# chrism0dwk/covid19uk

Hardware: AMD Instinct MI355X
Metric: posterior samples/sec, 380-LAD UK SEIR (higher is better)
Workload: dtype f64; 1 GPU; uk380: M=380 LADs x T=365 days, P=750 parameters; chains_per_gpu=8, chains_total=8, sweep=HMC(16 leapfrogs) + 5 x [S->E move, E->I move, S->E occult, E->I occult], draws_recorded=theta + events[M,T,3] (uint16 counts) + kernel results per sweep, parallelism=chains sharded over 1 GPU(s), no data-path collective

## Files before the change

covid19uk_amd/_lib.py:

```python
from __future__ import annotations

import ctypes
import os

_HERE = os.path.dirname(os.path.abspath(__file__))
LIB_PATH = os.path.join(_HERE, "libseirhip.so")

c_double_p = ctypes.POINTER(ctypes.c_double)
c_void_pp = ctypes.POINTER(ctypes.c_void_p)
c_int64_p = ctypes.POINTER(ctypes.c_int64)


class SeirDesc(ctypes.Structure):
    _fields_ = [
        ("M", ctypes.c_int32), ("T", ctypes.c_int32),
        ("max_chains", ctypes.c_int32), ("device", ctypes.c_int32),
        ("Cstar", c_double_p), ("N", c_double_p), ("W", c_double_p),
        ("weekday_c", c_double_p), ("log_area_c", c_double_p),
        ("car_Q", c_double_p), ("car_half_logdet", ctypes.c_double),
        ("init_state", c_double_p),
        ("nu", ctypes.c_double), ("time_delta", ctypes.c_double),
        ("rate_floor", ctypes.c_double),
    ]


class SeirSamplerDesc(ctypes.Structure):
    _fields_ = [
        ("num_chains", ctypes.c_int32),
        ("dmax", ctypes.c_int32), ("nmax", ctypes.c_int32), ("m", ctypes.c_int32),
        ("occult_nmax", ctypes.c_int32), ("num_event_time_updates", ctypes.c_int32),
        ("t_range_lo", ctypes.c_int32), ("t_range_hi", ctypes.c_int32),
        ("num_leapfrog_steps", ctypes.c_int32), ("trace_capacity", ctypes.c_int32),
        ("first_chain_id", ctypes.c_int32), ("record_events", ctypes.c_int32),
        ("seed", ctypes.c_uint64),
        ("moves_mode", ctypes.c_int32), ("hmc_mode", ctypes.c_int32), ("use_graph", ctypes.c_int32),
        ("chain_groups", ctypes.c_int32), ("disable_mask", ctypes.c_int32), ("debug_pair", ctypes.c_int32),
        ("leap_rows", ctypes.c_int32), ("thin", ctypes.c_int32),
    ]


class SeirSimDesc(ctypes.Structure):
    _fields_ = [
        ("num_draws", ctypes.c_int32), ("num_steps", ctypes.c_int32),
        ("first_draw_id", ctypes.c_int32), ("reserved", ctypes.c_int32),
        ("seed", ctypes.c_uint64),
        ("par", ctypes.POINTER(ctypes.c_double)), ("log_baseline", ctypes.POINTER(ctypes.c_double)),
        ("spatial", ctypes.POINTER(ctypes.c_double)), ("W", ctypes.POINTER(ctypes.c_double)),
        ("weekday_c", ctypes.POINTER(ctypes.c_double)), ("init_state", ctypes.POINTER(ctypes.c_double)),
        ("events", ctypes.POINTER(ctypes.c_double)),
    ]


ABI_VERSION = 4
OPT_DEBUG_SKEW, OPT_XCD_AFFINITY, OPT_GEMM_F32, OPT_EVAL_FORM, OPT_RT_STAGING_KIB = 0, 1, 2, 3, 4
ERR_INVALID, ERR_STATE = -1, -3
ERR_HANDOFF = -4
MMAX = 4
MOVE_TRACE = 2 + 4 * MMAX
FORECAST_MAX_H = 128
FORECAST_ID_SHIFT, FORECAST_MAX_CHAIN = 20, 2048
CHECK_MAX_DAYS = 128
ORDER_STATS_MAX_RANKS = 16
GROUPS_MAX = 256
SELFTEST_FN = {"fast_log": (0, False, False), "fast_rcp": (1, False, False), "mv_log": (2, False, False),
               "softplus_tab": (3, False, False), "softplus_sigmoid_tab": (4, False, True), "softplus": (5, False, False),
               "lfact_bf": (6, False, False), "lbinom_tab": (7, True, False), "lbinom_const": (8, True, False),
               "lbinom_bf": (9, True, False), "log1mexp_tab": (10, False, False), "log1mexp": (11, False, False),
               "log1mexp_series": (12, False, True), "l1me_inv_series": (13, False, True), "l1me_inv_k": (14, False, True),
               "l1me_inv_series_k": (15, False, True), "log1mexp_diff_slow": (16, True, False), "fast_log_k": (17, False, False)}
SELFTEST_DELTA = {"band": 0, "own_ei": 1, "own_se": 2}
SELFTEST_WAVE = {"wave_sum": (0, True), "wave_min": (1, False), "wave_incl_scan": (2, True),
                 "wave_incl_suffix_scan": (3, False), "block_excl_scan_256": (4, True),
                 "block_incl_suffix_scan_256": (5, False), "block_sum_256": (6, False)}


class SeirError(RuntimeError):
    def __init__(self, msg, code=0):
        super().__init__(msg)
        self.code = code


class HandoffTimeout(SeirError):
    """A wait inside one of the persistent launches gave up (SEIR_ERR_HANDOFF from a read of the trace): its
    workgroups were not all resident -- something else holds part of the GPU.  `ChainSampler` recovers from it by
    itself (snapshot, restore, per-step launch forms)."""


_SIGNATURES = {
    "seir_abi_version": (ctypes.c_int, []),
    "seir_last_error": (ctypes.c_char_p, []),
    "seir_create": (ctypes.c_int, [ctypes.POINTER(SeirDesc), c_void_pp]),
    "seir_destroy": (None, [ctypes.c_void_p]),
    "seir_num_params": (ctypes.c_int, [ctypes.c_void_p]),
    "seir_set_initial_state": (ctypes.c_int, [ctypes.c_void_p, c_double_p]),
    "seir_log_prob": (ctypes.c_int, [ctypes.c_void_p, ctypes.c_int32, c_double_p, c_double_p, c_double_p]),
    "seir_log_prob_grad": (ctypes.c_int, [ctypes.c_void_p, ctypes.c_int32, c_double_p, c_double_p,
                                          c_double_p, c_double_p]),
    "seir_log_prob_dev": (ctypes.c_int, [ctypes.c_void_p, ctypes.c_int32] + [ctypes.c_void_p] * 4),
    "seir_prepare_events_dev": (ctypes.c_int, [ctypes.c_void_p, ctypes.c_int32, ctypes.c_void_p]),
    "seir_eval_prepared_dev": (ctypes.c_int, [ctypes.c_void_p, ctypes.c_int32] + [ctypes.c_void_p] * 3),
    "seir_sync": (ctypes.c_int, [ctypes.c_void_p]),
    "seir_stream": (ctypes.c_void_p, [ctypes.c_void_p]),
    "seir_set_option": (ctypes.c_int, [ctypes.c_void_p, ctypes.c_int32, ctypes.c_int32]),
    "seir_malloc": (ctypes.c_int, [c_void_pp, ctypes.c_uint64]),
    "seir_free": (ctypes.c_int, [ctypes.c_void_p]),
    "seir_memcpy_h2d": (ctypes.c_int, [ctypes.c_void_p, ctypes.c_void_p, ctypes.c_uint64]),
    "seir_memcpy_d2h": (ctypes.c_int, [ctypes.c_void_p, ctypes.c_void_p, ctypes.c_uint64]),
    "seir_timer_start": (ctypes.c_int, [ctypes.c_void_p]),
    "seir_timer_stop": (ctypes.c_int, [ctypes.c_void_p, ctypes.POINTER(ctypes.c_float)]),
    "seir_time_kernel": (ctypes.c_int, [ctypes.c_void_p, ctypes.c_int32, ctypes.c_int32, ctypes.c_int32,
                                        ctypes.POINTER(ctypes.c_float)]),
    "seir_selftest_math": (ctypes.c_int, [ctypes.c_void_p, ctypes.c_int32] + [c_double_p] * 4),
    "seir_selftest_math_wide": (ctypes.c_int, [ctypes.c_void_p, ctypes.c_int32] + [c_double_p] * 3),
    "seir_selftest_fn": (ctypes.c_int, [ctypes.c_void_p, ctypes.c_int32, ctypes.c_int32] + [c_double_p] * 4),
    "seir_selftest_band_delta": (ctypes.c_int, [ctypes.c_void_p, ctypes.c_int32, ctypes.c_int32] + [c_double_p] * 7 +
                                 [ctypes.c_double, ctypes.c_double, c_double_p]),
    "seir_selftest_wave": (ctypes.c_int, [ctypes.c_void_p, ctypes.c_int32, ctypes.c_int32, ctypes.c_int32] +
                           [ctypes.c_void_p] * 3),
    "seir_reproduction_number": (ctypes.c_int, [ctypes.c_void_p, ctypes.c_int32, c_double_p, c_double_p, c_double_p]),
    "seir_within_between": (ctypes.c_int, [ctypes.c_void_p, ctypes.c_int32, c_double_p, c_double_p, ctypes.c_double,
                                           c_double_p, c_double_p]),
    "seir_simulate": (ctypes.c_int, [ctypes.c_void_p, ctypes.POINTER(SeirSimDesc)]),
    "seir_selftest_binomial": (ctypes.c_int, [ctypes.c_void_p, ctypes.c_int32, ctypes.POINTER(ctypes.c_int32),
                                              c_double_p, ctypes.c_uint64, ctypes.POINTER(ctypes.c_int32)]),
    "seir_sampler_create": (ctypes.c_int, [ctypes.c_void_p, ctypes.POINTER(SeirSamplerDesc), c_void_pp]),
    "seir_sampler_destroy": (None, [ctypes.c_void_p]),
    "seir_sampler_set_state": (ctypes.c_int, [ctypes.c_void_p, c_double_p, c_double_p]),
    "seir_sampler_get_state": (ctypes.c_int, [ctypes.c_void_p, c_double_p, c_double_p, c_double_p]),
    "seir_sampler_set_kernel": (ctypes.c_int, [ctypes.c_void_p, c_double_p, c_double_p]),
    "seir_sampler_get_kernel": (ctypes.c_int, [ctypes.c_void_p, c_double_p, c_double_p]),
    "seir_sampler_set_adaptation": (ctypes.c_int, [ctypes.c_void_p, ctypes.c_int32, ctypes.c_int32,
                                                   ctypes.c_int32, ctypes.c_double, c_double_p, c_double_p,
                                                   c_double_p]),
    "seir_sampler_refresh": (ctypes.c_int, [ctypes.c_void_p]),
    "seir_sampler_reset_trace": (ctypes.c_int, [ctypes.c_void_p]),
    "seir_sampler_reset_trace_at": (ctypes.c_int, [ctypes.c_void_p, ctypes.c_int32]),
    "seir_sampler_set_thin": (ctypes.c_int, [ctypes.c_void_p, ctypes.c_int32]),
    "seir_sampler_thin": (ctypes.c_int, [ctypes.c_void_p, ctypes.POINTER(ctypes.c_int32)]),
    "seir_sampler_read_trace_async": (ctypes.c_int, [ctypes.c_void_p, ctypes.c_int32, ctypes.c_int32, c_double_p,
                                                     ctypes.c_void_p, c_double_p, c_double_p]),
    "seir_sampler_trace_wait": (ctypes.c_int, [ctypes.c_void_p]),
    "seir_host_alloc": (ctypes.c_int, [c_void_pp, ctypes.c_uint64]),
    "seir_host_free": (ctypes.c_int, [ctypes.c_void_p]),
    "seir_sampler_run": (ctypes.c_int, [ctypes.c_void_p, ctypes.c_int32]),
    "seir_sampler_read_trace": (ctypes.c_int, [ctypes.c_void_p, ctypes.c_int32, ctypes.c_int32, c_double_p,
                                               ctypes.c_void_p, c_double_p, c_double_p]),
    "seir_sampler_time_grad_kernel": (ctypes.c_int, [ctypes.c_void_p, ctypes.c_int32,
                                                     ctypes.POINTER(ctypes.c_float)]),
    "seir_sampler_time_leapfrog": (ctypes.c_int, [ctypes.c_void_p, ctypes.c_int32, ctypes.POINTER(ctypes.c_float),
                                                  ctypes.POINTER(ctypes.c_int32), ctypes.POINTER(ctypes.c_int32)]),
    "seir_sampler_pair_timeouts": (ctypes.c_int, [ctypes.c_void_p, ctypes.POINTER(ctypes.c_uint32)]),
    "seir_sampler_xcd_local": (ctypes.c_int, [ctypes.c_void_p]),
    "seir_sampler_snapshot": (ctypes.c_int, [ctypes.c_void_p, ctypes.c_int32]),
    "seir_sampler_restore": (ctypes.c_int, [ctypes.c_void_p, ctypes.c_int32]),
    "seir_sampler_debug_fail_handoff": (ctypes.c_int, [ctypes.c_void_p, ctypes.c_int32]),
    "seir_sampler_set_launch_form": (ctypes.c_int, [ctypes.c_void_p, ctypes.c_int32, ctypes.c_int32]),
    "seir_sampler_launch_form": (ctypes.c_int, [ctypes.c_void_p, ctypes.POINTER(ctypes.c_int32),
                                                ctypes.POINTER(ctypes.c_int32)]),
    "seir_sampler_summary_reset": (ctypes.c_int, [ctypes.c_void_p]),
    "seir_sampler_summarize": (ctypes.c_int, [ctypes.c_void_p, ctypes.c_int32, ctypes.c_int32, ctypes.c_int32]),
    "seir_sampler_read_marginals": (ctypes.c_int, [ctypes.c_void_p, ctypes.c_int32, ctypes.c_int32,
                                                   c_int64_p, c_int64_p, c_int64_p]),
    "seir_sampler_read_marginals_async": (ctypes.c_int, [ctypes.c_void_p, ctypes.c_int32, ctypes.c_int32,
                                                         c_int64_p, c_int64_p, c_int64_p]),
    "seir_sampler_read_summary": (ctypes.c_int, [ctypes.c_void_p, ctypes.POINTER(ctypes.c_uint64),
                                                 ctypes.POINTER(ctypes.c_int32), c_int64_p,
                                                 ctypes.POINTER(ctypes.c_uint64)]),
    "seir_sampler_diag_reset": (ctypes.c_int, [ctypes.c_void_p, ctypes.c_int32]),
    "seir_sampler_diag_mark": (ctypes.c_int, [ctypes.c_void_p, ctypes.c_int32]),
    "seir_sampler_read_diag": (ctypes.c_int, [ctypes.c_void_p, ctypes.POINTER(ctypes.c_uint64), c_int64_p,
                                              ctypes.POINTER(ctypes.c_uint64)]),
    "seir_sampler_read_diag_mark": (ctypes.c_int, [ctypes.c_void_p, ctypes.c_int32, ctypes.POINTER(ctypes.c_uint64),
                                                   c_int64_p, ctypes.POINTER(ctypes.c_uint64)]),
    "seir_sampler_forecast_reset": (ctypes.c_int, [ctypes.c_void_p, ctypes.c_int32, c_double_p, c_double_p, ctypes.c_uint64]),
    "seir_sampler_forecast": (ctypes.c_int, [ctypes.c_void_p, ctypes.c_int32, ctypes.c_int32, c_double_p]),
    "seir_sampler_read_forecast_marginals": (ctypes.c_int, [ctypes.c_void_p, ctypes.c_int32, ctypes.c_int32,
                                                            c_int64_p, c_int64_p, c_int64_p]),
    "seir_sampler_read_forecast_marginals_async": (ctypes.c_int, [ctypes.c_void_p, ctypes.c_int32, ctypes.c_int32,
                                                                  c_int64_p, c_int64_p, c_int64_p]),
    "seir_sampler_read_forecast": (ctypes.c_int, [ctypes.c_void_p, ctypes.POINTER(ctypes.c_uint64),
                                                  ctypes.POINTER(ctypes.c_int32), c_int64_p,
                                                  ctypes.POINTER(ctypes.c_uint64)]),
    "seir_sampler_forecast_keep": (ctypes.c_int, [ctypes.c_void_p, ctypes.c_int64]),
    "seir_sampler_forecast_order_stats": (ctypes.c_int, [ctypes.c_void_p, c_int64_p, ctypes.c_int32, ctypes.c_int32,
                                                         ctypes.POINTER(ctypes.c_int32)]),
    "seir_order_stats": (ctypes.c_int, [ctypes.c_void_p, ctypes.POINTER(ctypes.c_int32), ctypes.c_int64, ctypes.c_int32,
                                        ctypes.c_int64, ctypes.c_int64, ctypes.c_int64, c_int64_p, ctypes.c_int32,
                                        ctypes.POINTER(ctypes.c_int32)]),
    "seir_sampler_check_reset": (ctypes.c_int, [ctypes.c_void_p, ctypes.c_int32, c_double_p, c_double_p, ctypes.c_uint64]),
    "seir_sampler_check": (ctypes.c_int, [ctypes.c_void_p, ctypes.c_int32, ctypes.c_int32]),
    "seir_sampler_read_check": (ctypes.c_int, [ctypes.c_void_p, ctypes.POINTER(ctypes.c_uint64),
                                               ctypes.POINTER(ctypes.c_int32), c_int64_p, ctypes.POINTER(ctypes.c_uint64)]),
    "seir_sampler_read_check_marginals": (ctypes.c_int, [ctypes.c_void_p, ctypes.c_int32, ctypes.c_int32,
                                                         c_int64_p, c_int64_p, c_int64_p]),
    "seir_sampler_read_check_marginals_async": (ctypes.c_int, [ctypes.c_void_p, ctypes.c_int32, ctypes.c_int32,
                                                               c_int64_p, c_int64_p, c_int64_p]),
    "seir_sampler_read_check_counts": (ctypes.c_int, [ctypes.c_void_p, ctypes.POINTER(ctypes.c_int32)] +
                                       [ctypes.POINTER(ctypes.c_uint32)] * 8),
    "seir_sampler_rt_reset": (ctypes.c_int, [ctypes.c_void_p, ctypes.c_int32, c_double_p]),
    "seir_sampler_rt": (ctypes.c_int, [ctypes.c_void_p, ctypes.c_int32, ctypes.c_int32]),
    "seir_sampler_read_rt_draws": (ctypes.c_int, [ctypes.c_void_p, ctypes.c_int32, ctypes.c_int32, c_double_p]),
    "seir_sampler_read_rt_draws_async": (ctypes.c_int, [ctypes.c_void_p, ctypes.c_int32, ctypes.c_int32, c_double_p]),
    "seir_sampler_read_rt": (ctypes.c_int, [ctypes.c_void_p, ctypes.POINTER(ctypes.c_uint64), c_double_p, c_double_p,
                                            c_double_p, ctypes.POINTER(ctypes.c_uint32)]),
    "seir_sampler_rt_keep": (ctypes.c_int, [ctypes.c_void_p, ctypes.c_int64]),
    "seir_sampler_rt_order_stats": (ctypes.c_int, [ctypes.c_void_p, c_int64_p, ctypes.c_int32, ctypes.c_int32, c_double_p]),
    "seir_order_stats_f64": (ctypes.c_int, [ctypes.c_void_p, c_double_p, ctypes.c_int64, ctypes.c_int32, ctypes.c_int64,
                                            ctypes.c_int64, ctypes.c_int64, c_int64_p, ctypes.c_int32, c_double_p]),
    "seir_sampler_wb_reset": (ctypes.c_int, [ctypes.c_void_p, ctypes.c_int32]),
    "seir_sampler_wb": (ctypes.c_int, [ctypes.c_void_p, ctypes.c_int32, ctypes.c_int32]),
    "seir_sampler_read_wb": (ctypes.c_int, [ctypes.c_void_p, ctypes.POINTER(ctypes.c_uint64), ctypes.POINTER(ctypes.c_uint32),
                                            c_double_p, c_double_p, c_double_p, c_double_p, c_double_p,
                                            ctypes.POINTER(ctypes.c_uint32)]),
    "seir_sampler_read_wb_draws": (ctypes.c_int, [ctypes.c_void_p, ctypes.c_int32, ctypes.c_int32, c_double_p, c_double_p]),
    "seir_sampler_read_wb_draws_async": (ctypes.c_int, [ctypes.c_void_p, ctypes.c_int32, ctypes.c_int32, c_double_p,
                                                        c_double_p]),
    "seir_sampler_groups_set": (ctypes.c_int, [ctypes.c_void_p, ctypes.c_int32, ctypes.POINTER(ctypes.c_int32),
                                               ctypes.POINTER(ctypes.c_int32)]),
    "seir_sampler_read_group_marginals": (ctypes.c_int, [ctypes.c_void_p, ctypes.c_int32, ctypes.c_int32, ctypes.c_int32,
                                                         c_int64_p, c_int64_p]),
    "seir_sampler_read_group_marginals_async": (ctypes.c_int, [ctypes.c_void_p, ctypes.c_int32, ctypes.c_int32, ctypes.c_int32,
                                                               c_int64_p, c_int64_p]),
    "seir_group_sums": (ctypes.c_int, [ctypes.c_void_p, ctypes.POINTER(ctypes.c_int32), ctypes.c_int64, ctypes.c_int32,
                                       ctypes.c_int32, ctypes.c_int32, ctypes.POINTER(ctypes.c_int32),
                                       ctypes.POINTER(ctypes.c_int32), c_int64_p]),
    "seir_sampler_group_rt": (ctypes.c_int, [ctypes.c_void_p, c_double_p]),
    "seir_sampler_group_wb": (ctypes.c_int, [ctypes.c_void_p, ctypes.c_int32]),
    "seir_sampler_read_group_rt": (ctypes.c_int, [ctypes.c_void_p, ctypes.c_int32, ctypes.c_int32, c_double_p]),
    "seir_sampler_read_group_rt_async": (ctypes.c_int, [ctypes.c_void_p, ctypes.c_int32, ctypes.c_int32, c_double_p]),
    "seir_sampler_read_group_wb": (ctypes.c_int, [ctypes.c_void_p, ctypes.c_int32, ctypes.c_int32, c_double_p, c_double_p]),
    "seir_sampler_read_group_wb_async": (ctypes.c_int, [ctypes.c_void_p, ctypes.c_int32, ctypes.c_int32, c_double_p, c_double_p]),
    "seir_group_wsums": (ctypes.c_int, [ctypes.c_void_p, c_double_p, ctypes.c_int64, ctypes.c_int32, ctypes.c_int32,
                                        ctypes.c_int32, ctypes.POINTER(ctypes.c_int32), ctypes.POINTER(ctypes.c_int32),
                                        c_double_p, c_double_p]),
}

_lib = None


def exported_symbols():
    return sorted(_SIGNATURES)


def load():
    global _lib
    if _lib is None:
        if not os.path.exists(LIB_PATH):
            raise SeirError(
                f"{LIB_PATH} not found: build the HIP extension first "
                "(python -c 'import __graft_entry__ as g; g.build()'). "
                "This package has no CPU fallback.")
        try:
            import torch
        except ImportError:
            pass
        lib = ctypes.CDLL(LIB_PATH)
        for name, (res, args) in _SIGNATURES.items():
            fn = getattr(lib, name)
            fn.restype = res
            fn.argtypes = args
        if lib.seir_abi_version() != ABI_VERSION:
            raise SeirError(f"{LIB_PATH} has ABI {lib.seir_abi_version()}, this binding needs {ABI_VERSION}: rebuild it")
        _lib = lib
    return _lib


def check(rc):
    if rc != 0:
        msg = load().seir_last_error()
        text = msg.decode() if msg else "?"
        cls = HandoffTimeout if rc == ERR_HANDOFF else SeirError
        raise cls(f"libseirhip call failed ({rc}): {text}", rc)
```

covid19uk_amd/csrc/moves_kernel.h:

```cpp
#pragma once
#include "handoff.h"
#include "sampler_kernels.h"

namespace seir {

#ifdef SEIR_STAMPS
#ifndef SEIR_STAMP_SLOT
#define SEIR_STAMP_SLOT 1
#endif
#define MSTAMP(i) do { if (threadIdx.x == 0 && stamp_on) ((unsigned long long *)(stamp_hs + 16))[i] = __builtin_amdgcn_s_memrealtime(); } while (0)
#else
#define MSTAMP(i) do {} while (0)
#endif

#ifdef PAIR_STAMPS
#define QSTAMP(slot_, step_, i_) do { if (threadIdx.x == 0 && (b_stamp) == 0 && (step_) < 12 && (slot_) < 27) \
    ch.leap_st[((size_t)(slot_) * 12 + (step_)) * 16 + (i_)] = __builtin_amdgcn_s_memrealtime(); } while (0)
#else
#define QSTAMP(slot_, step_, i_) do {} while (0)
#endif

constexpr int MVB = 512;
constexpr int MVW = MVB / WAVE;
constexpr int MVU = 4;

struct MvShared {
    Move mv;
    int acc;
    int nsel;
    int sel[MMAX];
    int ired[MVW * 4];
    double dred[MVW * 2];
    double u[2 * MMAX][2];
    double logq_part[MMAX];
    int pend_valid[MMAX];
};

template <int CTRL, int ROW_MASK>
__device__ __forceinline__ int dpp_min_step(int v) {
    return min(v, __builtin_amdgcn_update_dpp(0x7fffffff, v, CTRL, ROW_MASK, 0xf, false));
}
__device__ __forceinline__ int wave_min_int(int v) {
    v = dpp_min_step<0x111, 0xf>(v);
    v = dpp_min_step<0x112, 0xf>(v);
    v = dpp_min_step<0x114, 0xf>(v);
    v = dpp_min_step<0x118, 0xf>(v);
    v = dpp_min_step<0x142, 0xa>(v);
    v = dpp_min_step<0x143, 0xc>(v);
    return __builtin_amdgcn_readlane(v, 63);
}

__device__ __forceinline__ void mv_sum2(double &a, double &b2, double *sh) {
    a = wave_sum(a); b2 = wave_sum(b2);
    const int lane = threadIdx.x & 63, wave = threadIdx.x >> 6;
    lds_barrier();
    if (lane == 0) { sh[wave * 2] = a; sh[wave * 2 + 1] = b2; }
    lds_barrier();
    double x = 0.0, y = 0.0;
#pragma unroll
    for (int j = 0; j < MVW; ++j) { x += sh[j * 2]; y += sh[j * 2 + 1]; }
    a = x; b2 = y;
}

struct MvLds {
    const int *rt;
    int *rg;
#ifdef SEIR_STAMPS
    double *stamp_hs; bool stamp_on;
#endif
};

__device__ __forceinline__ double mv_log(double x, const double2 *ltab) { return x == 1.0 ? 0.0 : fast_log(x, ltab); }

__device__ inline void mv_draw(const SamplerCfg &s, const Chains &ch, int b, MoveSpec spec, MvShared &sm, int T) {
    Move &mv = sm.mv;
    const int tid = threadIdx.x;
    if (tid >= 2 * MMAX && tid != 64) return;
    const RngKey key = rng_key(s, ch, b);
    const uint32_t stream = RS_MOVE_BASE + (uint32_t)(spec.scan * 4 + spec.slot);
    if (tid < 2 * MMAX) rng_uniform2(key, stream, (uint32_t)tid, sm.u[tid][0], sm.u[tid][1]);
    if (tid == 64) {
        mv.valid = (s.disable_mask >> (1 + spec.slot)) & 1 ? 0 : 1;
        mv.n = 0; mv.tgt = spec.tgt; mv.kind = spec.kind; mv.slot = spec.slot;
        mv.logq = 0.0; mv.any_dI = 0; mv.LO = T; mv.HI = -1;
        for (int j = 0; j < MMAX; ++j) { mv.tm[j] = mv.tt[j] = mv.tdt[j] = mv.tx[j] = 0; mv.b[j] = -1; sm.pend_valid[j] = -1; }
        double ua, ub;
        rng_uniform2(key, stream, 15u, ua, ub);
        mv.logu = cold_log(ua);
    }
}

__device__ __forceinline__ int wv_popc(unsigned long long m) { return __builtin_popcountll(m); }
__device__ __forceinline__ int wv_kth_bit(unsigned long long mask, int k, int lane) {
    const int below = (int)__builtin_amdgcn_mbcnt_hi((unsigned)(mask >> 32), __builtin_amdgcn_mbcnt_lo((unsigned)mask, 0u));
    const bool me = ((mask >> lane) & 1ull) != 0ull && below == k;
    return (int)__builtin_ctzll(__builtin_amdgcn_ballot_w64(me));
}
constexpr int WV_MCH = 6;
struct HotRows {
    unsigned long long mask[WV_MCH];
    int H;
};
__device__ __forceinline__ HotRows wv_hot_rows(const int *tot, int M, int lane) {
    HotRows h;
    h.H = 0;
    if (M <= WV_MCH * WAVE) {
        int v[WV_MCH];
#pragma unroll
        for (int c = 0; c < WV_MCH; ++c) { const int m = c * WAVE + lane; v[c] = m < M ? tot[m] : 0; }
#pragma unroll
        for (int c = 0; c < WV_MCH; ++c) { h.mask[c] = __builtin_amdgcn_ballot_w64(v[c] > 0); h.H += wv_popc(h.mask[c]); }
    } else {
#pragma unroll
        for (int c = 0; c < WV_MCH; ++c) h.mask[c] = 0ull;
        for (int m0 = 0; m0 < M; m0 += WAVE) {
            const int m = m0 + lane;
            h.H += wv_popc(__builtin_amdgcn_ballot_w64(m < M && tot[m] > 0));
        }
    }
    return h;
}
__device__ __forceinline__ int wv_hot_row(const HotRows &h, const int *tot, int M, int p, int lane) {
    int row = 0;
    bool found = false;
    if (M <= WV_MCH * WAVE) {
#pragma unroll
        for (int c = 0; c < WV_MCH; ++c) {
            const int cnt = wv_popc(h.mask[c]);
            if (!found && p < cnt) { row = c * WAVE + wv_kth_bit(h.mask[c], p, lane); found = true; }
            if (!found) p -= cnt;
        }
    } else {
        for (int m0 = 0; m0 < M; m0 += WAVE) {
            const int m = m0 + lane;
            const unsigned long long mask = __builtin_amdgcn_ballot_w64(m < M && tot[m] > 0);
            const int cnt = wv_popc(mask);
            if (!found && p < cnt) { row = m0 + wv_kth_bit(mask, p, lane); found = true; }
            if (!found) p -= cnt;
        }
    }
    return row;
}
template <int NCH>
__device__ __forceinline__ int wv_at(const int (&v)[NCH], int t) {
    int r = 0;
#pragma unroll
    for (int c = 0; c < NCH; ++c)
        if ((t >> 6) == c) r = __builtin_amdgcn_readlane(v[c], t & 63);
    return r;
}

template <int NCH>
__device__ inline void mv_propose_wave(const Dims &d, const Work &w, const SamplerCfg &s, const Chains &ch, int b,
                                       MoveSpec spec, MvShared &sm, const MvLds &L, const double2 *ltab,
                                       bool rows_only) {
    Move &mv = sm.mv;
    const int tid = threadIdx.x, wave = tid >> 6, lane = tid & 63, M = d.M, T = d.T;
#ifdef SEIR_STAMPS
    double *stamp_hs = L.stamp_hs; const bool stamp_on = L.stamp_on;
#endif
    MSTAMP(4);
    const int tgt = spec.tgt;
    lds_barrier();
    if (spec.kind == 0) {
        const int *rt = L.rt;
        const HotRows hr = wv_hot_rows(rt, M, lane);
        const int H = hr.H;
        const int nsel = min(min(s.mmax, MMAX), H);
        int pos[MMAX], chosen[MMAX], rowj[MMAX];
#pragma unroll
        for (int j = 0; j < MMAX; ++j) { pos[j] = 0; rowj[j] = 0; chosen[j] = 0x7fffffff; }
#pragma unroll
        for (int j = 0; j < MMAX; ++j) {
            if (j < nsel) {
                int p = rng_index(sm.u[2 * j][0], H - j);
#pragma unroll
                for (int a = 0; a < MMAX; ++a)
                    if (a < j && p >= chosen[a]) ++p;
                pos[j] = p;
                chosen[j] = p;
#pragma unroll
                for (int a = MMAX - 1; a >= 1; --a)
                    if (a <= j && chosen[a - 1] > chosen[a]) { const int tmp = chosen[a]; chosen[a] = chosen[a - 1]; chosen[a - 1] = tmp; }
            }
        }
#pragma unroll
        for (int j = 0; j < MMAX; ++j)
            if (j < nsel) rowj[j] = wv_hot_row(hr, rt, M, pos[j], lane);
        if (rows_only) {
            if (tid == 0) {
                sm.nsel = nsel;
#pragma unroll
                for (int j = 0; j < MMAX; ++j)
                    if (j < nsel) sm.sel[j] = rowj[j];
            }
            lds_barrier();
            return;
        }
        MSTAMP(5);
        if (wave < nsel) {
            const int j = wave;
            int m = 0;
#pragma unroll
            for (int jj = 0; jj < MMAX; ++jj)
                if (jj == j) m = rowj[jj];
            const size_t rowoff = ((size_t)b * d.Mp + m) * d.Tp;
            int rk[NCH], rsrc[NCH], rdst[NCH];
#pragma unroll
            for (int c = 0; c < NCH; ++c) {
                const int t = c * WAVE + lane;
                const bool in = t < T;
                rk[c] = in ? w.K[tgt][rowoff + t] : 0;
                rsrc[c] = in ? w.St[tgt][rowoff + t] : 0;
                rdst[c] = in ? w.St[tgt + 1][rowoff + t] : 0;
            }
            MSTAMP(6);
            int D = 0;
            unsigned long long hot[NCH];
#pragma unroll
            for (int c = 0; c < NCH; ++c) { hot[c] = __builtin_amdgcn_ballot_w64(rk[c] > 0); D += wv_popc(hot[c]); }
            int r = rng_index(sm.u[2 * j][1], D), t = 0;
            {
                bool found = false;
#pragma unroll
                for (int c = 0; c < NCH; ++c) {
                    const int cnt = wv_popc(hot[c]);
                    if (!found && r < cnt) { t = c * WAVE + wv_kth_bit(hot[c], r, lane); found = true; }
                    if (!found) r -= cnt;
                }
            }
            MSTAMP(7);
// ... 323 lines not shown
            } else {
                __syncthreads();
                for (int m = tid; m < M; m += MVB) rtl[m] = w.rowtot[((size_t)b * 2 + next.tgt) * d.Mp + m];
            }
            lds_barrier();
        } else {
            if (pre_rt) {
#pragma unroll
                for (int k = 0; k < PRE_RT; ++k) {
                    const int m = tid + k * MVB;
                    if (m < M) L.rg[m] = rt_pre[k];
                }
                lds_barrier();
                if (patch && tid == 0)
                    for (int i = 0; i < pend.n; ++i) {
                        if (pend.a[i] >= s.tr_lo && pend.a[i] < s.tr_hi) L.rg[pend.m[i]] += pend.dka[i];
                        if (pend.b[i] >= s.tr_lo && pend.b[i] < s.tr_hi) L.rg[pend.m[i]] += pend.dkb[i];
                    }
                lds_barrier();
            } else {
                __syncthreads();
                range_totals_to_lds(d, w, s, b, next.tgt, L.rg);
            }
        }
        MSTAMP(3);
#ifdef SEIR_STAMPS
        L.stamp_hs = stamp_hs; L.stamp_on = stamp_on;
#endif
        mv_propose<NCH>(d, w, s, ch, b, next, sm, L, ltab);
        MSTAMP(10);
        if (tid == 0) ch.mv[(size_t)(pbuf ^ 1) * s.B + b] = sm.mv;
        MSTAMP(11);
    }
}

constexpr int PRE_RT = 4;

__device__ __forceinline__ void mv_prefetch_rows(const Dims &d, const Work &w, const SamplerCfg &s, int b, MoveSpec spec,
                                                 bool on, int (&pre)[PRE_RT]) {
    const int tid = threadIdx.x;
#pragma unroll
    for (int k = 0; k < PRE_RT; ++k) {
        const int m = tid + k * MVB;
        pre[k] = 0;
        if (on && m < d.M) {
            if (spec.kind == 0) {
                pre[k] = w.rowtot[((size_t)b * 2 + spec.tgt) * d.Mp + m];
            } else {
                pre[k] = w.rngtot[((size_t)b * 2 + spec.tgt) * d.Mp + m];
            }
        }
    }
}

__device__ __forceinline__ void mv_rows_to_lds(const Dims &d, const Work &w, const SamplerCfg &s, int b, MoveSpec spec,
                                               bool pre_ok, const int (&pre)[PRE_RT], const Move *fix, MvLds &L,
                                               int *rtl) {
    const int tid = threadIdx.x, M = d.M;
    int *dst = spec.kind == 0 ? rtl : L.rg;
    if (pre_ok) {
#pragma unroll
        for (int k = 0; k < PRE_RT; ++k) {
            const int m = tid + k * MVB;
            if (m < M) dst[m] = pre[k];
        }
        lds_barrier();
        if (fix && tid == 0)
            for (int i = 0; i < fix->n; ++i) {
                if (spec.kind == 0) {
                    dst[fix->m[i]] += fix->dka[i] + fix->dkb[i];
                } else {
                    if (fix->a[i] >= s.tr_lo && fix->a[i] < s.tr_hi) dst[fix->m[i]] += fix->dka[i];
                    if (fix->b[i] >= s.tr_lo && fix->b[i] < s.tr_hi) dst[fix->m[i]] += fix->dkb[i];
                }
            }
        lds_barrier();
    } else {
        __syncthreads();
        if (spec.kind == 0) {
            for (int m = tid; m < M; m += MVB) dst[m] = w.rowtot[((size_t)b * 2 + spec.tgt) * d.Mp + m];
            lds_barrier();
        } else {
            range_totals_to_lds(d, w, s, b, spec.tgt, L.rg);
        }
    }
}

__device__ __forceinline__ void mv_apply_rows(const Dims &d, const Work &w, const SamplerCfg &s, int b, const Move &mv,
                                              int *trans = nullptr) {
    const int tid = threadIdx.x;
    for (int i = 0; i < mv.n; ++i) {
        const size_t rowoff = ((size_t)b * d.Mp + mv.m[i]) * d.Tp;
        const int src = mv.tgt, dst = mv.tgt + 1;
        for (int t = mv.lo[i] + 1 + tid; t <= mv.hi[i]; t += MVB) {
            w.St[src][rowoff + t] += mv.dsrc[i];
            w.St[dst][rowoff + t] -= mv.dsrc[i];
            if (mv.tgt == 1) w.Dir[(size_t)b * d.Tp + t] -= (double)mv.dsrc[i];
        }
        if (tid == 0) {
            w.K[mv.tgt][rowoff + mv.a[i]] += mv.dka[i];
            if (mv.b[i] >= 0) w.K[mv.tgt][rowoff + mv.b[i]] += mv.dkb[i];
            int *prt = w.rowtot + ((size_t)b * 2 + mv.tgt) * d.Mp + mv.m[i];
            const int dk = mv.dka[i] + mv.dkb[i];
            const int ra = (mv.a[i] >= s.tr_lo && mv.a[i] < s.tr_hi) ? mv.dka[i] : 0;
            const int rb = (mv.b[i] >= s.tr_lo && mv.b[i] < s.tr_hi) ? mv.dkb[i] : 0;
            int *prg = w.rngtot + ((size_t)b * 2 + mv.tgt) * d.Mp + mv.m[i];
            if (trans != nullptr) {
                const int rt0 = *prt, rg0 = (ra + rb != 0) ? *prg : 1;
                int tb = 0;
                if ((rt0 > 0) != (rt0 + dk > 0)) tb |= 1;
                if (ra + rb != 0 && (rg0 > 0) != (rg0 + ra + rb > 0)) tb |= 2;
                *trans |= tb;
                *prt = rt0 + dk;
                if (ra + rb != 0) *prg = rg0 + ra + rb;
            } else {
                *prt += dk;
                if (ra + rb != 0) *prg += ra + rb;
            }
        }
        __syncthreads();
    }
}

__device__ __forceinline__ void mv_trace(const SamplerCfg &s, const Chains &ch, int b, const Move &mv, int acc,
                                         unsigned tr_slot, double lp) {
    if (tr_slot < (unsigned)s.cap) {
        double *tr = ch.tr_mv + (((size_t)tr_slot * s.B + b) * 4 + mv.slot) * NMVTR;
        tr[0] = (double)acc;
        tr[1] = lp;
        for (int j = 0; j < MMAX; ++j) {
            tr[2 + j] = mv.tm[j]; tr[2 + MMAX + j] = mv.tt[j];
            tr[2 + 2 * MMAX + j] = mv.tdt[j]; tr[2 + 3 * MMAX + j] = mv.tx[j];
        }
    }
}

__device__ __forceinline__ void mv_own_rows_to_down(const Dims &d, const Consts &c, const Work &w, int b, const Move &mv,
                                                    double psi, const double2 *ltab, const Move *fp, double *red,
                                                    double *od) {
    double dth = 0.0, dcn = 0.0;
    if (mv.valid && mv.n > 0) own_rows_delta<MVB>(d, c, w, b, mv, psi, 0, d.M, ltab, dth, dcn, fp);
    mv_sum2(dth, dcn, red);
    if (threadIdx.x == 0) {
        od[0] = dth;
        od[1] = dcn;
    }
}

struct PairNote {
    int ok;
    int n, rows[MMAX];
};
static_assert(sizeof(PairNote) == (2 + MMAX) * sizeof(int), "k_move_pair writes the note as 2 + MMAX ints");

__device__ __forceinline__ void move_copy_l2(Move *dst, const Move *src, int t0) {
    const int i = (int)threadIdx.x - t0;
    if (i >= 0 && i < MOVE_DW) reinterpret_cast<int *>(dst)[i] = ld_l2(reinterpret_cast<const int *>(src) + i);
}
__device__ __forceinline__ void wait_token(const unsigned *p_, unsigned token, unsigned *late) {
    hs_wait<1, HS_CHECK, HS_LIMIT, HS_CALLER>([&] { return ld_l2(p_) == token; }, late);
}
__device__ __forceinline__ unsigned wait_token_flag(const unsigned *p_, unsigned token, unsigned *late) {
    unsigned v;
    hs_wait<1, HS_CHECK, HS_LIMIT, HS_CALLER>([&] { return ((v = ld_l2(p_)) & 0x7fffffffu) == token; }, late);
    return v >> 31;
}
static_assert((MOVE_DW + 1) / 2 <= 32, "Chains::llmv holds 32 words per descriptor");
template <bool SOLO, typename TT>
__device__ __forceinline__ TT ld_band(const TT *p_) { return SOLO ? *p_ : ld_l2(p_); }
template <bool SOLO, int NRB>
__device__ __forceinline__ void pair_band_block(const Dims &d, const Consts &c, const Work &w, const SamplerCfg &s,
                                                const Chains &ch, int b, int bx, int nband, unsigned token, bool has_r1,
                                                bool has_r2, int buf, int st_slot = 0, int st_step = 0) {
    const int b_stamp = b - d.b0;
    (void)b_stamp;
    __shared__ Move mvA, mvB, fp;
    __shared__ int mv_sel;
    __shared__ double sh_th[MVW], sh_cn[MVW];
    __shared__ double2 ltab[LDSTAB_N];
    int tid = threadIdx.x;
    asm volatile("" : "+v"(tid));
    const int wave = tid >> 6, lane = tid & 63;
    if (tid < LDSTAB_N) ltab[tid] = c.logtab[tid];
    const double psi = w.scal[(size_t)b * NSCAL + SC_PSI];
    const unsigned *done = ch.done + (size_t)b * 2 * TAIL_STRIDE;
    const int rpb = (d.M + nband - 1) / nband;
    const int r_lo = bx * rpb, r_hi = min(d.M, r_lo + rpb);
#ifndef PAIR_BAND_BACKOFF
#define PAIR_BAND_BACKOFF 0
#endif
    if (tid == 0) {
        if (PAIR_BAND_BACKOFF > 0) __builtin_amdgcn_s_sleep(PAIR_BAND_BACKOFF);
        wait_token(done + 4, token, ch.late + ch.late_fatal + b);
    }
    QSTAMP(st_slot, st_step, 1);
    __syncthreads();
    move_copy_l2(&fp, ch.fpend + b, 128);
    __syncthreads();
    const bool has_fp = fp.valid == 1;
    constexpr int NPF = 2;
    constexpr bool PREF = NRB == 2;
    constexpr int NRP = PREF ? NRB : 1;
    double cfb[NRP][MMAX], Fpre[NRP][NPF];
#pragma unroll
    for (int r = 0; r < NRP; ++r) {
        const int j = r_lo + wave + r * MVW;
        const bool onr = PREF && has_fp && j < r_hi;
#pragma unroll
        for (int i = 0; i < MMAX; ++i)
            cfb[r][i] = (onr && i < fp.n) ? c.Cstar[(size_t)fp.m[i] * d.Kp0 + j] * c.invN[fp.m[i]] * (double)(-fp.dsrc[i]) : 0.0;
#pragma unroll
        for (int q = 0; q < NPF; ++q) {
            const int t = fp.LO + q * WAVE + lane;
            Fpre[r][q] = (onr && t <= fp.HI) ? ld_band<SOLO>(w.F + ((size_t)b * d.Mp + j) * d.Tp + t) : 0.0;
        }
    }
    const bool pre_ok = PREF && (!has_fp || fp.HI - fp.LO < NPF * WAVE);
    if (tid == 0) wait_token(done + 5, token, ch.late + ch.late_fatal + b);
    if (has_r1) {
        if (wave == 1) move_wait_ll<MOVE_DW>(reinterpret_cast<int *>(&mvA), ch.llmv + ((size_t)buf * s.B + b) * 32, lane, token, ch.late + ch.late_fatal + b);
        QSTAMP(st_slot, st_step, 2);
        __syncthreads();
    } else {
        QSTAMP(st_slot, st_step, 2);
        __syncthreads();
        move_copy_l2(&mvA, ch.mv + (size_t)buf * s.B + b, 0);
        __syncthreads();
    }
    auto evaluate = [&](const Move &mv) -> double {
        double dth = 0.0;
        if (mv.valid && mv.n > 0 && mv.any_dI) {
            const double *ea = w.ea + (size_t)b * d.Tp;
            constexpr int NR = 2;
    #pragma unroll 1
            for (int r0 = 0; r0 < NRB; r0 += NR) {
            int jr[NR];
            bool on[NR];
            double eb[NR], coef[NR][MMAX], cfp[NR][MMAX];
    #pragma unroll
            for (int r = 0; r < NR; ++r) {
                jr[r] = r_lo + wave + (r0 + r) * MVW;
                bool mine = false;
    #pragma unroll
                for (int i = 0; i < MMAX; ++i) mine |= (i < mv.n && mv.m[i] == jr[r]);
                on[r] = jr[r] < r_hi && !mine;
                const int j = on[r] ? jr[r] : r_lo;
                eb[r] = w.eb[(size_t)b * d.Mp + j];
    #pragma unroll
                for (int i = 0; i < MMAX; ++i) {
                    coef[r][i] = (on[r] && i < mv.n) ? c.Cstar[(size_t)mv.m[i] * d.Kp0 + j] * c.invN[mv.m[i]] * (double)(-mv.dsrc[i]) : 0.0;
                    if (PREF) cfp[r][i] = on[r] ? cfb[PREF ? r : 0][i] : 0.0;
                    else cfp[r][i] = (has_fp && on[r] && i < fp.n) ? c.Cstar[(size_t)fp.m[i] * d.Kp0 + j] * c.invN[fp.m[i]] * (double)(-fp.dsrc[i]) : 0.0;
                }
            }
            for (int t0 = mv.LO; t0 <= mv.HI; t0 += WAVE) {
                const int t = t0 + lane;
                double dF[NR], S[NR], I[NR], kse[NR], F[NR];
                bool act[NR];
    #pragma unroll
                for (int r = 0; r < NR; ++r) {
                    dF[r] = 0.0;
    #pragma unroll
                    for (int i = 0; i < MMAX; ++i)
                        if (i < mv.n && t > mv.lo[i] && t <= mv.hi[i]) dF[r] += coef[r][i];
                    act[r] = on[r] && t <= mv.HI && dF[r] != 0.0;
                    const size_t q = ((size_t)b * d.Mp + (on[r] ? jr[r] : r_lo)) * d.Tp + (act[r] ? t : mv.LO);
                    S[r] = (double)ld_band<SOLO>(w.St[0] + q); I[r] = (double)ld_band<SOLO>(w.St[2] + q);
                    kse[r] = (double)ld_band<SOLO>(w.K[0] + q); F[r] = ld_band<SOLO>(w.F + q);
                }
    #pragma unroll
                for (int r = 0; r < NR; ++r) {
                    if (!act[r]) continue;
                    if (has_fp) {
                        double dFp = 0.0;
    #pragma unroll
                        for (int i = 0; i < MMAX; ++i)
                            if (i < fp.n && t > fp.lo[i] && t <= fp.hi[i]) dFp += cfp[r][i];
                        if (dFp != 0.0) F[r] += dFp;
                    }
                    dth += band_delta(S[r], I[r], kse[r], F[r], dF[r], ea[t] * eb[r], psi * c.W[t], d.rate_floor * d.dt, d.dt, ltab);
                }
            }
            }
        }
        return dth;
    };
    double dth = evaluate(mvA);
    QSTAMP(st_slot, st_step, 3);
    if (tid == 0) mv_sel = (int)wait_token_flag(done + 0, token, ch.late + ch.late_fatal + b);
    __syncthreads();
    if (mv_sel) {
        move_copy_l2(&mvB, ch.mvfix + (size_t)buf * s.B + b, 64);
        __syncthreads();
        dth = evaluate(mvB);
    }
    dth = wave_sum(dth);
    if (lane == 0) sh_th[wave] = dth;
    __syncthreads();
    double dsum = 0.0;
    if (tid == 0) {
#pragma unroll
        for (int k = 0; k < MVW; ++k) dsum += sh_th[k];
        if (!SOLO) {
            double *out = ch.Dpart + ((size_t)b * nband + bx) * 2;
            out[0] = dsum;
            out[1] = 0.0;
        }
        QSTAMP(st_slot, st_step, 4);
        if (has_fp) {
            if (has_r1) wait_token(done + 1, token, ch.late + ch.late_fatal + b);
            if (has_r2) wait_token(done + 2, token, ch.late + ch.late_fatal + b);
        }
        QSTAMP(st_slot, st_step, 5);
    }
    auto publish = [&]() {
        if (!SOLO) return;
        asm volatile("s_waitcnt vmcnt(0)" ::: "memory");
        __syncthreads();
        if (tid == 0) {
            uint4 *out = ch.llD + (((size_t)buf * s.B + b) * nband + bx) * 2;
            pair_sums_store(out, dsum, 0.0, token);
            QSTAMP(st_slot, st_step, 10);
        }
    };
    if (!has_fp) { publish(); return; }
    if (!has_fp) return;
    __syncthreads();
#pragma unroll
    for (int r = 0; r < NRB; ++r) {
        const int j = r_lo + wave + r * MVW;
        if (j >= r_hi) continue;
        double *Fr = w.F + ((size_t)b * d.Mp + j) * d.Tp;
        double cfr[MMAX];
#pragma unroll
        for (int i = 0; i < MMAX; ++i) {
            if (PREF) cfr[i] = cfb[PREF ? r : 0][i];
            else cfr[i] = i < fp.n ? c.Cstar[(size_t)fp.m[i] * d.Kp0 + j] * c.invN[fp.m[i]] * (double)(-fp.dsrc[i]) : 0.0;
        }
        if (pre_ok) {
#pragma unroll
            for (int q = 0; q < NPF; ++q) {
                const int t = fp.LO + q * WAVE + lane;
                double dFp = 0.0;
#pragma unroll
                for (int i = 0; i < MMAX; ++i)
                    if (i < fp.n && t > fp.lo[i] && t <= fp.hi[i]) dFp += cfr[i];
                if (t <= fp.HI && dFp != 0.0) Fr[t] = Fpre[PREF ? r : 0][q] + dFp;
            }
        } else {
            for (int t = fp.LO + lane; t <= fp.HI; t += WAVE) {
                double dFp = 0.0;
#pragma unroll
                for (int i = 0; i < MMAX; ++i)
                    if (i < fp.n && t > fp.lo[i] && t <= fp.hi[i]) dFp += cfr[i];
                if (dFp != 0.0) Fr[t] = ld_band<SOLO>(Fr + t) + dFp;
            }
        }
    }
    publish();
    (void)sh_cn;
}

__device__ __forceinline__ void pair_band_finish(const Dims &d, const Consts &c, const Work &w, const SamplerCfg &s,
                                                 const Chains &ch, int b, int bx, int nband, unsigned token, unsigned slot,
                                                 int record) {
    __shared__ Move fp;
    int tid = threadIdx.x;
    asm volatile("" : "+v"(tid));
    const int wave = tid >> 6, lane = tid & 63;
    const unsigned *done = ch.done + (size_t)b * 2 * TAIL_STRIDE;
    const int rpb = (d.M + nband - 1) / nband;
    const int r_lo = bx * rpb, r_hi = min(d.M, r_lo + rpb);
    if (tid == 0) wait_token(done + 4, token, ch.late + ch.late_fatal + b);
    __syncthreads();
    move_copy_l2(&fp, ch.fpend + b, 128);
    if (tid == 0) wait_token(done + 5, token, ch.late + ch.late_fatal + b);
    __syncthreads();
    for (int m = r_lo + wave; m < r_hi; m += MVW) {
        if (fp.valid == 1) {
            double coef[MMAX];
#pragma unroll
            for (int i = 0; i < MMAX; ++i)
                coef[i] = i < fp.n ? c.Cstar[(size_t)fp.m[i] * d.Kp0 + m] * c.invN[fp.m[i]] * (double)(-fp.dsrc[i]) : 0.0;
            double *Fr = w.F + ((size_t)b * d.Mp + m) * d.Tp;
            for (int t = fp.LO + lane; t <= fp.HI; t += WAVE) {
                double dF = 0.0;
#pragma unroll
                for (int i = 0; i < MMAX; ++i)
                    if (i < fp.n && t > fp.lo[i] && t <= fp.hi[i]) dF += coef[i];
                if (dF != 0.0) Fr[t] += dF;
            }
        }
        if (!record || slot >= (unsigned)s.cap) continue;
        const size_t o0 = (((size_t)slot * s.B + b) * d.M + m) * d.T * 3;
        int *out = (int *)ch.tr_events + o0;
        unsigned short *out16 = (unsigned short *)ch.tr_events + o0;
        const size_t q0 = ((size_t)b * d.Mp + m) * d.Tp;
        for (int t0 = 0; t0 < d.T; t0 += 4 * WAVE) {
            int k0[4], k1[4], k2[4];
#pragma unroll
            for (int j = 0; j < 4; ++j) {
                const int t = t0 + j * WAVE + lane;
                const bool in = t < d.Tp;
                k0[j] = in ? w.K[0][q0 + t] : 0;
                k1[j] = in ? w.K[1][q0 + t] : 0;
                k2[j] = in ? w.K[2][q0 + t] : 0;
            }
#pragma unroll
            for (int j = 0; j < 4; ++j) {
                const int t = t0 + j * WAVE + lane;
                if (t < d.T) {
                    if (s.ev16) {
                        if ((unsigned)(k0[j] | k1[j] | k2[j]) > 0xffffu) ch.ev_overflow[0] = 1u;
                        out16[t * 3 + 0] = (unsigned short)k0[j]; out16[t * 3 + 1] = (unsigned short)k1[j];
                        out16[t * 3 + 2] = (unsigned short)k2[j];
                    } else {
                        out[t * 3 + 0] = k0[j]; out[t * 3 + 1] = k1[j]; out[t * 3 + 2] = k2[j];
                    }
                }
            }
        }
    }
}

template <int NCH, bool SOLO>
__device__ __forceinline__ void pair_step(const Dims &d, const Consts &c, const Work &w, const SamplerCfg &s, const Chains &ch,
                                          MoveSpec se, MoveSpec next, MoveSpec se_next, int have_prev, int have_pre, int pbuf,
                                          int lidx, int dbg, int nband, int nroles, int slot, int b, int fin = 0,
                                          unsigned sweep0 = 0u, int lprev = 0, unsigned tslot = TRACE_NOT_RECORDED) {
    extern __shared__ __attribute__((aligned(16))) int dyn_i[];
    __shared__ MvShared sm_se, sm_nx;
    __shared__ Move pendA, pendB;
    __shared__ PairNote note;
    __shared__ double pre_down[2], s_down[4], s_dsum[2];
    __shared__ double2 ltab[LDSTAB_N];
    __shared__ int s_sel, s_acc_se, s_conf, s_late, s_late2, s_use_pre, s_trans;
    int tid = threadIdx.x;
    asm volatile("" : "+v"(tid));
    asm volatile("" : "+s"(b));
    const int b_stamp = b - d.b0;
    (void)b_stamp;
    QSTAMP(slot, lidx, 0);
    if (slot >= nroles) {
        if (nband == 0) return;
        if (fin) {
            pair_band_finish(d, c, w, s, ch, b, slot - nroles, nband, pair_token(sweep0, lidx), tslot, fin & 2);
            return;
        }
        const unsigned tok = pair_token(ch.sweep[b], lidx);
        const bool r1 = next.kind >= 0 && nroles >= 2, r2 = se_next.kind >= 0 && nroles == 3;
        if ((d.M + nband - 1) / nband > 2 * MVW)
            pair_band_block<SOLO, 4>(d, c, w, s, ch, b, slot - nroles, nband, tok, r1, r2, pbuf ^ 1, slot, lidx);
        else
            pair_band_block<SOLO, 2>(d, c, w, s, ch, b, slot - nroles, nband, tok, r1, r2, pbuf ^ 1, slot, lidx);
        return;
    }
    const int role = slot == nroles - 1 ? 0 : slot + 1;
    const int M = d.M, T = d.T;
    const bool do_se = role == 0 && se.kind >= 0, do_nx = next.kind >= 0, do_pre = se_next.kind >= 0 && nroles == 3;
    if (role == 1 && !do_nx) return;
    if (role == 2 && !do_pre) return;
#ifdef SEIR_STAMPS
    double *stamp_hs = ch.hs + (size_t)b * NHS;
    const bool stamp_on = do_se && b == 0 && se.slot == (SEIR_STAMP_SLOT & 2) && se.scan == 0;
#define PSTAMP(i) do { if (threadIdx.x == 0 && stamp_on) ((unsigned long long *)(stamp_hs + 16))[i] = __builtin_amdgcn_s_memrealtime(); } while (0)
#ifndef SEIR_STAMP_ROLE
#define SEIR_STAMP_ROLE 1
#endif
    const bool rstamp_on = role == SEIR_STAMP_ROLE && b == 0 && se.slot == (SEIR_STAMP_SLOT & 2) && se.scan == 0;
#ifdef SEIR_STAMP_PROPOSE
#define RSTAMP(i) do { if (threadIdx.x == 0 && rstamp_on) ((unsigned long long *)(stamp_hs + 16))[(i) + 4] = __builtin_amdgcn_s_memrealtime(); } while (0)
#undef PSTAMP
#define PSTAMP(i) do {} while (0)
#else
#define RSTAMP(i) do { if (threadIdx.x == 0 && rstamp_on) ((unsigned long long *)(stamp_hs + 16))[i] = __builtin_amdgcn_s_memrealtime(); } while (0)
#endif
#else
#define PSTAMP(i) do {} while (0)
#define RSTAMP(i) do {} while (0)
#endif
    PSTAMP(0);
    RSTAMP(8);
    const bool pre_ok = M <= PRE_RT * MVB;
    const MoveSpec &mine = role == 2 ? se_next : next;
    int pre_se[PRE_RT], pre_nx[PRE_RT];
    mv_prefetch_rows(d, w, s, b, se, do_se && pre_ok, pre_se);
    mv_prefetch_rows(d, w, s, b, mine, (role == 2 || do_nx) && pre_ok, pre_nx);
    const unsigned token = pair_token(ch.sweep[b], lidx);
    double dth0 = 0.0, dcn0 = 0.0;
    int ld_i = 0;
    double ld_d = 0.0;
    if (have_prev) {
        if (tid >= 64 && tid < 64 + MOVE_DW) ld_i = reinterpret_cast<const int *>(ch.mv + (size_t)pbuf * s.B + b)[tid - 64];
        if (tid >= 128 && tid < 128 + MOVE_DW) ld_i = reinterpret_cast<const int *>(ch.mvfix + (size_t)pbuf * s.B + b)[tid - 128];
        if (tid == 192) ld_i = ch.mvsel[(size_t)pbuf * s.B + b];
        if (tid >= 196 && tid < 200) ld_d = ch.Down[(((size_t)pbuf * 2 + ((tid - 196) >> 1)) * s.B + b) * 2 + ((tid - 196) & 1)];
        if (!SOLO) {
            if (tid < s.nrb_d) {
                dth0 = ch.Dpart[((size_t)b * s.nrb_d + tid) * 2];
                dcn0 = ch.Dpart[((size_t)b * s.nrb_d + tid) * 2 + 1];
            }
            for (int i = tid + MVB; i < s.nrb_d; i += MVB) {
                dth0 += ch.Dpart[((size_t)b * s.nrb_d + i) * 2];
                dcn0 += ch.Dpart[((size_t)b * s.nrb_d + i) * 2 + 1];
            }
        }
    }
    constexpr int DW0 = SOLO ? MVB - WAVE : 0;
    if (SOLO && have_prev) {
        static_assert(MVB >= 253, "one thread per band workgroup (plan_sweep: 3 + nband <= 256)");
        const bool few = s.nrb_d <= WAVE;
        const int i0 = few ? tid - DW0 : tid;
        if (few ? tid >= DW0 : (tid & ~(WAVE - 1)) < s.nrb_d) {
            const uint4 *src = ch.llD + (((size_t)pbuf * s.B + b) * s.nrb_d + min(i0, s.nrb_d - 1)) * 2;
            double th, cn;
            pair_sums_wait(src, pair_token(ch.sweep[b], lprev), ch.late + ch.late_fatal + b, th, cn);
            if (i0 < s.nrb_d) { dth0 = th; dcn0 = cn; }
#ifdef PAIR_STAMPS
            if (tid == DW0 && b_stamp == 0 && lidx < 12) ch.leap_st[((size_t)slot * 12 + lidx) * 16 + 7] = __builtin_amdgcn_s_memrealtime();
#endif
        }
    }
    const bool pre_avail = do_se && have_pre;
    if (pre_avail) {
        if (tid >= 256 && tid < 256 + MOVE_DW) ld_i = reinterpret_cast<const int *>(ch.mvs + (size_t)pbuf * s.B + b)[tid - 256];
        if (tid >= 320 && tid < 320 + 2 + MMAX) ld_i = reinterpret_cast<const int *>(ch.prev + (size_t)pbuf * s.B + b)[tid - 320];
        if (tid == 328 || tid == 329) ld_d = ch.DownS[((size_t)pbuf * s.B + b) * 2 + (tid - 328)];
    }
    static_assert(MOVE_DW <= 64 && 2 + MMAX <= 8, "the entry loads of pair_step: disjoint thread ranges");
    double hs_th = 0.0, hs_cn = 0.0, psi = 0.0;
    unsigned tr_slot = 0xffffffffu;
    double2 ld_t = make_double2(0.0, 0.0);
    if (tid < LDSTAB_N) ld_t = c.logtab[tid];
    if (role == 0 && tid == 0) {
        const double *hs = ch.hs + (size_t)b * NHS;
        hs_th = hs[HS_LP_THETA]; hs_cn = hs[HS_LP_CONST];
        tr_slot = SOLO ? tslot : chain_trace_slot(s, ch, ch.sweep[b]);
    }
    psi = w.scal[(size_t)b * NSCAL + SC_PSI];
    QSTAMP(slot, lidx, 6);
    if (do_se && !pre_avail) mv_draw(s, ch, b, se, sm_se, T);
    if (role != 0 || do_nx) mv_draw(s, ch, b, mine, sm_nx, T);
    QSTAMP(slot, lidx, 14);
    if (have_prev) {
        if (tid >= 64 && tid < 64 + MOVE_DW) reinterpret_cast<int *>(&pendA)[tid - 64] = ld_i;
        if (tid >= 128 && tid < 128 + MOVE_DW) reinterpret_cast<int *>(&pendB)[tid - 128] = ld_i;
        if (tid == 192) s_sel = ld_i;
        if (tid >= 196 && tid < 200) s_down[tid - 196] = ld_d;
    }
    if (pre_avail) {
        if (tid >= 256 && tid < 256 + MOVE_DW) reinterpret_cast<int *>(&sm_se.mv)[tid - 256] = ld_i;
        if (tid >= 320 && tid < 320 + 2 + MMAX) reinterpret_cast<int *>(&note)[tid - 320] = ld_i;
        if (tid == 328 || tid == 329) pre_down[tid - 328] = ld_d;
    }
    if (tid < LDSTAB_N) ltab[tid] = ld_t;
    if (have_prev && s.nrb_d <= WAVE && tid >= DW0 && tid < DW0 + WAVE) {
        const double a = wave_sum(dth0), a2 = wave_sum(dcn0);
        if (tid == DW0) { s_dsum[0] = 0.0 + a; s_dsum[1] = 0.0 + a2; }
    }
    if (role != 0) {
        asm volatile("s_waitcnt vmcnt(0)" ::: "memory");
        QSTAMP(slot, lidx, 12);
        __syncthreads();
        QSTAMP(slot, lidx, 13);
        const int late_bit = role == 1 ? 1 : 4, absent_bit = role == 1 ? 2 : 8;
        if (dbg & late_bit)
            for (int i = 0; i < 100; ++i) __builtin_amdgcn_s_sleep(127);
        if (tid == 0 && !(dbg & absent_bit))
            st_l2((role == 1 ? ch.hand : ch.hand2) + b, token);
    }
    MvLds L{};
    int *rtl = dyn_i + M;
    L.rt = rtl;
    L.rg = dyn_i;
    bool pend_acc = false;
    const Move *pendp = nullptr;
    if (have_prev) {
        __syncthreads();
        QSTAMP(slot, lidx, 15);
        const Move &pend = s_sel ? pendB : pendA;
        pendp = &pend;
        if (s.nrb_d <= WAVE) {
            dth0 = s_dsum[0]; dcn0 = s_dsum[1];
        } else {
            mv_sum2(dth0, dcn0, sm_nx.dred);
        }
        dth0 += s_down[s_sel ? 2 : 0];
        dcn0 += s_down[s_sel ? 3 : 1];
        const double ratio = dth0 + dcn0 + pend.logq;
        pend_acc = pend.valid && pend.logu < ratio;
    }
    if (role != 0) {
        const Move *fix = (pend_acc && pendp->tgt == mine.tgt) ? pendp : nullptr;
        RSTAMP(9);
#if defined(SEIR_STAMPS) && defined(SEIR_STAMP_PROPOSE)
        L.stamp_hs = stamp_hs; L.stamp_on = rstamp_on;
#endif
        QSTAMP(slot, lidx, 1);
        mv_rows_to_lds(d, w, s, b, mine, pre_ok, pre_nx, fix, L, rtl);
        mv_propose<NCH>(d, w, s, ch, b, mine, sm_nx, L, ltab);
        QSTAMP(slot, lidx, 2);
        RSTAMP(10);
        Move *out = (role == 1 ? ch.mv : ch.mvs) + (size_t)(pbuf ^ 1) * s.B + b;
        move_copy(out, &sm_nx.mv, MVB - WAVE);
        if (nband > 0 && role == 1 && tid >= MVB - WAVE)
            move_store_ll<MOVE_DW>(ch.llmv + ((size_t)(pbuf ^ 1) * s.B + b) * 32, reinterpret_cast<const int *>(&sm_nx.mv), tid - (MVB - WAVE),
                                   token);
        const Move *fpp = (pend_acc && pendp->any_dI) ? pendp : nullptr;
        double *od = role == 1 ? ch.Down + (((size_t)(pbuf ^ 1) * 2 + 0) * s.B + b) * 2
                               : ch.DownS + ((size_t)(pbuf ^ 1) * s.B + b) * 2;
        mv_own_rows_to_down(d, c, w, b, sm_nx.mv, psi, ltab, fpp, sm_nx.dred, od);
        QSTAMP(slot, lidx, 3);
        RSTAMP(11);
        if (nband > 0) {
            __syncthreads();
            if (tid == 0)
                st_l2(ch.done + (size_t)b * 2 * TAIL_STRIDE + role, token);
        }
        return;
    }
    if (!have_prev && tid == 64) {
        ch.fpend[b].valid = 0;
        if (nband > 0) {
            asm volatile("s_waitcnt vmcnt(0)" ::: "memory");
            st_l2(ch.done + (size_t)b * 2 * TAIL_STRIDE + 4, token);
        }
    }
    bool late = false, late2 = false;
    auto wait_roles = [&]() {
        if (tid == 0) {
            const bool l1 = do_nx && hs_wait<2, 0, HS_LIMIT_ROLES, HS_NONE>([&] { return ld_l2(ch.hand + b) == token; });
            const bool l2 = do_pre && hs_wait<2, 0, HS_LIMIT_ROLES, HS_NONE>([&] { return ld_l2(ch.hand2 + b) == token; });
            s_late = l1; s_late2 = l2;
            if (l1 || l2) ch.late[b] += 1;
            __builtin_amdgcn_fence(__ATOMIC_ACQUIRE, "agent");
        }
        lds_barrier();
        late = s_late != 0;
        late2 = s_late2 != 0;
    };
    bool waited = !do_nx && !do_pre;
    if (have_prev) {
        const Move &mv = *pendp;
        if (pend_acc && !waited) { wait_roles(); waited = true; }
        if (pend_acc && mv.any_dI) move_copy(ch.fpend + b, &mv, MVB - WAVE);
        else if (tid == MVB - WAVE) ch.fpend[b].valid = 0;
        if (nband > 0 && tid >= MVB - WAVE) {
            asm volatile("s_waitcnt vmcnt(0)" ::: "memory");
            if (tid == MVB - WAVE)
                st_l2(ch.done + (size_t)b * 2 * TAIL_STRIDE + 4, token);
        }
        if (pend_acc) mv_apply_rows(d, w, s, b, mv);
        if (tid == 0) {
            if (pend_acc) {
                double *hs = ch.hs + (size_t)b * NHS;
                hs_th += dth0; hs_cn += dcn0;
                hs[HS_LP_THETA] = hs_th; hs[HS_LP_CONST] = hs_cn;
            }
            mv_trace(s, ch, b, mv, pend_acc ? 1 : 0, tr_slot, hs_th + hs_cn);
        }
        lds_barrier();
    }
    PSTAMP(1);
    QSTAMP(slot, lidx, 1);
    if (fin && nband > 0) {
        __syncthreads();
        if (tid == 0)
            st_l2(ch.done + (size_t)b * 2 * TAIL_STRIDE + 5, token);
    }
    bool se_acc = false;
    if (do_se) {
        const Move *fpp = (pend_acc && pendp->any_dI) ? pendp : nullptr;
        if (tid == 0) {
            int use = pre_avail && note.ok;
            if (use) {
                const Move &mv = sm_se.mv;
                for (int i = 0; i < mv.n; ++i) {
                    for (int j = 0; j < note.n; ++j) use &= mv.m[i] != note.rows[j];
                    if (pend_acc)
                        for (int j = 0; j < pendp->n; ++j) use &= mv.m[i] != pendp->m[j];
                }
            }
            s_use_pre = use;
        }
        lds_barrier();
        const bool use_pre = s_use_pre != 0;
        double dth = 0.0, dcn = 0.0;
        if (!use_pre) {
            if (pre_avail) {
                lds_barrier();
                mv_draw(s, ch, b, se, sm_se, T);
            }
            mv_rows_to_lds(d, w, s, b, se, pre_ok, pre_se, nullptr, L, rtl);
            PSTAMP(2);
            mv_propose<NCH>(d, w, s, ch, b, se, sm_se, L, ltab);
            PSTAMP(3);
        }
        const Move &mv = sm_se.mv;
        if (use_pre && fpp == nullptr) {
            dth = pre_down[0]; dcn = pre_down[1];
        } else {
            if (mv.valid && mv.n > 0) own_rows_delta<MVB>(d, c, w, b, mv, psi, 0, M, ltab, dth, dcn, fpp);
            PSTAMP(4);
            mv_sum2(dth, dcn, sm_se.dred);
        }
        if (tid == 0) {
            const double ratio = dth + dcn + mv.logq;
            s_acc_se = (mv.valid && mv.logu < ratio) ? 1 : 0;
        }
        lds_barrier();
        se_acc = s_acc_se != 0;
        if (se_acc && !waited) { wait_roles(); waited = true; }
        if (tid == 0) s_trans = 0;
        if (se_acc) mv_apply_rows(d, w, s, b, mv, &s_trans);
        if (tid == 0) {
            if (se_acc) {
                double *hs = ch.hs + (size_t)b * NHS;
                hs_th += dth; hs_cn += dcn;
                hs[HS_LP_THETA] = hs_th; hs[HS_LP_CONST] = hs_cn;
            }
            mv_trace(s, ch, b, mv, s_acc_se, tr_slot, hs_th + hs_cn);
        }
        __syncthreads();
        if (nband > 0 && tid == 0)
            st_l2(ch.done + (size_t)b * 2 * TAIL_STRIDE + 5, token);
        PSTAMP(5);
        QSTAMP(slot, lidx, 2);
    }
    if (next.kind == -2 && tid == 0) ch.sweep[b] += 1;
    if (do_nx) {
        const bool changed = se_acc || pend_acc;
        if (changed) {
            const Move *fix = (pend_acc && pendp->tgt == next.tgt) ? pendp : nullptr;
            mv_rows_to_lds(d, w, s, b, next, pre_ok, pre_nx, fix, L, rtl);
            PSTAMP(6);
            mv_propose<NCH>(d, w, s, ch, b, next, sm_nx, L, ltab, true);
        }
        if (tid == 0) {
            int conf = late ? 1 : 0;
            if (changed)
                for (int j = 0; j < sm_nx.nsel; ++j) {
                    const int row = sm_nx.sel[j];
                    if (se_acc)
                        for (int i = 0; i < sm_se.mv.n; ++i) conf |= sm_se.mv.m[i] == row;
                    if (pend_acc)
                        for (int i = 0; i < pendp->n; ++i) conf |= pendp->m[i] == row;
                }
            s_conf = conf;
            ch.mvsel[(size_t)(pbuf ^ 1) * s.B + b] = conf;
        }
        lds_barrier();
        if (s_conf) {
            mv_propose<NCH>(d, w, s, ch, b, next, sm_nx, L, ltab);
            move_copy(ch.mvfix + (size_t)(pbuf ^ 1) * s.B + b, &sm_nx.mv, MVB - WAVE);
            const Move *fpp = (pend_acc && pendp->any_dI) ? pendp : nullptr;
            mv_own_rows_to_down(d, c, w, b, sm_nx.mv, psi, ltab, fpp, sm_nx.dred,
                                ch.Down + (((size_t)(pbuf ^ 1) * 2 + 1) * s.B + b) * 2);
        }
        PSTAMP(7);
        QSTAMP(slot, lidx, 3);
    }
    if (do_pre && tid == 0) {
        int *nt = reinterpret_cast<int *>(ch.prev + (size_t)(pbuf ^ 1) * s.B + b);
        const int n_pend = pend_acc ? pendp->n : 0, n_se = se_acc ? sm_se.mv.n : 0;
        const bool se_keeps = !se_acc || (((s_trans & (se_next.kind == 0 ? 1 : 2)) == 0) && n_pend + n_se <= MMAX);
        nt[0] = (se_keeps && !(waited && late2)) ? 1 : 0;
        nt[1] = n_pend + (se_keeps ? n_se : 0);
#pragma unroll
        for (int j = 0; j < MMAX; ++j) {
            int row = -1;
            if (j < n_pend) row = pendp->m[j];
            else if (se_keeps && j - n_pend < n_se) row = sm_se.mv.m[j - n_pend];
            nt[2 + j] = row;
        }
    }
    if (nband > 0) {
        __syncthreads();
        if (tid == 0)
            st_l2(ch.done + (size_t)b * 2 * TAIL_STRIDE + 0, token | ((do_nx && s_conf) ? 0x80000000u : 0u));
    }
}

template <int NCH>
__global__ __launch_bounds__(MVB) void k_move_pair(Dims d, Consts c, Work w, SamplerCfg s, Chains ch, MoveSpec se,
                                                   MoveSpec next, MoveSpec se_next, int have_prev, int have_pre,
                                                   int pbuf, int nbk, int lidx, int dbg, int nband) {
    debug_skew(d);
    const int nroles = (int)gridDim.x / nbk - nband, slot = (int)blockIdx.x / nbk;
    const int b = d.b0 + (int)blockIdx.x - slot * nbk;
    if (d.nlive > 0 && (int)blockIdx.x - slot * nbk >= d.nlive) return;
    pair_step<NCH, false>(d, c, w, s, ch, se, next, se_next, have_prev, have_pre, pbuf, lidx, dbg, nband, nroles, slot, b);
    const int b_stamp = b - d.b0;
    (void)b_stamp;
    QSTAMP(slot, lidx, 8);
}

constexpr int PBAR_STRIDE = 64;
__device__ __forceinline__ void pair_chain_barrier(const Chains &ch, int b, unsigned target, int b_stamp = 0, int st_slot = 0,
                                                   int st_step = 0) {
    asm volatile("s_waitcnt vmcnt(0)" ::: "memory");
    __syncthreads();
    QSTAMP(st_slot, st_step, 10);
    if (threadIdx.x == 0) {
        unsigned *cnt = ch.pbar + (size_t)b * PBAR_STRIDE;
        const unsigned old = add_l2(cnt, 1u);
        __builtin_amdgcn_fence(__ATOMIC_ACQUIRE, "agent");
#ifndef PBAR_SLEEP
#define PBAR_SLEEP 1
#endif
        if (old + 1u != target)
            hs_wait<PBAR_SLEEP, HS_CHECK, HS_LIMIT, HS_CALLER>([&] { return (int)(ld_l2(cnt) - target) >= 0; }, ch.late + ch.late_fatal + b);
        asm volatile("s_waitcnt vmcnt(0)" ::: "memory");
    }
    QSTAMP(st_slot, st_step, 11);
    __syncthreads();
}

__device__ __forceinline__ void pair_band_next_step() {
    __syncthreads();
    if (threadIdx.x == 0) {
        __builtin_amdgcn_fence(__ATOMIC_ACQUIRE, "agent");
        asm volatile("s_waitcnt vmcnt(0)" ::: "memory");
    }
    __syncthreads();
}

constexpr int PAIR_DBG_DELAYS = 16 | 32 | 64 | 128;
__device__ __forceinline__ void pair_debug_delay(int dbg, int slot, int nroles, int pair, int b) {
    const bool band = slot >= nroles, role0 = slot == nroles - 1;
    bool on = ((dbg & 16) && band) || ((dbg & 32) && role0) || ((dbg & 64) && !band && !role0);
    if (dbg & 128) {
        unsigned h = (unsigned)slot * 0x9e3779b1u ^ (unsigned)pair * 0x85ebca6bu ^ (unsigned)b * 0xc2b2ae35u;
        h ^= h >> 15; h *= 0x2c1b3c6du; h ^= h >> 12;
        on = on || h % 3u == 0u;
    }
    if (on)
        for (int i = 0; i < 9; ++i) __builtin_amdgcn_s_sleep(127);
}

template <int NCH>
__global__ __launch_bounds__(MVB) void k_move_pairs(Dims d, Consts c, Work w, SamplerCfg s, Chains ch, int npairs, int pre_on,
                                                    int nbk, int dbg, int nband, unsigned pbase, int fin) {
    debug_skew(d);
    const int nroles = (int)gridDim.x / nbk - nband, slot = (int)blockIdx.x / nbk;
    const int b = d.b0 + (int)blockIdx.x - slot * nbk;
    if (d.nlive > 0 && (int)blockIdx.x - slot * nbk >= d.nlive) return;
    const MoveSpec none{-1, 0, 0, 0};
    const unsigned sweep0 = ch.sweep[b];
    const unsigned tslot = chain_trace_slot(s, ch, sweep0);
    for (int pair = 0; pair <= npairs; ++pair) {
        const bool closing = pair == npairs;
        const int scan = pair >> 1, half = pair & 1, nh = half ^ 1, nscan = scan + half;
        const bool pre = pre_on && pair + 1 < npairs;
        const MoveSpec se = closing ? none : MoveSpec{half, 0, 2 * half, scan};
        const MoveSpec nx = closing ? MoveSpec{-2, 0, 0, 0} : MoveSpec{half, 1, 2 * half + 1, scan};
        const MoveSpec se_next = pre ? MoveSpec{nh, 0, 2 * nh, nscan} : none;
        if (dbg & PAIR_DBG_DELAYS) pair_debug_delay(dbg, slot, nroles, pair, b);
        pair_step<NCH, true>(d, c, w, s, ch, se, nx, se_next, pair > 0 ? 1 : 0, (pair > 0 && pre_on && !closing) ? 1 : 0, pair & 1,
                       closing ? 62 : pair, closing ? 0 : dbg, (closing && !fin) ? 0 : nband, nroles, slot, b, closing ? fin : 0, sweep0,
                       pair - 1, tslot);
        if (closing) break;
        const int b_stamp = b - d.b0;
        (void)b_stamp;
        QSTAMP(slot, pair, 8);
        if (slot < nroles) pair_chain_barrier(ch, b, pbase + (unsigned)((pair + 1) * nroles), b_stamp, slot, pair);
        else pair_band_next_step();
        QSTAMP(slot, pair, 9);
    }
}

inline size_t k_move_pa2_lds_bytes(const Dims &d) {
    return sizeof(int) * ((size_t)2 * d.M);
}
inline size_t k_move_pairs_lds_bytes(const Dims &d) {
    const size_t need = k_move_pa2_lds_bytes(d), half = 82 * 1024;
    return need > half ? need : half;
}

}
```

covid19uk_amd/csrc/seir_hip.hip:

```cpp
#include <hip/hip_runtime.h>

#include <algorithm>
#include <atomic>
#include <cmath>
#include <cstdarg>
#include <cstdio>
#include <cstring>
#include <new>
#include <vector>

#include "../../include/seir_hip.h"
#include "sampler_kernels.h"
#include "sim_kernels.h"
#include "moves_kernel.h"
#include "selftest_kernels.h"
#include "rt_kernels.h"
#include "sweep_plan.h"
#include "summary_kernels.h"
#include "forecast_kernels.h"
#include "check_kernels.h"
#include "rt_trace_kernels.h"
#include "wb_kernels.h"
#include "order_stats_kernels.h"
#include "order_stats64_kernels.h"
// ... 994 lines not shown
        HIP_TRY(hipMemcpyAsync(sp.p, sd->spatial + (size_t)s0 * M, sizeof(double) * nb * M, hipMemcpyHostToDevice, st));
        HIP_TRY(hipMemcpyAsync(init.p, sd->init_state + (size_t)s0 * M * 4, sizeof(double) * nb * M * 4,
                               hipMemcpyHostToDevice, st));
        SimArgs a{};
        a.n = nb; a.S = S; a.first_draw = sd->first_draw_id + s0;
        a.k0 = (uint32_t)(sd->seed & 0xffffffffu); a.k1 = (uint32_t)(sd->seed >> 32);
        a.par = par.as<double>(); a.a_path = ap.as<double>(); a.spatial = sp.as<double>();
        a.W = W.as<double>(); a.wd = wd.as<double>(); a.init = init.as<double>(); a.events = ev.as<double>();
        hipLaunchKernelGGL(k_simulate, dim3(nb), dim3(SIM_THREADS), lds, st, d, ctx->c, a);
        HIP_TRY(hipGetLastError());
        HIP_TRY(hipMemcpyAsync(sd->events + (size_t)s0 * M * S * 3, ev.p, per_draw * nb, hipMemcpyDeviceToHost, st));
        HIP_TRY(hipStreamSynchronize(st));
    }
    return 0;
}

__global__ void k_selftest_binomial(int count, const int *n, const double *p, uint32_t k0, uint32_t k1, int *out) {
    const int i = blockIdx.x * blockDim.x + threadIdx.x;
    if (i >= count) return;
    RngKey key{k0, k1, 0u, (uint32_t)i};
    out[i] = sim_binomial(n[i], p[i], key, RS_SIM_BASE);
}

extern "C" int seir_selftest_binomial(seir_ctx *ctx, int32_t count, const int32_t *n, const double *p, uint64_t seed,
                                      int32_t *out) {
    int rc = check_batch(ctx, 1);
    if (rc) return rc;
    if (count < 1 || !n || !p || !out) return fail(SEIR_ERR_INVALID, "bad arguments");
    DevBuf dn, dp, dout;
    if ((rc = dn.alloc(sizeof(int) * count)) || (rc = dp.alloc(sizeof(double) * count)) ||
        (rc = dout.alloc(sizeof(int) * count)))
        return rc;
    HIP_TRY(hipMemcpyAsync(dn.p, n, sizeof(int) * count, hipMemcpyHostToDevice, ctx->stream));
    HIP_TRY(hipMemcpyAsync(dp.p, p, sizeof(double) * count, hipMemcpyHostToDevice, ctx->stream));
    hipLaunchKernelGGL(k_selftest_binomial, dim3((count + 255) / 256), dim3(256), 0, ctx->stream, count, dn.as<int>(),
                       dp.as<double>(), (uint32_t)(seed & 0xffffffffu), (uint32_t)(seed >> 32), dout.as<int>());
    HIP_TRY(hipGetLastError());
    HIP_TRY(hipMemcpyAsync(out, dout.p, sizeof(int) * count, hipMemcpyDeviceToHost, ctx->stream));
    HIP_TRY(hipStreamSynchronize(ctx->stream));
    return 0;
}

struct Shadowed {
    void *p = nullptr;
    size_t bytes = 0;
    void *snap[2] = {nullptr, nullptr};
    bool valid[2] = {false, false};
};
struct MomentAcc : Shadowed {
    size_t cells = 0, B = 0;
    size_t count_words() const { return (B + 31) / 32 * 32; }
};

static void acc_layout(const MomentAcc &a, MomentBufs &mb) {
    mb.sum = (int64_t *)a.p;
    mb.sumsq = (uint64_t *)(mb.sum + a.cells);
    mb.count = mb.sumsq + a.cells;
    mb.ref = (int32_t *)(mb.count + a.count_words());
    mb.overflow = (unsigned *)(mb.ref + a.cells);
}
static int acc_alloc(Shadowed &a, size_t bytes) {
    a.bytes = bytes;
    HIP_TRY(hipMalloc(&a.p, bytes));
    HIP_TRY(hipMemset(a.p, 0, bytes));
    return 0;
}
static int acc_alloc(MomentAcc &a, size_t cells, size_t B, MomentBufs &mb) {
    a.cells = cells; a.B = B;
    if (int rc = acc_alloc(a, cells * (sizeof(int64_t) + sizeof(uint64_t) + sizeof(int32_t)) + a.count_words() * sizeof(uint64_t) + 8))
        return rc;
    acc_layout(a, mb);
    return 0;
}
static int acc_zero(Shadowed &a, hipStream_t st) {
    HIP_TRY(hipMemsetAsync(a.p, 0, a.bytes, st));
    return 0;
}
static int acc_shadow(Shadowed &a, int slot, bool save, hipStream_t st) {
    if (!save && !a.valid[slot]) return 0;
    if (!a.snap[slot]) HIP_TRY(hipMalloc(&a.snap[slot], a.bytes));
    HIP_TRY(hipMemcpyAsync(save ? a.snap[slot] : a.p, save ? a.p : a.snap[slot], a.bytes, hipMemcpyDeviceToDevice, st));
    if (save) a.valid[slot] = true;
    return 0;
}
static void acc_invalidate(Shadowed &a) { a.valid[0] = a.valid[1] = false; }
static void acc_free(Shadowed &a) {
    for (void *q : {a.p, a.snap[0], a.snap[1]}) if (q) (void)hipFree(q);
    a = Shadowed{};
}
static int acc_read(const MomentAcc &a, hipStream_t st, uint64_t *count, int32_t *ref, int64_t *sum, uint64_t *sumsq, unsigned *flag) {
    MomentBufs mb{};
    acc_layout(a, mb);
    HIP_TRY(hipMemcpyAsync(flag, mb.overflow, sizeof(*flag), hipMemcpyDeviceToHost, st));
    if (count) HIP_TRY(hipMemcpyAsync(count, mb.count, sizeof(uint64_t) * a.B, hipMemcpyDeviceToHost, st));
    if (ref) HIP_TRY(hipMemcpyAsync(ref, mb.ref, sizeof(int32_t) * a.cells, hipMemcpyDeviceToHost, st));
    if (sum) HIP_TRY(hipMemcpyAsync(sum, mb.sum, sizeof(int64_t) * a.cells, hipMemcpyDeviceToHost, st));
    if (sumsq) HIP_TRY(hipMemcpyAsync(sumsq, mb.sumsq, sizeof(uint64_t) * a.cells, hipMemcpyDeviceToHost, st));
    HIP_TRY(hipStreamSynchronize(st));
    return 0;
}

struct GroupOut {
    int64_t *ev = nullptr, *st0 = nullptr;
    int L = 0;
};

struct GroupCurve {
    bool on = false;
    int planes = 1;
    int D = 0, slots = 0;
    int *offsets = nullptr;
    double *weights = nullptr;
    double *cells[2] = {nullptr, nullptr}, *out[2] = {nullptr, nullptr};
};

struct Rollout {
    bool on = false;
    ForecastBufs fb{};
    int slots = 0;
    int ndmax = 0;
    std::vector<void *> allocs;
    MomentAcc acc;
    long long j = 0;
    long long snap_j[2] = {0, 0};
};

struct seir_sampler {
    seir_ctx *ctx = nullptr;
    SamplerCfg cfg{};
    Chains ch{};
    int record_events = 1;
    int cus = 0, leap_occ[2] = {0, 0};
    bool pairs_lds_attr = false;
    std::vector<void *> allocs;
    int ngroups = 1;
    std::vector<hipStream_t> gstream;
    std::vector<hipGraph_t> graph;
    std::vector<hipGraphExec_t> gexec;
    hipEvent_t ev_fork = nullptr;
    std::vector<hipEvent_t> ev_join;
    hipStream_t copy_stream = nullptr;
    hipEvent_t ev_burst = nullptr, ev_copy = nullptr;
    bool copy_pending = false;
    bool use_graph = false;
    int leap_rows = 0;
    std::vector<hipEvent_t> prof_ev;
    int prof_i = -1;
    bool vt_dirty = true;
    unsigned long long leap_rsteps = 0;
    unsigned long long leap_steps = 0;
    bool xcd_local = false;
    unsigned long long tail_count = 0;
    unsigned pbar_count = 0;
    int pair_debug = 0;
    int moves_mode = 0;
    int graph_skew = 0, graph_aff = 3;
    bool have_state = false;
    double *ev_stage = nullptr;
    enum { R_OTHER = 0, R_STATE = 1, R_HANDOFF = 2 };
    struct Region { void *p; size_t bytes; int kind; };
    std::vector<Region> regions;
    void *snap[2] = {nullptr, nullptr};
    bool snap_valid[2] = {false, false};
    size_t snap_bytes = 0;
    bool poisoned = false;
    int poison_chain = 0;
    unsigned poison_count = 0;
    int hmc_mode = 0;
    int thin_pending = 1;
    bool sum_on = false;
    MomentBufs sum{};
    MomentAcc sum_acc;
    bool diag_on = false;
    SummaryDiag<1> diag{};
    Shadowed diag_buf;
    Rollout fc;
    double *fc_steps_host = nullptr;
    double *fc_steps_dev = nullptr;
    hipEvent_t fc_ev_steps = nullptr;
    bool fc_steps_pending = false;
    int *fc_keep = nullptr;
    long long fc_keep_cap = 0;
    Rollout ck;
    CheckCmp ck_cmp{};
    Shadowed ck_cnt;
    bool rt_on = false;
    RtBufs rt{};
    int rt_slots = 0;
    std::vector<void *> rt_allocs;
    Shadowed rt_acc;
    double *rt_keep = nullptr;
    long long rt_keep_cap = 0;
    long long rt_keep_stride = 0;
    long long rt_j = 0;
    long long rt_snap_j[2] = {0, 0};
    bool wb_on = false;
    WbBufs wb{};
    int wb_slots = 0;
    std::vector<void *> wb_allocs;
    Shadowed wb_acc;
    bool grp_on = false;
    GroupTable grp{};
    GroupOut grp_out[3];
    std::vector<int> grp_offsets;
    GroupCurve grt, gwb;
};

template <typename T>
static int s_alloc(seir_sampler *s, std::vector<void *> &list, T **p, size_t count, int kind = seir_sampler::R_OTHER) {
    void *q = nullptr;
    const size_t bytes = (count ? count : 1) * sizeof(T);
    HIP_TRY(hipMalloc(&q, bytes));
    list.push_back(q);
    if (kind != seir_sampler::R_OTHER) s->regions.push_back({q, bytes, kind});
    HIP_TRY(hipMemset(q, 0, bytes));
    *p = (T *)q;
    return 0;
}
#define S_ALLOC(list, ptr, ...) if (!rc) rc = s_alloc(s, s->list, &(ptr), __VA_ARGS__)

static void rollout_free(Rollout &r) {
    for (void *p : r.allocs) (void)hipFree(p);
    r.allocs.clear();
    acc_free(r.acc);
    r.on = false;
    r.fb = ForecastBufs{};
}
static int rollout_shadow(Rollout &r, int slot, bool save, hipStream_t st) {
    if (save) r.snap_j[slot] = r.j;
    else if (r.acc.valid[slot]) r.j = r.snap_j[slot];
    return acc_shadow(r.acc, slot, save, st);
}

static void gcurve_release(GroupCurve &c) {
    for (int x = 0; x < 2; ++x) {
        if (c.cells[x]) (void)hipFree(c.cells[x]);
        if (c.out[x]) (void)hipFree(c.out[x]);
        c.cells[x] = c.out[x] = nullptr;
    }
    if (c.offsets) (void)hipFree(c.offsets);
    c.offsets = nullptr;
    c.D = c.slots = 0;
}
static void gcurve_rt_off(seir_sampler *s) {
    gcurve_release(s->grt);
    if (s->grt.weights) (void)hipFree(s->grt.weights);
    s->grt.weights = nullptr;
    s->grt.on = false;
}
static int gcurve_fit(seir_sampler *s, bool rt);

static void groups_free(seir_sampler *s) {
    gcurve_rt_off(s);
    gcurve_release(s->gwb);
    s->grp_offsets.clear();
    for (GroupOut &o : s->grp_out) {
        if (o.ev) (void)hipFree(o.ev);
        if (o.st0) (void)hipFree(o.st0);
        o = GroupOut{};
    }
    if (s->grp.seg) (void)hipFree(const_cast<int *>(s->grp.seg));
    if (s->grp.members) (void)hipFree(const_cast<int *>(s->grp.members));
    s->grp = GroupTable{};
    s->grp_on = false;
}

static void drop_graph(seir_sampler *s) {
    for (auto &g : s->gexec) if (g) { (void)hipGraphExecDestroy(g); g = nullptr; }
    for (auto &g : s->graph) if (g) { (void)hipGraphDestroy(g); g = nullptr; }
}

extern "C" void seir_sampler_destroy(seir_sampler *s) {
    if (s) for (hipEvent_t e : s->prof_ev) (void)hipEventDestroy(e);
    if (s) s->prof_ev.clear();
    if (!s) return;
    (void)hipSetDevice(s->ctx->device);
    (void)hipStreamSynchronize(s->ctx->stream);
    drop_graph(s);
    for (auto st : s->gstream) if (st) { (void)hipStreamSynchronize(st); (void)hipStreamDestroy(st); }
    for (auto e : s->ev_join) if (e) (void)hipEventDestroy(e);
    if (s->ev_fork) (void)hipEventDestroy(s->ev_fork);
    if (s->copy_stream) { (void)hipStreamSynchronize(s->copy_stream); (void)hipStreamDestroy(s->copy_stream); }
    if (s->ev_burst) (void)hipEventDestroy(s->ev_burst);
    if (s->ev_copy) (void)hipEventDestroy(s->ev_copy);
    for (void *p : s->allocs) (void)hipFree(p);
    for (void *p : s->snap) if (p) (void)hipFree(p);
    for (void *p : s->rt_allocs) (void)hipFree(p);
    for (void *p : s->wb_allocs) (void)hipFree(p);
    rollout_free(s->fc); rollout_free(s->ck);
    acc_free(s->sum_acc); acc_free(s->diag_buf); acc_free(s->rt_acc); acc_free(s->ck_cnt); acc_free(s->wb_acc);
    if (s->fc_steps_host) (void)hipHostFree(s->fc_steps_host);
    if (s->fc_keep) (void)hipFree(s->fc_keep);
    if (s->rt_keep) (void)hipFree(s->rt_keep);
    groups_free(s);
    if (s->fc_ev_steps) (void)hipEventDestroy(s->fc_ev_steps);
    Work &w = s->ctx->w;
    for (int x = 0; x < 3; ++x) { w.K[x] = nullptr; w.St[x] = nullptr; }
    w.rowtot = w.rngtot = nullptr;
    w.TS = w.sp = w.gst = w.Vt = w.acur = w.rirc = w.CT = w.CG = w.Lpart0 = nullptr;
    delete s;
}

static const void *leap_fn(int ts_mode, int ntc, int nst) {
    if (nst == 1) return (const void *)k_leap<1, 6, 1, 6>;
#define LEAP_ROW(TSM_, NTC_) ((const void *)k_leap<TSM_, NTC_, 2>)
    if (ts_mode == 1) return ntc == 1 ? LEAP_ROW(1, 1) : ntc == 6 ? LEAP_ROW(1, 6) : LEAP_ROW(1, 12);
    return ntc == 1 ? LEAP_ROW(2, 1) : ntc == 6 ? LEAP_ROW(2, 6) : LEAP_ROW(2, 12);
#undef LEAP_ROW
}
static decltype(&k_se_chunk<1, 1>) se_chunk_fn(int ts_mode, int ntc) {
    if (ts_mode == 1) return ntc == 1 ? k_se_chunk<1, 1> : ntc == 6 ? k_se_chunk<1, 6> : k_se_chunk<1, 12>;
    return ntc == 1 ? k_se_chunk<2, 1> : ntc == 6 ? k_se_chunk<2, 6> : k_se_chunk<2, 12>;
}
static decltype(&k_hmc_final<1>) hmc_final_fn(int ntc) { return ntc == 1 ? k_hmc_final<1> : ntc == 6 ? k_hmc_final<6> : k_hmc_final<12>; }
static decltype(&k_hmc_chunk<0>) hmc_chunk_fn(int ntc) {
    return ntc == 1 ? k_hmc_chunk<1> : ntc == 6 ? k_hmc_chunk<6> : ntc == 12 ? k_hmc_chunk<12> : k_hmc_chunk<0>;
}
static decltype(&k_hmc_step<0, 1, 1>) hmc_step_fn(int stage, const Dims &d) {
    const int ht = (d.Tp + HB - 1) / HB, hm = (d.M + HB - 1) / HB;
#define HMC_STEP(S_) (ht <= 1 ? (hm <= 1 ? k_hmc_step<S_, 1, 1> : hm <= 2 ? k_hmc_step<S_, 1, 2> : k_hmc_step<S_, 1, 4>) \
                              : (hm <= 1 ? k_hmc_step<S_, 2, 1> : hm <= 2 ? k_hmc_step<S_, 2, 2> : k_hmc_step<S_, 2, 4>))
    return stage == 0 ? HMC_STEP(0) : stage == 1 ? HMC_STEP(1) : HMC_STEP(2);
#undef HMC_STEP
}
static decltype(&k_move_pair<6>) move_pair_fn(int nch) { return nch == 6 ? k_move_pair<6> : nch == 12 ? k_move_pair<12> : k_move_pair<16>; }
static decltype(&k_move_pairs<6>) move_pairs_fn(int nch) { return nch == 6 ? k_move_pairs<6> : nch == 12 ? k_move_pairs<12> : k_move_pairs<16>; }
static decltype(&k_move_pa2<6>) move_pa2_fn(int nch) { return nch == 6 ? k_move_pa2<6> : nch == 12 ? k_move_pa2<12> : k_move_pa2<16>; }

static void apply_launch_form(seir_sampler *s, int hmc_mode, int moves_mode) {
    s->hmc_mode = hmc_mode;
    s->moves_mode = moves_form(moves_mode, s->cfg.n_scans);
}

extern "C" int seir_sampler_create(seir_ctx *ctx, const seir_sampler_desc *ds, seir_sampler **out) {
    if (!ctx || !ds || !out) return fail(SEIR_ERR_INVALID, "null argument");
    *out = nullptr;
    const Dims &d = ctx->d;
    const int B = ds->num_chains;
    if (B < 1 || B > ctx->Bmax) return fail(SEIR_ERR_INVALID, "num_chains=%d outside [1, %d]", B, ctx->Bmax);
    if (ctx->w.K[0]) return fail(SEIR_ERR_STATE, "this context already has a sampler");
    if (d.Tp > 2 * HB || d.M > 4 * HB)
        return fail(SEIR_ERR_INVALID, "sampler supports T <= %d and M <= %d", 2 * HB, 4 * HB);
    if (ds->m < 1 || ds->m > MMAX) return fail(SEIR_ERR_INVALID, "m=%d outside [1, %d]", ds->m, MMAX);
    if (ds->dmax < 1 || ds->nmax < 0 || ds->occult_nmax < 0 || ds->num_event_time_updates < 0)
        return fail(SEIR_ERR_INVALID, "bad dmax/nmax/occult_nmax/num_event_time_updates");
    if (ds->t_range_lo < 0 || ds->t_range_hi > d.T || ds->t_range_lo >= ds->t_range_hi)
        return fail(SEIR_ERR_INVALID, "occult t_range [%d,%d) outside [0,%d)", ds->t_range_lo, ds->t_range_hi, d.T);
    if (ds->num_leapfrog_steps < 1) return fail(SEIR_ERR_INVALID, "num_leapfrog_steps must be >= 1");
    if (ds->trace_capacity < 1) return fail(SEIR_ERR_INVALID, "trace_capacity must be >= 1");
    if (ds->record_events < 0 || ds->record_events > 2) return fail(SEIR_ERR_INVALID, "record_events is 0, 1 or 2");
    if (ds->moves_mode < 0 || ds->moves_mode > 4 || ds->hmc_mode < 0 || ds->hmc_mode > 6)
        return fail(SEIR_ERR_INVALID, "moves_mode is 0..4, hmc_mode 0..6");
    if (ds->disable_mask < 0 || ds->disable_mask > 31) return fail(SEIR_ERR_INVALID, "disable_mask is a 5-bit mask");
    if (ds->leap_rows != 0 && ds->leap_rows != 24 && ds->leap_rows != 32) return fail(SEIR_ERR_INVALID, "leap_rows is 0 (auto), 24 or 32");
    if (ds->thin < 0) return fail(SEIR_ERR_INVALID, "thin must be >= 0 (0 or 1: every sweep is recorded)");
    HIP_TRY(hipSetDevice(ctx->device));
    seir_sampler *s = new (std::nothrow) seir_sampler();
    if (!s) return fail(SEIR_ERR_DEVICE, "out of host memory");
    s->ctx = ctx;
    SamplerCfg &c = s->cfg;
    c.B = B; c.dmax = ds->dmax; c.nmax = ds->nmax; c.mmax = ds->m; c.occult_nmax = ds->occult_nmax;
    c.n_scans = ds->num_event_time_updates; c.tr_lo = ds->t_range_lo; c.tr_hi = ds->t_range_hi;
    c.L = ds->num_leapfrog_steps;
    c.k0 = (uint32_t)(ds->seed & 0xffffffffu); c.k1 = (uint32_t)(ds->seed >> 32);
    c.chain0 = ds->first_chain_id;
    c.adapt_step = 0; c.adapt_mass = 0; c.n_adapt = 0; c.target_accept = 0.75;
    c.cap = ds->trace_capacity;
    c.nrb_d = (d.M + 7) / 8;
    s->record_events = ds->record_events;
    c.ev16 = ds->record_events == 2 ? 1 : 0;
    s->use_graph = ds->use_graph != 0;
    s->pair_debug = ds->debug_pair;
    s->leap_rows = ds->leap_rows;
    apply_launch_form(s, ds->hmc_mode, ds->moves_mode);
    c.disable_mask = ds->disable_mask;
    c.thin = s->thin_pending = ds->thin < 1 ? 1 : ds->thin;
    {
        int g = ds->chain_groups;
        if (g < 1) g = 1;
        if (g > B) g = B;
        s->ngroups = g;
        s->gstream.assign(g, nullptr); s->graph.assign(g, nullptr); s->gexec.assign(g, nullptr);
        s->ev_join.assign(g, nullptr);
    }

    int rc = 0;
    Work &w = ctx->w;
    const size_t cells = (size_t)ctx->Bmax * d.Mp * d.Tp;
    Chains &ch = s->ch;
#define S_STATE(ptr, n) S_ALLOC(allocs, ptr, (n), seir_sampler::R_STATE)
#define S_HAND(ptr, n) S_ALLOC(allocs, ptr, (n), seir_sampler::R_HANDOFF)
    for (int x = 0; x < 3; ++x) { S_STATE(w.K[x], cells); S_STATE(w.St[x], cells); }
    S_STATE(w.rowtot, (size_t)ctx->Bmax * 2 * d.Mp);
    S_STATE(w.rngtot, (size_t)ctx->Bmax * 2 * d.Mp);
    S_ALLOC(allocs, w.TS, (size_t)ctx->Bmax * d.nmt * d.ntc * 4);
    S_ALLOC(allocs, w.Lpart0, (size_t)ctx->Bmax * d.nmt * d.ntc);
    S_STATE(w.sp, (size_t)ctx->Bmax * 2 * d.Mp);
    S_STATE(w.gst, (size_t)ctx->Bmax * 2 * GST_N);
    S_STATE(w.Vt, (size_t)ctx->Bmax * d.Tp);
    S_STATE(w.acur, (size_t)ctx->Bmax * d.Tp);
    S_ALLOC(allocs, w.rirc, (size_t)ctx->Bmax * 2 * d.Tp);
    S_STATE(w.CT, (size_t)ctx->Bmax * 2 * CT_MAXC * 4);
    S_STATE(w.CG, (size_t)ctx->Bmax * 2 * CT_MAXC * 2);
    S_STATE(ch.q, (size_t)B * d.Pp); S_STATE(ch.p, (size_t)B * d.Pp); S_STATE(ch.q0, (size_t)B * d.Pp);
    S_STATE(ch.grad, (size_t)B * d.Pp); S_STATE(ch.var, (size_t)B * d.Pp);
    S_STATE(ch.rv_mean, (size_t)B * d.Pp); S_STATE(ch.rv_m2, (size_t)B * d.Pp);
    S_STATE(ch.hs, (size_t)B * NHS);
    S_HAND(ch.mv, (size_t)2 * B);
    S_HAND(ch.fpend, (size_t)B);
    S_HAND(ch.mvfix, (size_t)2 * B);
    S_HAND(ch.mvsel, (size_t)2 * B);
    S_HAND(ch.hand, (size_t)B);
    S_HAND(ch.late, (size_t)2 * B);
    ch.late_fatal = B;
    S_HAND(ch.tail, (size_t)B * TAIL_STRIDE + (size_t)B * TAIL_FLAG_STRIDE);
    S_HAND(ch.leap, (size_t)B * LEAP_CH);
    S_HAND(ch.llK, (size_t)B * 2 * (d.Mp / 16) * d.Tp);
    S_HAND(ch.llR, (size_t)B * 2 * d.ntc * d.Mp);
    S_HAND(ch.llP, (size_t)B * 2 * d.ntc * (d.Mp / 16));
    S_HAND(ch.llTS, (size_t)B * 2 * d.ntc * (d.Mp / 16) * 4);
    S_HAND(ch.llT, (size_t)B * ((size_t)d.Tp + 2 * (size_t)d.Mp + 8));
    S_HAND(ch.llmv, (size_t)2 * B * 32);
    S_HAND(ch.k0part, (size_t)B * ROLE_SLOTS);
    S_HAND(ch.irl0, (size_t)B);
    S_ALLOC(allocs, ch.leap_st, (size_t)(B + 2) * 16 * 8 + 4096);
    S_HAND(ch.done, (size_t)B * 2 * TAIL_STRIDE);
    S_HAND(ch.pbar, (size_t)B * PBAR_STRIDE);
    S_HAND(ch.finpart, (size_t)B * ROLE_SLOTS * 4);
    S_HAND(ch.hand2, (size_t)B);
    S_HAND(ch.mvs, (size_t)2 * B);
    S_HAND(ch.DownS, (size_t)2 * B * 2);
    S_HAND(ch.prev, (size_t)2 * B);
    S_HAND(ch.Dpart, (size_t)B * c.nrb_d * 2);
    S_HAND(ch.llD, (size_t)2 * B * c.nrb_d * 2);
    S_HAND(ch.Down, (size_t)2 * 2 * B * 2);
    S_STATE(ch.sweep, (size_t)B); S_STATE(ch.slot0, 1);
    S_ALLOC(allocs, ch.tr_theta, (size_t)c.cap * B * d.P);
    {
        char *tre = nullptr;
        S_ALLOC(allocs, tre, s->record_events ? (size_t)c.cap * B * d.M * d.T * 3 * (c.ev16 ? 2 : 4) : 4);
        ch.tr_events = tre;
    }
    S_ALLOC(allocs, ch.ev_overflow, 1);
    S_ALLOC(allocs, ch.tr_hmc, (size_t)c.cap * B * 3);
    S_ALLOC(allocs, ch.tr_mv, (size_t)c.cap * B * 4 * NMVTR);
    S_ALLOC(allocs, s->ev_stage, (size_t)B * d.M * d.T * 3);
#undef S_STATE
#undef S_HAND
    if (!rc) {
        const size_t Bm = (size_t)ctx->Bmax;
        auto st_ = [&](void *p_, size_t bytes_) { s->regions.push_back({p_, bytes_, seir_sampler::R_STATE}); };
        st_(w.F, cells * sizeof(double));
        st_(w.rowconst, Bm * d.Mp * sizeof(double));
        st_(w.ea, Bm * d.Tp * sizeof(double)); st_(w.eb, Bm * d.Mp * sizeof(double)); st_(w.rir, Bm * d.Tp * sizeof(double));
        st_(w.scal, Bm * NSCAL * sizeof(double)); st_(w.Qs, Bm * d.Mp * sizeof(double));
        st_(w.Kir, Bm * d.Tp * sizeof(double)); st_(w.Dir, Bm * d.Tp * sizeof(double));
        st_(w.constsum, Bm * sizeof(double));
    }
    if (!rc) {
        std::vector<double> ones((size_t)B * d.Pp, 1.0), hs((size_t)B * NHS, 0.0);
        for (int b = 0; b < B; ++b) hs[(size_t)b * NHS + HS_EPS] = 0.1;
        hipError_t e = hipMemcpy(ch.var, ones.data(), ones.size() * sizeof(double), hipMemcpyHostToDevice);
        if (e == hipSuccess) e = hipMemcpy(ch.hs, hs.data(), hs.size() * sizeof(double), hipMemcpyHostToDevice);
        if (e != hipSuccess) rc = fail(SEIR_ERR_DEVICE, "sampler init copy failed: %s", hipGetErrorString(e));
    }
    if (!rc) {
        hipError_t e = hipEventCreateWithFlags(&s->ev_fork, hipEventDisableTiming);
        if (e == hipSuccess) e = hipStreamCreateWithFlags(&s->copy_stream, hipStreamNonBlocking);
        if (e == hipSuccess) e = hipEventCreateWithFlags(&s->ev_burst, hipEventDisableTiming);
        if (e == hipSuccess) e = hipEventCreateWithFlags(&s->ev_copy, hipEventDisableTiming);
        for (int g = 0; g < s->ngroups && e == hipSuccess; ++g) {
            e = hipStreamCreateWithFlags(&s->gstream[g], hipStreamNonBlocking);
            if (e == hipSuccess) e = hipEventCreateWithFlags(&s->ev_join[g], hipEventDisableTiming);
        }
        if (e != hipSuccess) rc = fail(SEIR_ERR_DEVICE, "sampler stream setup failed: %s", hipGetErrorString(e));
    }
    if (!rc && (HMC_FORMS[ds->hmc_mode].roles || ds->moves_mode == 0 || ds->moves_mode == 2 || ds->moves_mode == 4)) {
        if (ctx->xcd_local < 0) ctx->xcd_local = probe_xcd_local(ctx->stream) ? 1 : 0;
        const bool ok = ctx->xcd_local == 1;
        s->xcd_local = ok;
    }
    if (!rc) {
        (void)hipDeviceGetAttribute(&s->cus, hipDeviceAttributeMultiprocessorCount, ctx->device);
        for (int nst = 1; nst <= 2; ++nst)
            if (hipOccupancyMaxActiveBlocksPerMultiprocessor(&s->leap_occ[nst - 1], leap_fn(chunk_ts_mode(d.Mp), d.ntc, nst), 256, 0) != hipSuccess)
                s->leap_occ[nst - 1] = 0;
        const int nch = move_nch(d.Tp);
        s->pairs_lds_attr = hipFuncSetAttribute((const void *)move_pairs_fn(nch), hipFuncAttributeMaxDynamicSharedMemorySize,
                                                (int)k_move_pairs_lds_bytes(d)) == hipSuccess;
        const size_t plds = k_move_pa2_lds_bytes(d);
        for (const void *fn : {(const void *)move_pair_fn(nch), (const void *)move_pa2_fn(nch)})
            if (plds > 64 * 1024) (void)hipFuncSetAttribute(fn, hipFuncAttributeMaxDynamicSharedMemorySize, (int)plds);
    }
    if (rc) { seir_sampler_destroy(s); return rc; }
    *out = s;
    return 0;
}

extern "C" int seir_sampler_xcd_local(seir_sampler *s) { return (s && s->xcd_local) ? 1 : 0; }

static int sampler_check(seir_sampler *s) {
    if (!s) return fail(SEIR_ERR_INVALID, "null sampler");
    HIP_TRY(hipSetDevice(s->ctx->device));
    return 0;
}

static int drain(seir_sampler *s) {
    HIP_TRY(hipStreamSynchronize(s->ctx->stream));
    if (s->copy_pending) { (void)hipEventSynchronize(s->ev_copy); s->copy_pending = false; }
    return 0;
}

static int reset_handoffs(seir_sampler *s) {
    hipStream_t st = s->ctx->stream;
    for (const auto &r : s->regions)
        if (r.kind == seir_sampler::R_HANDOFF) HIP_TRY(hipMemsetAsync(r.p, 0, r.bytes, st));
    s->leap_rsteps = s->leap_steps = 0;
    s->tail_count = 0;
    s->pbar_count = 0;
    s->poisoned = false;
    return 0;
}

extern "C" int seir_sampler_set_launch_form(seir_sampler *s, int32_t hmc_mode, int32_t moves_mode) {
    int rc = sampler_check(s);
    if (rc) return rc;
    if (moves_mode < 0 || moves_mode > 4 || hmc_mode < 0 || hmc_mode > 6)
        return fail(SEIR_ERR_INVALID, "moves_mode is 0..4, hmc_mode 0..6");
    if (hmc_mode != s->hmc_mode || moves_form(moves_mode, s->cfg.n_scans) != s->moves_mode) {
        HIP_TRY(hipStreamSynchronize(s->ctx->stream));
        drop_graph(s);
        apply_launch_form(s, hmc_mode, moves_mode);
    }
    return 0;
}

extern "C" int seir_sampler_launch_form(seir_sampler *s, int32_t *hmc_mode, int32_t *moves_mode) {
    if (!s) return fail(SEIR_ERR_INVALID, "null sampler");
    if (hmc_mode) *hmc_mode = s->hmc_mode;
    if (moves_mode) *moves_mode = s->moves_mode;
    return 0;
}

extern "C" int seir_sampler_debug_fail_handoff(seir_sampler *s, int32_t chain) {
    int rc = sampler_check(s);
    if (rc) return rc;
    if (chain < 0 || chain >= s->cfg.B) return fail(SEIR_ERR_INVALID, "chain %d outside [0, %d)", chain, s->cfg.B);
    static const uint32_t one = 1u;
    HIP_TRY(hipMemcpyAsync(s->ch.late + s->ch.late_fatal + chain, &one, sizeof(one), hipMemcpyHostToDevice, s->ctx->stream));
    return 0;
}

static size_t summary_cells(const seir_sampler *s) { return (size_t)s->cfg.B * s->ctx->d.M * s->ctx->d.T * seir::SUMMARY_Q; }
static size_t diag_words(const seir_sampler *s) { return 6 * summary_cells(s) + 3 * (size_t)s->cfg.B; }
static uint64_t *diag_mark(const seir_sampler *s, int which) {
    const size_t n = summary_cells(s), B = (size_t)s->cfg.B;
    return (uint64_t *)s->diag_buf.p + 2 * n + B + (size_t)which * (B + 2 * n);
}
static int moments_shadow(seir_sampler *s, int slot, bool save) {
    hipStream_t st = s->ctx->stream;
    int rc = 0;
    if (s->sum_on) {
        if (s->diag_on) rc = acc_shadow(s->diag_buf, slot, save, st);
        if (!rc) rc = acc_shadow(s->sum_acc, slot, save, st);
    }
    if (!rc && s->fc.on) rc = rollout_shadow(s->fc, slot, save, st);
    if (!rc && s->rt_on) {
        if (save) s->rt_snap_j[slot] = s->rt_j;
        else if (s->rt_acc.valid[slot]) s->rt_j = s->rt_snap_j[slot];
        rc = acc_shadow(s->rt_acc, slot, save, st);
    }
    if (!rc && s->ck.on) {
        rc = rollout_shadow(s->ck, slot, save, st);
        if (!rc) rc = acc_shadow(s->ck_cnt, slot, save, st);
    }
    if (!rc && s->wb_on) rc = acc_shadow(s->wb_acc, slot, save, st);
    return rc;
}

extern "C" int seir_sampler_snapshot(seir_sampler *s, int32_t slot) {
    int rc = sampler_check(s);
    if (rc) return rc;
    if (slot < 0 || slot > 1) return fail(SEIR_ERR_INVALID, "snapshot slot is 0 or 1");
    if (!s->have_state) return fail(SEIR_ERR_STATE, "no chain state set");
    if (s->poisoned) return fail(SEIR_ERR_STATE, "the sampler's state is unreliable (hand-off time-out): nothing to snapshot");
    if (!s->snap_bytes)
        for (const auto &r : s->regions)
            if (r.kind == seir_sampler::R_STATE) s->snap_bytes += (r.bytes + 255) / 256 * 256;
    if (!s->snap[slot]) HIP_TRY(hipMalloc(&s->snap[slot], s->snap_bytes));
    size_t off = 0;
    for (const auto &r : s->regions)
        if (r.kind == seir_sampler::R_STATE) {
            HIP_TRY(hipMemcpyAsync((char *)s->snap[slot] + off, r.p, r.bytes, hipMemcpyDeviceToDevice, s->ctx->stream));
            off += (r.bytes + 255) / 256 * 256;
        }
    s->snap_valid[slot] = true;
    return moments_shadow(s, slot, true);
}

extern "C" int seir_sampler_restore(seir_sampler *s, int32_t slot) {
    int rc = sampler_check(s);
    if (rc) return rc;
    if (slot < 0 || slot > 1) return fail(SEIR_ERR_INVALID, "snapshot slot is 0 or 1");
    if (!s->snap_valid[slot] || !s->snap[slot]) return fail(SEIR_ERR_STATE, "no snapshot in slot %d", slot);
    hipStream_t st = s->ctx->stream;
    if ((rc = drain(s))) return rc;
    size_t off = 0;
    for (const auto &r : s->regions)
        if (r.kind == seir_sampler::R_STATE) {
            HIP_TRY(hipMemcpyAsync(r.p, (const char *)s->snap[slot] + off, r.bytes, hipMemcpyDeviceToDevice, st));
            off += (r.bytes + 255) / 256 * 256;
        }
    if ((rc = reset_handoffs(s))) return rc;
    if ((rc = moments_shadow(s, slot, false))) return rc;
    s->vt_dirty = true;
    HIP_TRY(hipStreamSynchronize(st));
    return 0;
}

static void enqueue_refresh(seir_sampler *s) {
    seir_ctx *ctx = s->ctx;
    const Dims &d = ctx->d;
    const int B = s->cfg.B;
    launch_scan<1>(ctx, whole(ctx, B), nullptr);
    hipLaunchKernelGGL(k_range_totals, dim3((d.M + 3) / 4, B), dim3(256), 0, ctx->stream, d, ctx->w, s->cfg);
    launch_colreduce(ctx, whole(ctx, B));
    launch_gemm(ctx, whole(ctx, B));
    hipLaunchKernelGGL(k_chain_tables, dim3(B), dim3(256), 0, ctx->stream, d, ctx->c, ctx->w, s->ch);
    launch_se<1>(ctx, whole(ctx, B), false);
    hipLaunchKernelGGL(k_chain_refresh, dim3(B), dim3(256), (size_t)d.Tp * sizeof(double), ctx->stream, d, ctx->c,
                       ctx->w, s->ch);
}

extern "C" int seir_sampler_refresh(seir_sampler *s) {
    int rc = sampler_check(s);
    if (rc) return rc;
    if (!s->have_state) return fail(SEIR_ERR_STATE, "no chain state set");
    if (s->poisoned) {
        HIP_TRY(hipStreamSynchronize(s->ctx->stream));
        if ((rc = reset_handoffs(s))) return rc;
    }
    enqueue_refresh(s);
    HIP_TRY(hipGetLastError());
    return 0;
}

extern "C" int seir_sampler_set_state(seir_sampler *s, const double *u, const double *events) {
    int rc = sampler_check(s);
    if (rc) return rc;
    if (!u || !events) return fail(SEIR_ERR_INVALID, "null pointer");
    seir_ctx *ctx = s->ctx;
    const Dims &d = ctx->d;
    const int B = s->cfg.B;
    for (size_t i = 0, n = (size_t)B * d.M * d.T * 3; i < n; ++i)
        if (!(events[i] >= 0.0 && events[i] < 2147483648.0 && events[i] == std::floor(events[i])))
            return fail(SEIR_ERR_INVALID, "events[%zu]=%g is not a non-negative integer count", i, events[i]);
    HIP_TRY(hipMemcpyAsync(s->ch.q, u, sizeof(double) * B * d.P, hipMemcpyHostToDevice, ctx->stream));
    HIP_TRY(hipMemcpyAsync(s->ch.q0, u, sizeof(double) * B * d.P, hipMemcpyHostToDevice, ctx->stream));
    HIP_TRY(hipMemcpyAsync(s->ev_stage, events, sizeof(double) * B * d.M * d.T * 3, hipMemcpyHostToDevice,
                           ctx->stream));
    hipLaunchKernelGGL(k_import_events, dim3(1024), dim3(256), 0, ctx->stream, d, ctx->w, s->ev_stage, B);
    s->have_state = true;
    if (s->poisoned && (rc = reset_handoffs(s))) return rc;
    enqueue_refresh(s);
    HIP_TRY(hipGetLastError());
    HIP_TRY(hipStreamSynchronize(ctx->stream));
    return 0;
}

extern "C" int seir_sampler_get_state(seir_sampler *s, double *u, double *events, double *logp) {
    int rc = sampler_check(s);
    if (rc) return rc;
    if (!s->have_state) return fail(SEIR_ERR_STATE, "no chain state set");
    seir_ctx *ctx = s->ctx;
    const Dims &d = ctx->d;
    const int B = s->cfg.B;
    if (u) HIP_TRY(hipMemcpyAsync(u, s->ch.q, sizeof(double) * B * d.P, hipMemcpyDeviceToHost, ctx->stream));
    if (events) {
        hipLaunchKernelGGL(k_export_events, dim3(1024), dim3(256), 0, ctx->stream, d, ctx->w, s->ev_stage, B);
        HIP_TRY(hipMemcpyAsync(events, s->ev_stage, sizeof(double) * B * d.M * d.T * 3, hipMemcpyDeviceToHost,
                               ctx->stream));
    }
    std::vector<double> hs;
    if (logp) {
        hs.resize((size_t)B * NHS);
        HIP_TRY(hipMemcpyAsync(hs.data(), s->ch.hs, sizeof(double) * B * NHS, hipMemcpyDeviceToHost, ctx->stream));
    }
    HIP_TRY(hipStreamSynchronize(ctx->stream));
    if (logp)
        for (int b = 0; b < B; ++b) logp[b] = hs[(size_t)b * NHS + HS_LP_THETA] + hs[(size_t)b * NHS + HS_LP_CONST];
    return 0;
}

static int hs_update(seir_sampler *s, const std::vector<std::pair<int, const double *>> &cols) {
    const int B = s->cfg.B;
    std::vector<double> hs((size_t)B * NHS);
    HIP_TRY(hipStreamSynchronize(s->ctx->stream));
    HIP_TRY(hipMemcpy(hs.data(), s->ch.hs, sizeof(double) * B * NHS, hipMemcpyDeviceToHost));
    for (auto &c : cols)
        for (int b = 0; b < B; ++b) hs[(size_t)b * NHS + c.first] = c.second[b];
    HIP_TRY(hipMemcpy(s->ch.hs, hs.data(), sizeof(double) * B * NHS, hipMemcpyHostToDevice));
    return 0;
}

extern "C" int seir_sampler_set_kernel(seir_sampler *s, const double *step_size, const double *variance) {
    int rc = sampler_check(s);
    if (rc) return rc;
    const Dims &d = s->ctx->d;
    const int B = s->cfg.B;
    if (step_size) {
        for (int b = 0; b < B; ++b)
            if (!(step_size[b] > 0.0)) return fail(SEIR_ERR_INVALID, "step_size[%d] must be positive", b);
        if ((rc = hs_update(s, {{HS_EPS, step_size}}))) return rc;
    }
    HIP_TRY(hipStreamSynchronize(s->ctx->stream));
    if (variance) {
        for (size_t i = 0; i < (size_t)B * d.P; ++i)
            if (!(variance[i] > 0.0)) return fail(SEIR_ERR_INVALID, "variance[%zu] must be positive", i);
        HIP_TRY(hipMemcpy(s->ch.var, variance, sizeof(double) * B * d.P, hipMemcpyHostToDevice));
        s->vt_dirty = true;
    } else {
        std::vector<double> ones((size_t)B * d.P, 1.0);
        HIP_TRY(hipMemcpy(s->ch.var, ones.data(), sizeof(double) * B * d.P, hipMemcpyHostToDevice));
        s->vt_dirty = true;
    }
    return 0;
}

extern "C" int seir_sampler_get_kernel(seir_sampler *s, double *step_size, double *variance) {
    int rc = sampler_check(s);
    if (rc) return rc;
    const Dims &d = s->ctx->d;
    const int B = s->cfg.B;
    HIP_TRY(hipStreamSynchronize(s->ctx->stream));
    if (step_size) {
        std::vector<double> hs((size_t)B * NHS);
        HIP_TRY(hipMemcpy(hs.data(), s->ch.hs, sizeof(double) * B * NHS, hipMemcpyDeviceToHost));
        for (int b = 0; b < B; ++b) step_size[b] = hs[(size_t)b * NHS + HS_EPS];
    }
    if (variance) HIP_TRY(hipMemcpy(variance, s->ch.var, sizeof(double) * B * d.P, hipMemcpyDeviceToHost));
    return 0;
}

extern "C" int seir_sampler_set_adaptation(seir_sampler *s, int32_t adapt_step, int32_t adapt_mass, int32_t n_adapt,
                                           double target, const double *rv_count, const double *rv_mean,
                                           const double *rv_var) {
    int rc = sampler_check(s);
    if (rc) return rc;
    const Dims &d = s->ctx->d;
    const int B = s->cfg.B;
    if (adapt_mass && (!rv_count || !rv_mean || !rv_var))
        return fail(SEIR_ERR_INVALID, "adapt_mass needs the initial running variance");
    if (adapt_step && !(target > 0.0 && target < 1.0)) return fail(SEIR_ERR_INVALID, "target_accept_prob in (0,1)");
    HIP_TRY(hipStreamSynchronize(s->ctx->stream));
    std::vector<double> hs((size_t)B * NHS);
    HIP_TRY(hipMemcpy(hs.data(), s->ch.hs, sizeof(double) * B * NHS, hipMemcpyDeviceToHost));
    for (int b = 0; b < B; ++b) {
        double *h = hs.data() + (size_t)b * NHS;
        h[HS_DA_ERR] = 0.0; h[HS_DA_STEP] = 0.0; h[HS_DA_LOGAVG] = 0.0;
        h[HS_DA_MU] = std::log(10.0 * h[HS_EPS]);
        if (adapt_mass) h[HS_RV_N] = rv_count[b];
    }
    HIP_TRY(hipMemcpy(s->ch.hs, hs.data(), sizeof(double) * B * NHS, hipMemcpyHostToDevice));
    if (adapt_mass) {
        std::vector<double> m2((size_t)B * d.P);
        for (int b = 0; b < B; ++b)
            for (int i = 0; i < d.P; ++i) {
                const double v = rv_var[(size_t)b * d.P + i];
                if (!(v > 0.0)) return fail(SEIR_ERR_INVALID, "running variance must be positive");
                m2[(size_t)b * d.P + i] = v * rv_count[b];
            }
        HIP_TRY(hipMemcpy(s->ch.rv_mean, rv_mean, sizeof(double) * B * d.P, hipMemcpyHostToDevice));
        HIP_TRY(hipMemcpy(s->ch.rv_m2, m2.data(), sizeof(double) * B * d.P, hipMemcpyHostToDevice));
        HIP_TRY(hipMemcpy(s->ch.var, rv_var, sizeof(double) * B * d.P, hipMemcpyHostToDevice));
    }
    SamplerCfg &c = s->cfg;
    if (c.adapt_step != adapt_step || c.adapt_mass != adapt_mass || c.n_adapt != n_adapt ||
        c.target_accept != target)
        drop_graph(s);
    c.adapt_step = adapt_step; c.adapt_mass = adapt_mass; c.n_adapt = n_adapt; c.target_accept = target;
    s->vt_dirty = true;
    return 0;
}

static int drop_graph_for_thin(seir_sampler *s) {
    bool captured = false;
    for (auto g : s->gexec) captured = captured || g != nullptr;
    if (!captured) return 0;
    HIP_TRY(hipStreamSynchronize(s->ctx->stream));
    drop_graph(s);
    return 0;
}
static int apply_pending_thin(seir_sampler *s) {
    if (s->cfg.thin == s->thin_pending) return 0;
    int rc = drop_graph_for_thin(s);
    if (rc) return rc;
    s->cfg.thin = s->thin_pending;
    return 0;
}

extern "C" int seir_sampler_set_thin(seir_sampler *s, int32_t thin) {
    int rc = sampler_check(s);
    if (rc) return rc;
    if (thin < 0) return fail(SEIR_ERR_INVALID, "thin must be >= 0 (0 or 1: every sweep is recorded)");
    s->thin_pending = thin < 1 ? 1 : thin;
    return s->thin_pending != s->cfg.thin ? drop_graph_for_thin(s) : 0;
}

extern "C" int seir_sampler_thin(seir_sampler *s, int32_t *thin) {
    if (!s) return fail(SEIR_ERR_INVALID, "null sampler");
    if (thin) *thin = s->thin_pending;
    return 0;
}

extern "C" int seir_sampler_reset_trace(seir_sampler *s) {
    int rc = sampler_check(s);
// ... 32 lines not shown
    group_range(s, g, b0, nb);
    return {d.M, d.Mp, d.Tp, d.ntc, d.nmt, c.nrb_d,
            nb, c.L, c.n_scans, s->record_events,
            s->hmc_mode, s->moves_mode, s->leap_rows,
            s->xcd_local, s->ngroups == 1, s->use_graph, s->ctx->opt_affinity,
            s->cus, s->leap_occ[0], s->leap_occ[1], s->pairs_lds_attr};
}

static void enqueue_sweep(seir_sampler *s, int g) {
    seir_ctx *ctx = s->ctx;
    const SamplerCfg &c = s->cfg;
    const SweepPlan p = plan_sweep(sweep_inputs(s, g));
    int b0, nb;
    group_range(s, g, b0, nb);
    LaunchCfg l{ctx->d, s->gstream[g], nb, ctx->opt_affinity};
    l.d.b0 = b0;
    l.d.skew = ctx->opt_skew;
    const Dims d0 = l.d;
    hipStream_t st = l.st;
    const int ntile = d0.ntc * d0.nmt;
    const bool prof = s->prof_i >= 0 && (size_t)(2 * s->prof_i + 1) < s->prof_ev.size() && g == 0;
    auto prof_mark = [&](int end) {
        if (prof) (void)hipEventRecord(s->prof_ev[2 * s->prof_i + end], st);
        if (prof) s->prof_i += end;
    };
    auto vt = [&] {
        if (s->vt_dirty || c.adapt_mass) hipLaunchKernelGGL(k_vt, dim3(nb), dim3(WAVE), 0, st, l.d, ctx->w, s->ch);
        s->vt_dirty = false;
    };
    auto launch_leap = [&](int par0, int nsteps, int fold) {
        Dims df = l.d;
        df.aff_nb = p.leap_nbv;
        df.nlive = p.leap_nlive;
        df.sp_par = 0;
        df.chunked = p.ts_mode;
        df.nmt = p.leap_nmt;
        const dim3 gf((unsigned)((p.leap_wgs + p.per) * p.leap_nbv));
        const unsigned long long step_base = s->leap_steps, role_base = s->leap_rsteps;
        s->leap_steps += (unsigned long long)nsteps;
        s->leap_rsteps += (unsigned long long)(nsteps - (((fold & 2) && !(fold & 4)) ? 1 : 0));
        for (int sub = 0; sub < p.leap_launches; ++sub) {
            df.b0 = l.d.b0 + sub * p.leap_nbv;
            void *args[] = {(void *)&df, (void *)&ctx->c, (void *)&ctx->w, (void *)&c, (void *)&s->ch, (void *)&par0, (void *)&nsteps,
                            (void *)&step_base, (void *)&role_base, (void *)&fold};
            (void)hipLaunchKernel(leap_fn(p.ts_mode, d0.ntc, p.leap_nst), gf, dim3(256), args, 0, st);
        }
    };
    auto se_chunk_steps = [&](int it0, int it1, int par, bool ends) {
        Dims df = l.d;
        df.aff_nb = p.nbv;
        df.nlive = p.nlive;
        df.chunked = p.ts_mode;
        for (int it = it0; it <= it1; ++it) {
            const int traj = !ends ? 0 : it == 0 ? 1 : it == 1 ? 2 : it == c.L ? 3 : 0;
            df.sp_par = par;
            Work wf = ctx->w;
            if (it == 0) wf.Lpart = wf.Lpart0;
            s->tail_count += (unsigned long long)ntile;
            const unsigned long long target = s->tail_count;
            hipLaunchKernelGGL(se_chunk_fn(p.ts_mode, d0.ntc), dim3((unsigned)((ntile + p.per) * p.nbv)), dim3(256), 0, st, df, ctx->c, wf,
                               c, s->ch, par, target, traj);
            if (it < c.L) par ^= 1;
        }
        return par;
    };
    l.d.sp_par = 0;
    if (p.hmc == SweepPlan::FOLD) {
        vt();
        prof_mark(0);
        launch_leap(1, c.L + 1, p.end_in_leap ? 7 : 3);
        prof_mark(1);
        if (!p.end_in_leap) {
            l.d.sp_par = c.L & 1 ? 0 : 1;
            l.d.chunked = 0;
            l.d.nmt = p.leap_nmt;
            launch_hmc(ctx, l, c, s->ch, 2, 3);
            l.d.nmt = d0.nmt;
        }
    } else if (p.hmc == SweepPlan::TAILFOLD) {
        vt();
        int par = 1;
        if (p.ts_mode == 2) hipLaunchKernelGGL(k_sp_prep, dim3(nb), dim3(256), 0, st, l.d, ctx->w, s->ch, par);
        prof_mark(0);
        par = se_chunk_steps(0, c.L, par, true);
        Dims dz = l.d;
        dz.aff_nb = p.final_aff ? nb : 0;
        hipLaunchKernelGGL(hmc_final_fn(d0.ntc), p.final_aff ? dim3(p.per * nb) : dim3(p.per, nb), dim3(WAVE), 0, st, dz, ctx->c, ctx->w, c, s->ch, par);
        prof_mark(1);
    } else {
        l.d.chunked = 0;
        launch_se<1>(ctx, l, true);
        l.d.chunked = p.ts_mode;
        launch_hmc(ctx, l, c, s->ch, 0);
        s->vt_dirty = false;
        if (p.inner == SweepPlan::SINGLE) {
            for (int i = 1; i < c.L; ++i) {
                launch_se<1>(ctx, l, true);
                launch_hmc(ctx, l, c, s->ch, 1);
            }
        } else {
            int par = 0;
            prof_mark(0);
            if (p.inner == SweepPlan::LEAP) {
                launch_leap(par, c.L - 1, 0);
                par = (c.L - 1) & 1;
            } else if (p.inner == SweepPlan::SE_CHUNK) {
                par = se_chunk_steps(1, c.L - 1, par, false);
            } else {
                for (int i = 1; i < c.L; ++i) {
                    l.d.sp_par = par;
                    launch_se<1>(ctx, l, true);
                    Dims dc = l.d;
                    dc.aff_nb = p.chunk_aff ? nb : 0;
                    hipLaunchKernelGGL(hmc_chunk_fn(d0.ntc), p.chunk_aff ? dim3(p.per * nb) : dim3(p.per, nb), dim3(WAVE), 0, st, dc, ctx->c, ctx->w, c, s->ch, par);
                    par ^= 1;
                }
            }
            l.d.sp_par = par;
            prof_mark(1);
        }
        l.d.chunked = 0;
        launch_se<1>(ctx, l, true);
        launch_hmc(ctx, l, c, s->ch, 2, p.inner == SweepPlan::SINGLE ? 0 : 3);
    }
    Dims d = l.d;
    d.aff_nb = p.move_aff ? nb : 0;
    const dim3 gm = p.move_aff ? dim3(c.nrb_d * nb) : dim3(c.nrb_d, nb);
    const size_t plds = k_move_pa2_lds_bytes(d);
    int have_prev = 0, pbuf = 0;
    if (p.moves == SweepPlan::SPLIT_MOVES) {
        const auto pa2_fn = move_pa2_fn(p.nch);
        for (int scan = 0; scan < c.n_scans; ++scan)
            for (int slot = 0; slot < 4; ++slot) {
                const MoveSpec spec{slot >= 2 ? 1 : 0, slot & 1, slot, scan};
                hipLaunchKernelGGL(pa2_fn, gm, dim3(MVB), plds, st, d, ctx->c, ctx->w, c, s->ch, spec,
                                   have_prev, pbuf);
                pbuf ^= 1;
                hipLaunchKernelGGL((k_move_delta<true>), gm, dim3(DELTA_THREADS), 0, st, d, ctx->c, ctx->w, c, s->ch, pbuf, 0);
                have_prev = 1;
            }
        if (have_prev) {
            const MoveSpec none{-2, 0, 0, 0};
            hipLaunchKernelGGL(pa2_fn, gm, dim3(MVB), plds, st, d, ctx->c, ctx->w, c, s->ch, none, 1, pbuf);
        }
    } else {
        const int npairs = 2 * c.n_scans;
        const auto pair_fn = move_pair_fn(p.nch);
        Dims dp = d;
        dp.nlive = p.pair_nlive;
        SamplerCfg cp = c;
        if (p.nband) cp.nrb_d = p.nband;
        if (p.moves == SweepPlan::PAIRS) {
            hipLaunchKernelGGL(move_pairs_fn(p.nch), dim3((3 + p.nband) * p.nbk), dim3(MVB), k_move_pairs_lds_bytes(d), st, dp, ctx->c, ctx->w, cp,
                               s->ch, npairs, 1, p.nbk, s->pair_debug, p.nband, s->pbar_count, s->record_events ? 3 : 1);
            s->pbar_count += (unsigned)(npairs * 3);
        } else {
            int have_pre = 0;
            for (int scan = 0; scan < c.n_scans; ++scan)
                for (int half = 0; half < 2; ++half) {
                    const int pair = 2 * scan + half;
                    const MoveSpec se{half, 0, 2 * half, scan}, nx{half, 1, 2 * half + 1, scan};
                    const bool pre = p.pre && pair + 1 < npairs;
                    const int nh = (half + 1) & 1, nscan = scan + (half == 1 ? 1 : 0);
                    const MoveSpec se_next = pre ? MoveSpec{nh, 0, 2 * nh, nscan} : MoveSpec{-1, 0, 0, 0};
                    hipLaunchKernelGGL(pair_fn, dim3(((pre ? 3 : 2) + p.nband) * p.nbk), dim3(MVB), plds, st, dp, ctx->c, ctx->w, cp,
                                       s->ch, se, nx, se_next, have_prev, have_pre, pbuf, p.nbk, pair, s->pair_debug, p.nband);
                    have_pre = pre ? 1 : 0;
                    pbuf ^= 1;
                    if (!p.nband)
                        hipLaunchKernelGGL((k_move_delta<false>), gm, dim3(DELTA_THREADS), 0, st, d, ctx->c, ctx->w, c, s->ch, pbuf, 1);
                    have_prev = 1;
                }
            if (have_prev) {
                const MoveSpec none{-1, 0, 0, 0}, close{-2, 0, 0, 0};
                hipLaunchKernelGGL(pair_fn, dim3(nb), dim3(MVB), plds, st, d, ctx->c, ctx->w, cp, s->ch, none, close, none, 1,
                                   0, pbuf, nb, 62, 0, 0);
                if (p.fpend == SweepPlan::F_APPLY) hipLaunchKernelGGL(k_apply_fpend, gm, dim3(256), 0, st, d, ctx->c, ctx->w, c, s->ch);
            }
        }
    }
    d.aff_nb = 0;
    if (p.record)
        hipLaunchKernelGGL(k_record, dim3((d.M + 3) / 4, nb), dim3(256), 0, st, d, ctx->c, ctx->w, c, s->ch, p.advance ? 0 : 1,
                           p.fpend == SweepPlan::F_RECORD ? 1 : 0);
    if (p.advance) hipLaunchKernelGGL(k_advance, dim3((nb + 63) / 64), dim3(64), 0, st, s->ch, b0, nb);
}

static int check_handoffs(seir_sampler *s);
extern "C" int seir_sampler_run(seir_sampler *s, int32_t n) {
    int rc = sampler_check(s);
    if (rc) return rc;
    if (!s->have_state) return fail(SEIR_ERR_STATE, "no chain state set");
    if (n < 0) return fail(SEIR_ERR_INVALID, "num_sweeps must be >= 0");
    if (s->poisoned) return check_handoffs(s);
    hipStream_t main_st = s->ctx->stream;
    HIP_TRY(hipEventRecord(s->ev_fork, main_st));
    for (int g = 0; g < s->ngroups; ++g) {
        hipStream_t st = s->gstream[g];
        HIP_TRY(hipStreamWaitEvent(st, s->ev_fork, 0));
        if (s->use_graph && (s->graph_skew != s->ctx->opt_skew || s->graph_aff != s->ctx->opt_affinity)) {
            drop_graph(s);
            s->graph_skew = s->ctx->opt_skew; s->graph_aff = s->ctx->opt_affinity;
        }
        if (s->use_graph && !s->gexec[g]) {
            HIP_TRY(hipStreamBeginCapture(st, hipStreamCaptureModeThreadLocal));
            enqueue_sweep(s, g);
            HIP_TRY(hipStreamEndCapture(st, &s->graph[g]));
            HIP_TRY(hipGraphInstantiate(&s->gexec[g], s->graph[g], nullptr, nullptr, 0));
        }
    }
    for (int i = 0; i < n; ++i)
        for (int g = 0; g < s->ngroups; ++g) {
            if (s->use_graph) HIP_TRY(hipGraphLaunch(s->gexec[g], s->gstream[g]));
            else enqueue_sweep(s, g);
        }
    for (int g = 0; g < s->ngroups; ++g) {
        HIP_TRY(hipEventRecord(s->ev_join[g], s->gstream[g]));
        HIP_TRY(hipStreamWaitEvent(main_st, s->ev_join[g], 0));
    }
    HIP_TRY(hipGetLastError());
    return 0;
}

static int check_handoffs(seir_sampler *s) {
    if ((s->pair_debug & 15) != 0) return 0;
    if (!s->poisoned) {
        std::vector<uint32_t> late((size_t)s->cfg.B, 0u);
        uint32_t *fatal = s->ch.late + s->ch.late_fatal;
        HIP_TRY(hipMemcpy(late.data(), fatal, sizeof(uint32_t) * late.size(), hipMemcpyDeviceToHost));
        for (size_t b = 0; b < late.size(); ++b)
            if (late[b]) { s->poisoned = true; s->poison_chain = (int)b; s->poison_count = late[b]; break; }
    }
    if (s->poisoned)
        return fail(SEIR_ERR_HANDOFF, "chain %d: %u in-launch hand-off(s) timed out -- the persistent launches could not get all "
                    "their workgroups on the GPU at once (another sampler or process holds part of it?).  Draws since the last "
                    "check are unreliable and the sampler refuses to go on until seir_sampler_restore / _set_state / _refresh; "
                    "hmc_mode 3 + moves_mode 4 (seir_sampler_set_launch_form) are the launch forms for a shared GPU",
                    s->poison_chain, s->poison_count);
    return 0;
}

static int check_ev_overflow(seir_sampler *s) {
    int rc = check_handoffs(s);
    if (rc) return rc;
    if (!s->cfg.ev16) return 0;
    unsigned flag = 0;
    HIP_TRY(hipMemcpy(&flag, s->ch.ev_overflow, sizeof(flag), hipMemcpyDeviceToHost));
    if (flag) return fail(SEIR_ERR_STATE, "an event count exceeded 65535: record_events=2 (uint16 trace) cannot hold this chain");
    return 0;
}

static int need_events(const seir_sampler *s, const char *verb) {
    if (s->record_events) return 0;
    if (!verb) return fail(SEIR_ERR_STATE, "sampler was created with record_events=0");
    return fail(SEIR_ERR_STATE, "sampler was created with record_events=0: there are no recorded events to %s", verb);
}

template <typename F>
static int on_copy_stream(seir_sampler *s, F fn) {
    HIP_TRY(hipEventRecord(s->ev_burst, s->ctx->stream));
    HIP_TRY(hipStreamWaitEvent(s->copy_stream, s->ev_burst, 0));
    if (int rc = fn(s->copy_stream)) return rc;
    HIP_TRY(hipEventRecord(s->ev_copy, s->copy_stream));
    s->copy_pending = true;
    return 0;
}

static int read_trace_check(seir_sampler *s, int32_t first, int32_t count, const void *events) {
    if (first < 0 || count < 0 || first + count > s->cfg.cap)
        return fail(SEIR_ERR_INVALID, "trace range [%d,%d) outside capacity %d", first, first + count, s->cfg.cap);
    return events ? need_events(s, nullptr) : 0;
}

static int copy_trace(seir_sampler *s, hipStream_t st, int32_t first, int32_t count, double *theta, void *events, double *hmc,
                      double *moves) {
    const Dims &d = s->ctx->d;
    const SamplerCfg &c = s->cfg;
    const size_t B = c.B;
    if (theta)
        HIP_TRY(hipMemcpyAsync(theta, s->ch.tr_theta + (size_t)first * B * d.P, sizeof(double) * count * B * d.P,
                               hipMemcpyDeviceToHost, st));
    if (events)
        HIP_TRY(hipMemcpyAsync(events, (const char *)s->ch.tr_events + (size_t)first * B * d.M * d.T * 3 * (c.ev16 ? 2 : 4),
                               (size_t)(c.ev16 ? 2 : 4) * count * B * d.M * d.T * 3, hipMemcpyDeviceToHost, st));
    if (hmc)
        HIP_TRY(hipMemcpyAsync(hmc, s->ch.tr_hmc + (size_t)first * B * 3, sizeof(double) * count * B * 3,
                               hipMemcpyDeviceToHost, st));
    if (moves)
        HIP_TRY(hipMemcpyAsync(moves, s->ch.tr_mv + (size_t)first * B * 4 * NMVTR,
                               sizeof(double) * count * B * 4 * NMVTR, hipMemcpyDeviceToHost, st));
    return 0;
}

extern "C" int seir_sampler_read_trace(seir_sampler *s, int32_t first, int32_t count, double *theta,
                                       void *events, double *hmc, double *moves) {
    int rc = sampler_check(s);
    if (rc) return rc;
    if ((rc = read_trace_check(s, first, count, events))) return rc;
    if ((rc = copy_trace(s, s->ctx->stream, first, count, theta, events, hmc, moves))) return rc;
    HIP_TRY(hipStreamSynchronize(s->ctx->stream));
    return check_ev_overflow(s);
}

extern "C" int seir_sampler_read_trace_async(seir_sampler *s, int32_t first, int32_t count, double *theta,
                                             void *events, double *hmc, double *moves) {
    int rc = sampler_check(s);
    if (rc) return rc;
    if ((rc = read_trace_check(s, first, count, events))) return rc;
    return on_copy_stream(s, [&](hipStream_t st) { return copy_trace(s, st, first, count, theta, events, hmc, moves); });
}

extern "C" int seir_sampler_trace_wait(seir_sampler *s) {
    int rc = sampler_check(s);
    if (rc) return rc;
    if (s->copy_pending) {
        HIP_TRY(hipEventSynchronize(s->ev_copy));
        s->copy_pending = false;
        return check_ev_overflow(s);
    }
    return 0;
}

struct TraceUser { const char *verb, *not_enabled, *name, *done; };
static const TraceUser SUMMARY_USER = {"summarise", "summaries are not enabled: call seir_sampler_summary_reset first"};
static const TraceUser RT_USER = {"form the reproduction number from",
                                   "the reproduction number is not enabled: call seir_sampler_rt_reset first"};
static const TraceUser WB_USER = {"form the within/between pressure shares from",
                                   "the within/between pressure shares are not enabled: call seir_sampler_wb_reset first"};
static const TraceUser FORECAST_USER = {"forecast from", "the forecast is not enabled: call seir_sampler_forecast_reset first",
                                         "forecast", "forecast"};
static const TraceUser CHECK_USER = {"check", "the in-sample check is not enabled: call seir_sampler_check_reset first", "check",
                                      "checked"};

static int trace_range_check(seir_sampler *s, bool enabled, const TraceUser &what, int32_t first = 0, int32_t count = 0) {
    if (int rc = need_events(s, what.verb)) return rc;
    if (!enabled) return fail(SEIR_ERR_STATE, "%s", what.not_enabled);
    if (first < 0 || count < 0 || (long long)first + count > s->cfg.cap)
        return fail(SEIR_ERR_INVALID, "trace range [%d,%lld) outside capacity %d", first, (long long)first + count, s->cfg.cap);
    return 0;
}

static int copy_marginals(seir_sampler *s, hipStream_t st, int32_t first, int32_t count, const MomentBufs &m, size_t E,
                          int64_t *by_day, int64_t *by_loc, int64_t *state_by_day) {
    const size_t B = s->cfg.B, f = (size_t)first, n = (size_t)count, M = (size_t)s->ctx->d.M;
    if (by_day) HIP_TRY(hipMemcpyAsync(by_day, m.by_day + f * B * E * 3, sizeof(int64_t) * n * B * E * 3, hipMemcpyDeviceToHost, st));
    if (by_loc) HIP_TRY(hipMemcpyAsync(by_loc, m.by_loc + f * B * M * 3, sizeof(int64_t) * n * B * M * 3, hipMemcpyDeviceToHost, st));
    if (state_by_day)
        HIP_TRY(hipMemcpyAsync(state_by_day, m.state_by_day + f * B * E * 3, sizeof(int64_t) * n * B * E * 3, hipMemcpyDeviceToHost, st));
// ... 1284 lines not shown
    if (async) return on_copy_stream(s, [&](hipStream_t st) { return copy_group_curves(s, st, c, first, count, dst); });
    if ((rc = copy_group_curves(s, s->ctx->stream, c, first, count, dst))) return rc;
    HIP_TRY(hipStreamSynchronize(s->ctx->stream));
    return check_ev_overflow(s);
}

extern "C" int seir_sampler_read_group_rt(seir_sampler *s, int32_t first, int32_t count, double *Rg) {
    return read_group_curves(s, true, false, first, count, Rg, nullptr);
}
extern "C" int seir_sampler_read_group_rt_async(seir_sampler *s, int32_t first, int32_t count, double *Rg) {
    return read_group_curves(s, true, true, first, count, Rg, nullptr);
}
extern "C" int seir_sampler_read_group_wb(seir_sampler *s, int32_t first, int32_t count, double *Wg, double *Bg) {
    return read_group_curves(s, false, false, first, count, Wg, Bg);
}
extern "C" int seir_sampler_read_group_wb_async(seir_sampler *s, int32_t first, int32_t count, double *Wg, double *Bg) {
    return read_group_curves(s, false, true, first, count, Wg, Bg);
}

static void gcurve_wsums_launch(const Dims &d, hipStream_t st, const int *offsets, const int *members, const double *weights,
                                const double *v, int G, int L, long long ld, long long v_d0, long long out_d0, long long nd,
                                double *out);

extern "C" int seir_group_wsums(seir_ctx *ctx, const double *v, int64_t nd, int32_t L, int32_t M, int32_t G, const int32_t *offsets,
                                const int32_t *members, const double *weights, double *out) {
    int rc = check_batch(ctx, 1);
    if (rc) return rc;
    if (!v || !out) return fail(SEIR_ERR_INVALID, "null pointer");
    if (nd < 1 || M < 1 || L < 1 || nd > 0x7fffffffll)
        return fail(SEIR_ERR_INVALID, "nd=%lld, M=%d, L=%d: at least one of each, nd below 2^31", (long long)nd, M, L);
    std::vector<int> seg;
    if ((rc = groups_parse(G, offsets, members, M, seg))) return rc;
    const size_t nin = (size_t)nd * L * M, nout = (size_t)nd * G * L, nnz = (size_t)offsets[G];
    DevBuf dv, dout, doff, dmem, dw;
    if ((rc = dv.alloc(sizeof(double) * nin)) || (rc = dout.alloc(sizeof(double) * nout)) ||
        (rc = doff.alloc(sizeof(int) * (size_t)(G + 1))) || (rc = dmem.alloc(sizeof(int) * nnz)) ||
        (weights && (rc = dw.alloc(sizeof(double) * nnz))))
        return rc;
    hipStream_t st = ctx->stream;
    HIP_TRY(hipMemcpyAsync(dv.p, v, sizeof(double) * nin, hipMemcpyHostToDevice, st));
    HIP_TRY(hipMemcpyAsync(doff.p, offsets, sizeof(int) * (size_t)(G + 1), hipMemcpyHostToDevice, st));
    HIP_TRY(hipMemcpyAsync(dmem.p, members, sizeof(int) * nnz, hipMemcpyHostToDevice, st));
    if (weights) HIP_TRY(hipMemcpyAsync(dw.p, weights, sizeof(double) * nnz, hipMemcpyHostToDevice, st));
    gcurve_wsums_launch(whole(ctx, 1).d, st, doff.as<int>(), dmem.as<int>(), dw.as<double>(), dv.as<double>(), G, L, M, 0, 0, nd,
                        dout.as<double>());
    HIP_TRY(hipGetLastError());
    HIP_TRY(hipMemcpyAsync(out, dout.p, sizeof(double) * nout, hipMemcpyDeviceToHost, st));
    HIP_TRY(hipStreamSynchronize(st));
    return 0;
}

extern "C" int seir_host_alloc(void **p, uint64_t bytes) {
    if (!p) return fail(SEIR_ERR_INVALID, "null pointer");
    HIP_TRY(hipHostMalloc(p, bytes ? bytes : 8, hipHostMallocDefault));
    return 0;
}
extern "C" int seir_host_free(void *p) {
    HIP_TRY(hipHostFree(p));
    return 0;
}

extern "C" int seir_sampler_time_grad_kernel(seir_sampler *s, int32_t iters, float *mean_ms) {
    int rc = sampler_check(s);
    if (rc) return rc;
    if (!s->have_state) return fail(SEIR_ERR_STATE, "no chain state set");
    if (!mean_ms || iters < 1) return fail(SEIR_ERR_INVALID, "bad iters/mean_ms");
    seir_ctx *ctx = s->ctx;
    LaunchCfg l = whole(ctx, s->cfg.B);
    l.d.chunked = plan_sweep(sweep_inputs(s, 0)).ts_mode;
    launch_se<1>(ctx, l, true);
    HIP_TRY(hipEventRecord(ctx->ev0, ctx->stream));
    for (int i = 0; i < iters; ++i) launch_se<1>(ctx, l, true);
    HIP_TRY(hipEventRecord(ctx->ev1, ctx->stream));
    HIP_TRY(hipEventSynchronize(ctx->ev1));
    float ms = 0.f;
    HIP_TRY(hipEventElapsedTime(&ms, ctx->ev0, ctx->ev1));
    HIP_TRY(hipGetLastError());
    *mean_ms = ms / iters;
    return 0;
}

extern "C" int seir_sampler_time_leapfrog(seir_sampler *s, int32_t sweeps, float *mean_ms, int32_t *launches, int32_t *evals) {
    int rc = sampler_check(s);
    if (rc) return rc;
    if (!s->have_state) return fail(SEIR_ERR_STATE, "no chain state set");
    if (!mean_ms || sweeps < 1 || sweeps > 4096) return fail(SEIR_ERR_INVALID, "bad sweeps/mean_ms");
    if (s->use_graph || s->ngroups != 1) return fail(SEIR_ERR_STATE, "timing of the leapfrog section needs stream launches on one stream");
    while (s->prof_ev.size() < (size_t)2 * sweeps) {
        hipEvent_t e;
        HIP_TRY(hipEventCreate(&e));
        s->prof_ev.push_back(e);
    }
    s->prof_i = 0;
    rc = seir_sampler_run(s, sweeps);
    const int recorded = s->prof_i;
    s->prof_i = -1;
    if (rc) return rc;
    HIP_TRY(hipStreamSynchronize(s->ctx->stream));
    if (recorded < 1) return fail(SEIR_ERR_STATE, "this sampler's sweep has no chunked leapfrog section (hmc_mode 1 or fewer than 3 leapfrog steps)");
    double sum = 0.0;
    for (int i = 0; i < recorded; ++i) {
        float ms = 0.f;
        HIP_TRY(hipEventElapsedTime(&ms, s->prof_ev[2 * i], s->prof_ev[2 * i + 1]));
        sum += ms;
    }
    *mean_ms = (float)(sum / recorded);
    const SweepPlan p = plan_sweep(sweep_inputs(s, 0));
    if (launches) *launches = p.section_launches;
    if (evals) *evals = p.section_evals;
    return 0;
}

#ifdef SE_STAMPS
extern "C" int seir_debug_read_ts(seir_ctx *ctx, double *out, int64_t n) {
    HIP_TRY(hipStreamSynchronize(ctx->stream));
    HIP_TRY(hipMemcpy(out, ctx->w.TS, sizeof(double) * n, hipMemcpyDeviceToHost));
    return 0;
}
#endif

#if defined(LEAP_STAMPS) || defined(PAIR_STAMPS)
extern "C" int seir_debug_leap_stamps(seir_sampler *s, unsigned long long *out, int reset) {
    HIP_TRY(hipStreamSynchronize(s->ctx->stream));
    const size_t n = (size_t)(s->cfg.B + 2) * 16 * 8 + 4096;
    HIP_TRY(hipMemcpy(out, s->ch.leap_st, n * 8, hipMemcpyDeviceToHost));
    if (reset) {
        std::vector<unsigned long long> h(n);
        for (size_t i = 0; i < n; ++i) h[i] = (i & 1) ? 0ull : ~0ull;
        HIP_TRY(hipMemcpy(s->ch.leap_st, h.data(), n * 8, hipMemcpyHostToDevice));
    }
    return 0;
}
#endif

#ifdef TAIL_STAMPS
extern "C" int seir_debug_tail_stamps(seir_sampler *s, unsigned long long *out, int reset) {
    HIP_TRY(hipStreamSynchronize(s->ctx->stream));
    const int B = s->cfg.B;
    std::vector<unsigned long long> h((size_t)B * TAIL_STRIDE);
    HIP_TRY(hipMemcpy(h.data(), s->ch.tail, h.size() * 8, hipMemcpyDeviceToHost));
    for (int b = 0; b < B; ++b)
        for (int k = 0; k < 8; ++k) out[b * 8 + k] = h[(size_t)b * TAIL_STRIDE + 8 + k];
    if (reset) {
        for (int b = 0; b < B; ++b) {
            unsigned long long *p = h.data() + (size_t)b * TAIL_STRIDE + 8;
            p[0] = p[2] = p[5] = ~0ull; p[1] = p[3] = p[4] = 0;
        }
        HIP_TRY(hipMemcpy(s->ch.tail, h.data(), h.size() * 8, hipMemcpyHostToDevice));
    }
    return 0;
}
#endif

extern "C" int seir_sampler_pair_timeouts(seir_sampler *s, uint32_t *out) {
    int rc = sampler_check(s);
    if (rc) return rc;
    if (!out) return fail(SEIR_ERR_INVALID, "null pointer");
    HIP_TRY(hipStreamSynchronize(s->ctx->stream));
    std::vector<uint32_t> both((size_t)2 * s->cfg.B, 0u);
    HIP_TRY(hipMemcpy(both.data(), s->ch.late, sizeof(uint32_t) * both.size(), hipMemcpyDeviceToHost));
    for (int b = 0; b < s->cfg.B; ++b) out[b] = both[b] + both[(size_t)s->cfg.B + b];
    return 0;
}

#ifdef SEIR_STAMPS
extern "C" int seir_sampler_debug_hs(seir_sampler *s, double *out) {
    HIP_TRY(hipStreamSynchronize(s->ctx->stream));
    HIP_TRY(hipMemcpy(out, s->ch.hs, sizeof(double) * s->cfg.B * NHS, hipMemcpyDeviceToHost));
    return 0;
}
#endif

static void groups_launch(const Dims &d, hipStream_t st, const GroupTable &gt, bool ev16, const void *ev, int M, int L,
                          long long ev_d0, long long out_d0, long long nd, int64_t *out, const int *St0, long long plane, int ndp,
                          int64_t *state0) {
    const int nchunk = (L + 63) / 64;
    for (long long off = 0; off < nd; off += GRP_NDMAX) {
        const dim3 grid((unsigned)(gt.nseg * nchunk), (unsigned)std::min<long long>(GRP_NDMAX, nd - off)), block(64 * GRP_WAVES);
        hipLaunchKernelGGL(ev16 ? k_group_sums<1> : k_group_sums<0>, grid, block, 0, st, d, gt, ev, M, L, nchunk, ev_d0 + off,
                           out_d0 + off, (unsigned long long *)out, St0, plane, ndp, (unsigned long long *)state0);
    }
}

#include "group_curve_kernels.h"

static void gcurve_wsums_launch(const Dims &d, hipStream_t st, const int *offsets, const int *members, const double *weights,
                                const double *v, int G, int L, long long ld, long long v_d0, long long out_d0, long long nd,
                                double *out) {
    const int nchunk = (L + GC_WAVES - 1) / GC_WAVES;
    for (long long off = 0; off < nd; off += GRP_NDMAX) {
        const dim3 grid((unsigned)(G * nchunk), (unsigned)std::min<long long>(GRP_NDMAX, nd - off)), block(64 * GC_WAVES);
        hipLaunchKernelGGL(weights ? k_group_wsums<1> : k_group_wsums<0>, grid, block, 0, st, d, offsets, members, weights, v, G, L,
                           ld, nchunk, v_d0 + off, out_d0 + off, out);
    }
}

static void gcurve_sums(seir_sampler *s, const LaunchCfg &l, const GroupCurve &c, int D, int slot0, int nj) {
    const int B = s->cfg.B;
    for (int x = 0; x < c.planes; ++x)
        gcurve_wsums_launch(l.d, l.st, c.offsets, s->grp.members, c.weights, c.cells[x], s->grp.G, D, l.d.Mp, 0,
                            (long long)slot0 * B, (long long)nj * B, c.out[x]);
}

static void gcurve_rt_trace_cells(seir_sampler *s, const LaunchCfg &l, int slot0, int nj) {
    const RtBufs &rb = s->rt;
    const int B = s->cfg.B;
    hipLaunchKernelGGL(k_rt_trace_cells<RT_DT>, dim3(rb.ncb, (rb.D + RT_DT - 1) / RT_DT, B), dim3(256),
                       k_rt_trace_lds_bytes<RT_DT>(l.d.Mp), l.st, l.d, s->ctx->c, rb, (const double *)s->ch.tr_theta, B, slot0, nj,
                       s->grt.cells[0], (long long)l.d.Mp);
}

static void gcurve_rt_gather(seir_sampler *s, const LaunchCfg &l, long long pos0, int nj) {
    const int B = s->cfg.B, D = s->rt.D;
    hipLaunchKernelGGL(k_rt_cells_from_keep, dim3((l.d.M + 255) / 256, D, B), dim3(256), 0, l.st, l.d, (const double *)s->rt_keep,
                       s->rt_keep_stride, pos0, B, D, nj, s->grt.cells[0], (long long)l.d.Mp);
}

static void gcurve_wb_trace_cells(seir_sampler *s, const LaunchCfg &l, int slot0, int nj) {
    const WbBufs &wb = s->wb;
    const int B = s->cfg.B;
    hipLaunchKernelGGL(k_wb_trace_cells<WB_DT>, dim3(wb.ncb, (wb.D + WB_DT - 1) / WB_DT, B), dim3(256),
                       k_wb_trace_lds_bytes<WB_DT>(l.d.Mp), l.st, l.d, s->ctx->c, wb, (const double *)s->ch.tr_theta, B, slot0, nj,
                       s->gwb.cells[0], s->gwb.cells[1], (long long)l.d.Mp);
}

static void gcurve_lds_attributes(int Mp) {
    const size_t rl = k_rt_trace_lds_bytes<RT_DT>(Mp), wl = k_wb_trace_lds_bytes<WB_DT>(Mp);
    if (rl > 64 * 1024)
        (void)hipFuncSetAttribute((const void *)k_rt_trace_cells<RT_DT>, hipFuncAttributeMaxDynamicSharedMemorySize, (int)rl);
    if (wl > 64 * 1024)
        (void)hipFuncSetAttribute((const void *)k_wb_trace_cells<WB_DT>, hipFuncAttributeMaxDynamicSharedMemorySize, (int)wl);
}
```

covid19uk_amd/csrc/sweep_plan.h:

```cpp
#pragma once

namespace seir {

namespace plan {
constexpr int WAVE = 64;
constexpr int CT_MAXC = 16;
constexpr int ROLE_SLOTS = 64;
}

inline bool xcd_affinity_applies(int per, int nb) {
    return (nb == 1 || nb == 2 || nb == 4 || (nb > 0 && nb % 8 == 0)) && ((long long)per * nb) % 8 == 0;
}

inline int moves_form(int moves_mode, int n_scans) { return n_scans > 30 ? 1 : moves_mode; }
inline int chunk_ts_mode(int Mp) { return Mp <= 512 ? 1 : 2; }
inline int move_nch(int Tp) { return Tp <= 6 * plan::WAVE ? 6 : Tp <= 12 * plan::WAVE ? 12 : 16; }

struct HmcForm { bool chunked, roles, leap, fold, end, tailfold; };
constexpr HmcForm HMC_FORMS[7] = {
    {true,  true,  true,  true,  true,  true},
    {false, false, false, false, false, false},
    {true,  false, false, false, false, false},
    {true,  true,  false, false, false, false},
    {true,  true,  true,  false, false, false},
    {true,  true,  true,  true,  false, false},
    {true,  true,  false, false, false, true},
};

struct SweepInputs {
    int M, Mp, Tp, ntc, nmt, nrb_d;
    int nb, L, n_scans, record_events;
    int hmc_mode, moves_mode, leap_rows;
    bool xcd_local;
    bool one_group, use_graph;
    int affinity;
    int cus;
    int leap_occ24, leap_occ32;
    bool pairs_lds;
};

struct SweepPlan {
    enum { FOLD, TAILFOLD, STAGE };
    enum { SINGLE, LEAP, SE_CHUNK, SPLIT };
    enum { PAIRS, PAIR, SPLIT_MOVES };
    enum { F_NONE, F_PAIRS, F_RECORD, F_APPLY };
    int hmc, inner, ts_mode, per, nbv, nlive;
    bool end_in_leap, chunk_aff, final_aff;
    int leap_nst, leap_nmt, leap_wgs, leap_nbv, leap_nlive, leap_launches;
    int section_launches, section_evals;
    int moves, nband, nbk, pair_nlive, nch, fpend;
    bool pre, move_aff, record, advance;
};

inline SweepPlan plan_sweep(const SweepInputs &in) {
    SweepPlan p{};
    const HmcForm f = HMC_FORMS[in.hmc_mode];
    const bool chunked = f.chunked && in.L >= 3 && in.ntc <= plan::CT_MAXC;
    p.ts_mode = chunked ? chunk_ts_mode(in.Mp) : 0;
    p.per = in.ntc + in.Mp / plan::WAVE;
    const int ntile = in.ntc * in.nmt;
    p.nbv = (in.nb + 7) / 8 * 8;
    p.nlive = p.nbv != in.nb ? in.nb : 0;
    const bool roles = chunked && f.roles && in.xcd_local && in.one_group && (in.affinity & 1) && !in.use_graph &&
                       (in.ntc == 1 || in.ntc == 6 || in.ntc == 12) && xcd_affinity_applies(ntile, p.nbv) &&
                       p.per <= plan::ROLE_SLOTS;
    p.leap_nst = 2; p.leap_nmt = in.nmt; p.leap_wgs = ntile / 2; p.leap_nbv = p.nbv;
    bool leap = false;
    if (roles && f.leap && in.nmt <= plan::WAVE && in.nmt % 2 == 0) {
        const int nmt24 = in.Mp / 24, wgs24 = in.ntc * nmt24;
        auto fit = [&](int nbv) {
            if (in.leap_rows != 32 && p.ts_mode == 1 && in.ntc == 6 && in.Mp % 24 == 0 && xcd_affinity_applies(wgs24, nbv) &&
                (long long)(wgs24 + p.per) * nbv <= (long long)in.leap_occ24 * in.cus) {
                p.leap_nst = 1; p.leap_nmt = nmt24; p.leap_wgs = wgs24;
                return true;
            }
            return in.leap_rows != 24 && (long long)(ntile / 2 + p.per) * nbv <= (long long)in.leap_occ32 * in.cus;
        };
        leap = fit(p.nbv);
        if (!leap && in.nb == 16 && fit(8)) { leap = true; p.leap_nbv = 8; }
    }
    p.leap_nlive = p.leap_nbv == p.nbv ? p.nlive : 0;
    p.leap_launches = p.nbv / p.leap_nbv;
    p.hmc = leap && f.fold ? SweepPlan::FOLD : roles && f.tailfold ? SweepPlan::TAILFOLD : SweepPlan::STAGE;
    p.end_in_leap = p.hmc == SweepPlan::FOLD && f.end;
    p.inner = !chunked ? SweepPlan::SINGLE : leap ? SweepPlan::LEAP : roles ? SweepPlan::SE_CHUNK : SweepPlan::SPLIT;
    p.chunk_aff = (in.affinity & 1) && xcd_affinity_applies(p.per, in.nb);
    p.final_aff = xcd_affinity_applies(p.per, in.nb);
    p.section_evals = p.hmc != SweepPlan::STAGE ? in.L + 1 : chunked ? in.L - 1 : 0;
    p.section_launches = p.hmc == SweepPlan::FOLD ? p.leap_launches : p.hmc == SweepPlan::TAILFOLD ? in.L + 2
                       : !chunked ? 0 : leap ? 1 : roles ? in.L - 1 : 2 * (in.L - 1);
    const int moves = moves_form(in.moves_mode, in.n_scans);
    p.move_aff = (in.affinity & 2) && xcd_affinity_applies(in.nrb_d, in.nb);
    p.nch = move_nch(in.Tp);
    p.nbk = in.nb;
    if (moves == 1) {
        p.moves = SweepPlan::SPLIT_MOVES;
    } else {
        int nband = (in.M + 15) / 16;
        if ((3 + nband) * p.nbv > in.cus && (3 + (in.M + 31) / 32) * p.nbv <= in.cus) nband = (in.M + 31) / 32;
        if (moves != 3 && in.xcd_local && in.one_group && !in.use_graph && (3 + nband) * p.nbv <= in.cus) {
            p.nband = nband;
            p.nbk = p.nbv;
            p.pair_nlive = p.nlive;
        }
        p.pre = moves == 0 || moves == 3 || moves == 4;
        const bool pairs = p.nband > 0 && moves == 0 && in.n_scans > 0 && in.pairs_lds;
        p.moves = pairs ? SweepPlan::PAIRS : SweepPlan::PAIR;
        p.fpend = pairs ? SweepPlan::F_PAIRS : in.n_scans == 0 ? SweepPlan::F_NONE
                : in.record_events ? SweepPlan::F_RECORD : SweepPlan::F_APPLY;
    }
    p.record = in.record_events && p.moves != SweepPlan::PAIRS;
    p.advance = in.n_scans == 0;
    return p;
}

}
```

covid19uk_amd/sampler.py:

```python
from __future__ import annotations

import ctypes
import dataclasses
import sys

import numpy as np

from . import _lib
from .posterior.diagnostics import Diagnostics
from .seir import SeirModel, _dptr

MOVE_KEYS = ("move/S->E", "move/E->I", "occult/S->E", "occult/E->I")
MOVES_MODES = {"paired": 0, "split": 1, "paired-nopre": 2, "paired-delta": 3, "paired-launch": 4}
HMC_MODES = {"chunk": 0, "single": 1, "chunk-split": 2, "chunk-launch": 3, "chunk-leap": 4, "chunk-stage": 5,
             "chunk-launch-fold": 6}
FALLBACK_FORMS = (("chunk-launch", "paired-launch"), ("chunk-split", "paired-delta"))


@dataclasses.dataclass
class Trace:
    theta: np.ndarray
    events: np.ndarray
    hmc: dict
    moves: dict
    marginals: dict = None
    forecast: dict = None
    rt: np.ndarray = None
    check: dict = None
    wb: dict = None
    groups: dict = None
    group_curves: dict = None


MARGINAL_KEYS = ("events_by_day", "events_by_location", "state_by_day")
FORECAST_KEYS = ("forecast_by_day", "forecast_by_location", "forecast_state_by_day")
FORECAST_QUANTILE_PLANES = ("cases", "cum_cases", "prevalence")
CHECK_KEYS = ("check_by_day", "check_by_location", "check_state_by_day")
WB_KEYS = ("within_pressure", "between_pressure")
GROUP_SOURCES = {"trace": (0, "seir_by_group", None), "forecast": (1, "forecast_by_group", "forecast_group_state0"),
                 "check": (2, "check_by_group", "check_group_state0")}
GROUP_KEYS = tuple(k for _, ev, st in GROUP_SOURCES.values() for k in (ev, st) if k)
GROUP_CURVE_KEYS = ("rt_by_group", "within_by_group", "between_by_group")
SUMMARY_QUANTITIES = ("k_se", "k_ei", "k_ir", "S", "E", "I")


@dataclasses.dataclass
class Summary:
    count: np.ndarray
    ref: np.ndarray
    sum: np.ndarray
    sumsq: np.ndarray

    @property
    def mean(self) -> np.ndarray:
        return summary_mean(self.count, self.ref, self.sum)

    @property
    def var(self) -> np.ndarray:
        return summary_var(self.count, self.sum, self.sumsq)


@dataclasses.dataclass
class RtSummary:
    count: np.ndarray
    ref: np.ndarray
    sum: np.ndarray
    sumsq: np.ndarray
    gt1: np.ndarray

    @property
    def mean(self) -> np.ndarray:
        return summary_mean(self.count, self.ref, self.sum)

    @property
    def var(self) -> np.ndarray:
        return summary_var(self.count, self.sum, self.sumsq)

    @property
    def prob_gt1(self) -> np.ndarray:
        return rt_prob_gt1(self.count, self.gt1)


@dataclasses.dataclass
class WbSummary:
    count: np.ndarray
    defined: np.ndarray
    ref_w: np.ndarray
    sum_w: np.ndarray
    sumsq_w: np.ndarray
    ref_b: np.ndarray
    sum_b: np.ndarray
    gt: np.ndarray

    @property
    def within_mean(self) -> np.ndarray:
        return wb_mean(self.defined, self.ref_w, self.sum_w)

    @property
    def within_var(self) -> np.ndarray:
        return summary_var(self.defined, self.sum_w, self.sumsq_w)

    @property
    def between_mean(self) -> np.ndarray:
        return wb_mean(self.defined, self.ref_b, self.sum_b)

    @property
    def p_within_gt_between(self) -> np.ndarray:
        return wb_mean(self.defined, 0.0, self.gt)


def wb_mean(defined, ref, sum_):
    n = np.asarray(defined, np.float64)
    ok = n > 0
    return np.where(ok, np.asarray(ref, np.float64) + np.asarray(sum_, np.float64) / np.where(ok, n, 1.0), np.nan)


@dataclasses.dataclass
class CheckSummary:
    moments: Summary
    observed: np.ndarray
    lt: np.ndarray
    eq: np.ndarray
    location_lt: np.ndarray
    location_eq: np.ndarray
    day_lt: np.ndarray
    day_eq: np.ndarray
    total_lt: np.ndarray
    total_eq: np.ndarray

    @property
    def count(self) -> np.ndarray:
        return self.moments.count

    @property
    def pit(self) -> np.ndarray:
        return mid_p(self.count, self.lt, self.eq)

    @property
    def location_pit(self) -> np.ndarray:
        return mid_p(self.count, self.location_lt, self.location_eq)

    @property
    def day_pit(self) -> np.ndarray:
        return mid_p(self.count, self.day_lt, self.day_eq)

    @property
    def total_pit(self) -> np.ndarray:
        return mid_p(self.count, self.total_lt, self.total_eq)


def mid_p(count, lt, eq):
    n = _per_chain(count, lt)
    num = 2.0 * np.asarray(lt, np.float64) + np.asarray(eq, np.float64)
    ok = n > 0
    return np.where(ok, num / np.where(ok, 2.0 * n, 1.0), np.nan)


def rt_prob_gt1(count, gt1):
    n = _per_chain(count, gt1)
    with np.errstate(divide="ignore", invalid="ignore"):
        return np.where(n > 0, np.asarray(gt1, np.float64) / n, np.nan)


def forecast_draw_id(global_chain_id: int, j: int) -> int:
    c, j = int(global_chain_id), int(j)
    if not 0 <= c < _lib.FORECAST_MAX_CHAIN:
# ... 737 lines not shown
        do_sum, accumulate = self._summarize_mode(summarize)
        burst, num_bursts = int(burst), int(num_bursts)
        if 2 * burst > self.cap:
            raise ValueError(f"sample_bursts needs trace_capacity >= 2 * burst = {2 * burst}, have {self.cap}")
        do_fc = bool(forecast)
        do_rt = bool(rt)
        do_ck = bool(check)
        do_wb = bool(within_between)
        grp_src = self._group_sources(groups, do_sum, do_fc, do_ck)
        grp_lens = {k: self._group_len(k) for k in grp_src}
        gc_days = self._group_curve_days(do_rt, do_wb)
        key = (burst, bool(events), do_sum, self._forecast_H if do_fc else 0) + ((self._rt_D,) if do_rt else ()) + \
            ((("check", self._check_K),) if do_ck else ()) + ((("wb", self._wb_D),) if do_wb else ()) + \
            ((("groups", self._groups_G, tuple(grp_lens.items())),) if grp_src else ()) + \
            ((("group_curves", self._groups_G, tuple(gc_days.items())),) if gc_days else ())
        if getattr(self, "_pinned_key", None) != key:
            for bf in getattr(self, "_pinned", []):
                bf.close()
            mk = dict(marginals=True) if do_sum else {}
            if do_fc:
                mk["forecast"] = self._forecast_H
            if do_rt:
                mk["rt"] = self._rt_D
            if do_ck:
                mk["check"] = self._check_K
            if do_wb:
                mk["wb"] = self._wb_D
            if grp_src:
                mk["groups"] = (self._groups_G, grp_lens)
            if gc_days:
                mk["group_curves"] = (self._groups_G, gc_days)
            self._pinned = [PinnedTrace(self, burst, events, **mk), PinnedTrace(self, burst, events, **mk)]
            self._pinned_key = key
        bufs = self._pinned
        futs = [None, None]
        i, prev, retried = 0, -1, -1
        try:
            with ThreadPoolExecutor(max_workers=1) as pool:
                while i < num_bursts or prev >= 0:
                    try:
                        h = i & 1
                        if i < num_bursts:
                            if futs[h] is not None:
                                futs[h].result()
                                futs[h] = None
                            if self.auto_recover:
                                self.snapshot(h)
                            self.reset_trace(at=h * burst)
                            self.run(burst * self._thin)
                            if do_sum:
                                self.summarize(h * burst, burst, accumulate)
                            if marks and i in marks:
                                self.mark(marks[i])
                            if do_fc:
                                self._forecast_burst(h * burst, burst, forecast)
                            if do_rt:
                                self._rt_burst(h * burst, burst)
                            if do_ck:
                                self._check_burst(h * burst, burst)
                            if do_wb:
                                self._wb_burst(h * burst, burst)
                        if prev >= 0:
                            self.trace_wait()
                            futs[prev & 1] = pool.submit(consume, self.trace_view(bufs[prev & 1], burst), prev)
                            prev = -1
                            self._burst_ok()
                        if i < num_bursts:
                            self.read_trace_async(burst, h * burst, bufs[h])
                            if do_sum:
                                self.read_marginals_async(burst, h * burst, bufs[h])
                            if do_fc:
                                self.read_forecast_marginals_async(burst, h * burst, bufs[h])
                            if do_rt:
                                self.read_rt_draws_async(burst, h * burst, bufs[h])
                            if do_ck:
                                self.read_check_marginals_async(burst, h * burst, bufs[h])
                            if do_wb:
                                self.read_wb_draws_async(burst, h * burst, bufs[h])
                            for src in grp_src:
                                self.read_group_marginals_async(src, burst, h * burst, bufs[h])
                            if gc_days:
                                self._read_group_curves(gc_days, burst, h * burst, bufs[h])
                            prev = i
                            i += 1
                    except _lib.HandoffTimeout as e:
                        bad = prev if prev >= 0 else i
                        if not self.auto_recover or bad >= num_bursts:
                            raise
                        if bad == retried and self._fallback_level >= len(FALLBACK_FORMS):
                            raise
                        retried = bad
                        self._recover(bad & 1, e)
                        i, prev = bad, -1
                for f in futs:
                    if f is not None:
                        f.result()
        finally:
            try:
                self.trace_wait()
            except _lib.HandoffTimeout:
                pass

    def sample(self, num_sweeps: int, events: bool = True, summarize=False, forecast=False, rt=False, check=False,
               within_between=False, groups=False) -> Trace:
        do_sum, accumulate = self._summarize_mode(summarize)
        grp_src = self._group_sources(groups, do_sum, bool(forecast), bool(check))
        gc_days = self._group_curve_days(bool(rt), bool(within_between))
        if num_sweeps > self.cap:
            raise ValueError(f"num_sweeps={num_sweeps} exceeds trace_capacity={self.cap}")
        while True:
            if self.auto_recover:
                self.snapshot(0)
            self.reset_trace()
            self.run(num_sweeps * self._thin)
            try:
                if do_sum:
                    self.summarize(0, num_sweeps, accumulate)
                if forecast:
                    self._forecast_burst(0, num_sweeps, forecast)
                if rt:
                    self._rt_burst(0, num_sweeps)
                if check:
                    self._check_burst(0, num_sweeps)
                if within_between:
                    self._wb_burst(0, num_sweeps)
                tr = self.read_trace(num_sweeps, events=events)
                if do_sum:
                    tr.marginals = self.read_marginals(num_sweeps)
                if forecast:
                    tr.forecast = self.read_forecast_marginals(num_sweeps)
                if rt:
                    tr.rt = self.read_rt_draws(num_sweeps)
                if check:
                    tr.check = self.read_check_marginals(num_sweeps)
                if within_between:
                    tr.wb = self.read_wb_draws(num_sweeps)
                if grp_src:
                    tr.groups = {}
                    for src in grp_src:
                        tr.groups.update(self.read_group_marginals(src, num_sweeps))
                if gc_days:
                    tr.group_curves = self._read_group_curves(gc_days, num_sweeps)
            except _lib.HandoffTimeout as e:
                if not self.auto_recover:
                    raise
                self._recover(0, e)
                continue
            self._burst_ok()
            return tr

    def xcd_local(self) -> bool:
        return bool(self._lib.seir_sampler_xcd_local(self._s))

    def pair_timeouts(self) -> np.ndarray:
        out = np.zeros(self.B, dtype=np.uint32)
        _lib.check(self._lib.seir_sampler_pair_timeouts(self._s, out.ctypes.data_as(ctypes.POINTER(ctypes.c_uint32))))
        return out

    def time_leapfrog(self, sweeps: int = 50):
        ms_, nl, ne = ctypes.c_float(), ctypes.c_int32(), ctypes.c_int32()
        _lib.check(self._lib.seir_sampler_time_leapfrog(self._s, int(sweeps), ctypes.byref(ms_), ctypes.byref(nl), ctypes.byref(ne)))
        return float(ms_.value), int(nl.value), int(ne.value)

    def time_grad_kernel(self, iters: int = 100) -> float:
        ms_ = ctypes.c_float()
        _lib.check(self._lib.seir_sampler_time_grad_kernel(self._s, int(iters), ctypes.byref(ms_)))
        return float(ms_.value)
```

include/seir_hip.h:

```cpp
#ifndef SEIR_HIP_H
#define SEIR_HIP_H

#include <stdint.h>

#ifdef __cplusplus
extern "C" {
#endif

#define SEIR_ABI_VERSION 4

typedef enum {
    SEIR_OK = 0,
    SEIR_ERR_INVALID = -1,
    SEIR_ERR_DEVICE = -2,
    SEIR_ERR_STATE = -3,
    SEIR_ERR_HANDOFF = -4
} seir_status;

typedef struct seir_ctx seir_ctx;
typedef struct seir_sampler seir_sampler;

typedef struct {
    int32_t M;
    int32_t T;
    int32_t max_chains;
    int32_t device;
    const double *Cstar;
    const double *N;
    const double *W;
    const double *weekday_c;
    const double *log_area_c;
    const double *car_Q;
    double car_half_logdet;
    const double *init_state;
    double nu;
    double time_delta;
    double rate_floor;
} seir_desc;

int seir_abi_version(void);
const char *seir_last_error(void);

#define SEIR_MAX_M 2048
#define SEIR_MAX_T 1088

int seir_create(const seir_desc *desc, seir_ctx **out);
void seir_destroy(seir_ctx *ctx);
int seir_num_params(const seir_ctx *ctx);

int seir_set_initial_state(seir_ctx *ctx, const double *init_state);

int seir_log_prob(seir_ctx *ctx, int32_t B, const double *u, const double *events,
                  double *logp );

int seir_log_prob_grad(seir_ctx *ctx, int32_t B, const double *u, const double *events,
                       double *logp , double *grad );

int seir_log_prob_dev(seir_ctx *ctx, int32_t B, const double *u_dev, const double *events_dev,
                      double *logp_dev, double *grad_dev);

int seir_prepare_events_dev(seir_ctx *ctx, int32_t B, const double *events_dev);
int seir_eval_prepared_dev(seir_ctx *ctx, int32_t B, const double *u_dev,
                           double *logp_dev, double *grad_dev);

int seir_sync(seir_ctx *ctx);
void *seir_stream(seir_ctx *ctx);

enum { SEIR_OPT_DEBUG_SKEW = 0, SEIR_OPT_XCD_AFFINITY = 1, SEIR_OPT_GEMM_F32 = 2, SEIR_OPT_EVAL_FORM = 3,
       SEIR_OPT_RT_STAGING_KIB = 4 };
int seir_set_option(seir_ctx *ctx, int32_t option, int32_t value);

int seir_malloc(void **dev_ptr, uint64_t bytes);
int seir_free(void *dev_ptr);
int seir_memcpy_h2d(void *dst_dev, const void *src_host, uint64_t bytes);
int seir_memcpy_d2h(void *dst_host, const void *src_dev, uint64_t bytes);

int seir_timer_start(seir_ctx *ctx);
int seir_timer_stop(seir_ctx *ctx, float *ms);

enum { SEIR_K_SCAN = 0, SEIR_K_GEMM = 1, SEIR_K_SE_VALUE = 2, SEIR_K_SE_GRAD = 3,
       SEIR_K_FINISH = 4,
       SEIR_K_STATE = 5, SEIR_K_TILES_VALUE = 6, SEIR_K_TILES_GRAD = 7, SEIR_K_FINISH_FUSED = 8 };
int seir_time_kernel(seir_ctx *ctx, int32_t which, int32_t B, int32_t iters, float *mean_ms);

int seir_selftest_math(seir_ctx *ctx, int32_t n, const double *x, double *L, double *inv, double *lfact);
int seir_selftest_math_wide(seir_ctx *ctx, int32_t n, const double *x, double *L, double *inv);

enum { SEIR_FN_FAST_LOG = 0, SEIR_FN_FAST_RCP = 1, SEIR_FN_MV_LOG = 2, SEIR_FN_SOFTPLUS_TAB = 3,
       SEIR_FN_SOFTPLUS_SIGMOID_TAB = 4, SEIR_FN_SOFTPLUS = 5, SEIR_FN_LFACT_BF = 6, SEIR_FN_LBINOM_TAB = 7,
       SEIR_FN_LBINOM_CONST = 8, SEIR_FN_LBINOM_BF = 9, SEIR_FN_LOG1MEXP_TAB = 10, SEIR_FN_LOG1MEXP = 11,
       SEIR_FN_LOG1MEXP_SERIES = 12, SEIR_FN_L1ME_INV_SERIES = 13, SEIR_FN_L1ME_INV_K = 14,
       SEIR_FN_L1ME_INV_SERIES_K = 15, SEIR_FN_LOG1MEXP_DIFF_SLOW = 16, SEIR_FN_FAST_LOG_K = 17, SEIR_FN_COUNT = 18 };
int seir_selftest_fn(seir_ctx *ctx, int32_t op, int32_t n, const double *x, const double *y, double *out0, double *out1);

enum { SEIR_DELTA_BAND = 0, SEIR_DELTA_OWN_EI = 1, SEIR_DELTA_OWN_SE = 2 };
int seir_selftest_band_delta(seir_ctx *ctx, int32_t op, int32_t n, const double *S, const double *I, const double *K0,
                             const double *F, const double *dF, const double *ee, const double *psiW, double rate_floor,
                             double dt, double *out);

enum { SEIR_WAVE_SUM = 0, SEIR_WAVE_MIN = 1, SEIR_WAVE_INCL_SCAN = 2, SEIR_WAVE_INCL_SUFFIX_SCAN = 3,
       SEIR_BLOCK_EXCL_SCAN = 4, SEIR_BLOCK_INCL_SUFFIX_SCAN = 5, SEIR_BLOCK_SUM = 6 };
int seir_selftest_wave(seir_ctx *ctx, int32_t op, int32_t is_int, int32_t nblocks, const void *in, void *out, void *total);


#define SEIR_MMAX 4
#define SEIR_MOVE_TRACE (2 + 4 * SEIR_MMAX)

typedef struct {
    int32_t num_chains;
    int32_t dmax, nmax, m;
    int32_t occult_nmax;
    int32_t num_event_time_updates;
    int32_t t_range_lo, t_range_hi;
    int32_t num_leapfrog_steps;
    int32_t trace_capacity;
    int32_t first_chain_id;
    int32_t record_events;
    uint64_t seed;
    int32_t moves_mode;
    int32_t hmc_mode;
    int32_t use_graph;
    int32_t chain_groups;
    int32_t disable_mask;
    int32_t debug_pair;
    int32_t leap_rows;
    int32_t thin;
} seir_sampler_desc;

int seir_sampler_create(seir_ctx *ctx, const seir_sampler_desc *desc, seir_sampler **out);
void seir_sampler_destroy(seir_sampler *s);

int seir_sampler_set_state(seir_sampler *s, const double *u, const double *events);
int seir_sampler_get_state(seir_sampler *s, double *u, double *events, double *logp );

int seir_sampler_set_kernel(seir_sampler *s, const double *step_size , const double *variance );
int seir_sampler_get_kernel(seir_sampler *s, double *step_size, double *variance);

int seir_sampler_set_adaptation(seir_sampler *s, int32_t adapt_step_size, int32_t adapt_mass,
                                int32_t num_adaptation_steps, double target_accept_prob,
                                const double *rv_count, const double *rv_mean, const double *rv_variance);

int seir_sampler_refresh(seir_sampler *s);

int seir_sampler_reset_trace(seir_sampler *s);
int seir_sampler_reset_trace_at(seir_sampler *s, int32_t first_slot);
int seir_sampler_set_thin(seir_sampler *s, int32_t thin);
int seir_sampler_thin(seir_sampler *s, int32_t *thin);
int seir_sampler_run(seir_sampler *s, int32_t num_sweeps);
int seir_sampler_read_trace(seir_sampler *s, int32_t first, int32_t count, double *theta, void *events,
                            double *hmc, double *moves);

int seir_sampler_read_trace_async(seir_sampler *s, int32_t first, int32_t count, double *theta, void *events,
                                  double *hmc, double *moves);
int seir_sampler_trace_wait(seir_sampler *s);
int seir_host_alloc(void **host_ptr, uint64_t bytes);
int seir_host_free(void *host_ptr);

int seir_sampler_time_grad_kernel(seir_sampler *s, int32_t iters, float *mean_ms);

int seir_sampler_xcd_local(seir_sampler *s);

int seir_sampler_pair_timeouts(seir_sampler *s, uint32_t *out);

int seir_sampler_time_leapfrog(seir_sampler *s, int32_t sweeps, float *mean_ms, int32_t *launches, int32_t *evals);

int seir_sampler_snapshot(seir_sampler *s, int32_t slot );
int seir_sampler_restore(seir_sampler *s, int32_t slot);
int seir_sampler_set_launch_form(seir_sampler *s, int32_t hmc_mode, int32_t moves_mode);
int seir_sampler_launch_form(seir_sampler *s, int32_t *hmc_mode, int32_t *moves_mode);
int seir_sampler_debug_fail_handoff(seir_sampler *s, int32_t chain);

int seir_sampler_summary_reset(seir_sampler *s);
int seir_sampler_summarize(seir_sampler *s, int32_t first_slot, int32_t count, int32_t accumulate);
int seir_sampler_read_marginals(seir_sampler *s, int32_t first, int32_t count,
                                int64_t *events_by_day, int64_t *events_by_location, int64_t *state_by_day);
int seir_sampler_read_marginals_async(seir_sampler *s, int32_t first, int32_t count,
                                      int64_t *events_by_day, int64_t *events_by_location, int64_t *state_by_day);
int seir_sampler_read_summary(seir_sampler *s, uint64_t *count, int32_t *ref, int64_t *sum, uint64_t *sumsq);

int seir_sampler_diag_reset(seir_sampler *s, int32_t batch_len);
int seir_sampler_diag_mark(seir_sampler *s, int32_t which);
int seir_sampler_read_diag(seir_sampler *s, uint64_t *nbatch, int64_t *bsum, uint64_t *bsumsq);
int seir_sampler_read_diag_mark(seir_sampler *s, int32_t which, uint64_t *count, int64_t *sum, uint64_t *sumsq);

#define SEIR_FORECAST_MAX_H 128
int seir_sampler_forecast_reset(seir_sampler *s, int32_t horizon, const double *W, const double *weekday_c, uint64_t seed);
int seir_sampler_forecast(seir_sampler *s, int32_t first_slot, int32_t count, const double *log_baseline_steps);
int seir_sampler_read_forecast_marginals(seir_sampler *s, int32_t first, int32_t count, int64_t *forecast_by_day,
                                         int64_t *forecast_by_location, int64_t *forecast_state_by_day);
int seir_sampler_read_forecast_marginals_async(seir_sampler *s, int32_t first, int32_t count, int64_t *forecast_by_day,
                                               int64_t *forecast_by_location, int64_t *forecast_state_by_day);
int seir_sampler_read_forecast(seir_sampler *s, uint64_t *count, int32_t *ref, int64_t *sum, uint64_t *sumsq);

#define SEIR_ORDER_STATS_MAX_RANKS 16
int seir_sampler_forecast_keep(seir_sampler *s, int64_t cap);
int seir_sampler_forecast_order_stats(seir_sampler *s, const int64_t *ranks, int32_t R, int32_t pooled, int32_t *out);
int seir_order_stats(seir_ctx *ctx, const int32_t *values, int64_t cells, int32_t segs, int64_t seg_len, int64_t seg_stride,
                     int64_t cell_stride, const int64_t *ranks, int32_t R, int32_t *out);

int seir_sampler_rt_reset(seir_sampler *s, int32_t days, const double *weight);
int seir_sampler_rt(seir_sampler *s, int32_t first_slot, int32_t count);
int seir_sampler_read_rt_draws(seir_sampler *s, int32_t first, int32_t count, double *R_t);
int seir_sampler_read_rt_draws_async(seir_sampler *s, int32_t first, int32_t count, double *R_t);
int seir_sampler_read_rt(seir_sampler *s, uint64_t *count, double *ref, double *sum, double *sumsq, uint32_t *gt1);

int seir_sampler_rt_keep(seir_sampler *s, int64_t cap);
int seir_sampler_rt_order_stats(seir_sampler *s, const int64_t *ranks, int32_t R, int32_t pooled, double *out);
int seir_order_stats_f64(seir_ctx *ctx, const double *values, int64_t cells, int32_t segs, int64_t seg_len, int64_t seg_stride,
                         int64_t cell_stride, const int64_t *ranks, int32_t R, double *out);

int seir_sampler_wb_reset(seir_sampler *s, int32_t days);
int seir_sampler_wb(seir_sampler *s, int32_t first_slot, int32_t count);
int seir_sampler_read_wb(seir_sampler *s, uint64_t *count, uint32_t *n, double *ref_w, double *sum_w, double *sumsq_w,
                         double *ref_b, double *sum_b, uint32_t *gt);
int seir_sampler_read_wb_draws(seir_sampler *s, int32_t first, int32_t count, double *within_pressure, double *between_pressure);
int seir_sampler_read_wb_draws_async(seir_sampler *s, int32_t first, int32_t count, double *within_pressure,
                                     double *between_pressure);

#define SEIR_CHECK_MAX_DAYS 128
int seir_sampler_check_reset(seir_sampler *s, int32_t days, const double *W, const double *weekday_c, uint64_t seed);
int seir_sampler_check(seir_sampler *s, int32_t first_slot, int32_t count);
int seir_sampler_read_check(seir_sampler *s, uint64_t *count, int32_t *ref, int64_t *sum, uint64_t *sumsq);
int seir_sampler_read_check_marginals(seir_sampler *s, int32_t first, int32_t count, int64_t *check_by_day,
                                      int64_t *check_by_location, int64_t *check_state_by_day);
int seir_sampler_read_check_marginals_async(seir_sampler *s, int32_t first, int32_t count, int64_t *check_by_day,
                                            int64_t *check_by_location, int64_t *check_state_by_day);
int seir_sampler_read_check_counts(seir_sampler *s, int32_t *obs, uint32_t *lt, uint32_t *eq, uint32_t *loc_lt,
                                   uint32_t *loc_eq, uint32_t *day_lt, uint32_t *day_eq, uint32_t *all_lt, uint32_t *all_eq);

#define SEIR_GROUPS_MAX 256
int seir_sampler_groups_set(seir_sampler *s, int32_t G, const int32_t *offsets, const int32_t *members);
int seir_sampler_read_group_marginals(seir_sampler *s, int32_t which, int32_t first, int32_t count, int64_t *events_by_group,
                                      int64_t *state0_by_group);
int seir_sampler_read_group_marginals_async(seir_sampler *s, int32_t which, int32_t first, int32_t count,
                                            int64_t *events_by_group, int64_t *state0_by_group);
int seir_group_sums(seir_ctx *ctx, const int32_t *events, int64_t n, int32_t M, int32_t L, int32_t G, const int32_t *offsets,
                    const int32_t *members, int64_t *out);

int seir_sampler_group_rt(seir_sampler *s, const double *weights);
int seir_sampler_group_wb(seir_sampler *s, int32_t on);
int seir_sampler_read_group_rt(seir_sampler *s, int32_t first, int32_t count, double *Rg);
int seir_sampler_read_group_wb(seir_sampler *s, int32_t first, int32_t count, double *Wg, double *Bg);
int seir_sampler_read_group_rt_async(seir_sampler *s, int32_t first, int32_t count, double *Rg);
int seir_sampler_read_group_wb_async(seir_sampler *s, int32_t first, int32_t count, double *Wg, double *Bg);
int seir_group_wsums(seir_ctx *ctx, const double *v, int64_t nd, int32_t L, int32_t M, int32_t G, const int32_t *offsets,
                     const int32_t *members, const double *weights, double *out);

int seir_reproduction_number(seir_ctx *ctx, int32_t n, const double *theta, const double *events, double *R_it);

int seir_within_between(seir_ctx *ctx, int32_t n, const double *psi, const double *I_last, double W,
                        double *within, double *between);

typedef struct seir_sim_desc {
    int32_t num_draws;
    int32_t num_steps;
    int32_t first_draw_id;
    int32_t reserved;
    uint64_t seed;
    const double *par;
    const double *log_baseline;
    const double *spatial;
    const double *W;
    const double *weekday_c;
    const double *init_state;
    double *events;
} seir_sim_desc;

int seir_simulate(seir_ctx *ctx, const seir_sim_desc *sim);

int seir_selftest_binomial(seir_ctx *ctx, int32_t count, const int32_t *n, const double *p, uint64_t seed,
                           int32_t *out);

#ifdef __cplusplus
}
#endif
#endif
```

Measured before the change: 27950 posterior samples/sec.

## Carry first S->E move prefetch across sweeps in paired moves kernel

The closing step of the paired-moves kernel now draws and proposes the next sweep's first S->E move and stores it in an extra carry buffer with sweep tags. The first pair of the next sweep then reuses it when the tags match, instead of drawing it on the critical path. RNG keys in the solo path are made deterministic from sweep0 so the draw can happen a sweep ahead. Buffers are resized, the carry is dropped on restore, refresh and form changes, a paired-nocarry mode is added, and counters for used and discarded carries are exposed. This adds extra work in the closing step and recomputes the down delta when the carry is used, and a carried move is wasted if HMC changes the state it depended on.

Result: no change. 28170 posterior samples/sec, median of 6 (+0.8%).

```diff
diff --git a/covid19uk_amd/_lib.py b/covid19uk_amd/_lib.py
--- a/covid19uk_amd/_lib.py
+++ b/covid19uk_amd/_lib.py
@@ -150,6 +150,8 @@
     "seir_sampler_time_leapfrog": (ctypes.c_int, [ctypes.c_void_p, ctypes.c_int32, ctypes.POINTER(ctypes.c_float),
                                                   ctypes.POINTER(ctypes.c_int32), ctypes.POINTER(ctypes.c_int32)]),
     "seir_sampler_pair_timeouts": (ctypes.c_int, [ctypes.c_void_p, ctypes.POINTER(ctypes.c_uint32)]),
+    "seir_sampler_pair_carry": (ctypes.c_int, [ctypes.c_void_p, ctypes.POINTER(ctypes.c_uint32),
+                                               ctypes.POINTER(ctypes.c_uint32)]),
     "seir_sampler_xcd_local": (ctypes.c_int, [ctypes.c_void_p]),
     "seir_sampler_snapshot": (ctypes.c_int, [ctypes.c_void_p, ctypes.c_int32]),
     "seir_sampler_restore": (ctypes.c_int, [ctypes.c_void_p, ctypes.c_int32]),
diff --git a/covid19uk_amd/csrc/moves_kernel.h b/covid19uk_amd/csrc/moves_kernel.h
--- a/covid19uk_amd/csrc/moves_kernel.h
+++ b/covid19uk_amd/csrc/moves_kernel.h
@@ -72,11 +72,12 @@
 
 __device__ __forceinline__ double mv_log(double x, const double2 *ltab) { return x == 1.0 ? 0.0 : fast_log(x, ltab); }
 
-__device__ inline void mv_draw(const SamplerCfg &s, const Chains &ch, int b, MoveSpec spec, MvShared &sm, int T) {
+__device__ inline void mv_draw(const SamplerCfg &s, const Chains &ch, int b, MoveSpec spec, MvShared &sm, int T,
+                               bool fixed = false, unsigned sweep = 0u) {
     Move &mv = sm.mv;
     const int tid = threadIdx.x;
     if (tid >= 2 * MMAX && tid != 64) return;
-    const RngKey key = rng_key(s, ch, b);
+    const RngKey key = fixed ? RngKey{s.k0, s.k1, (uint32_t)(s.chain0 + b), sweep} : rng_key(s, ch, b);
     const uint32_t stream = RS_MOVE_BASE + (uint32_t)(spec.scan * 4 + spec.slot);
     if (tid < 2 * MMAX) rng_uniform2(key, stream, (uint32_t)tid, sm.u[tid][0], sm.u[tid][1]);
     if (tid == 64) {
@@ -706,6 +707,8 @@
     int n, rows[MMAX];
 };
 static_assert(sizeof(PairNote) == (2 + MMAX) * sizeof(int), "k_move_pair writes the note as 2 + MMAX ints");
+constexpr int CARRY_BUF = 2, CARRY_TAGS = 3;
+enum { CARRY_DRAW = 1, CARRY_USE = 2 };
 
 __device__ __forceinline__ void move_copy_l2(Move *dst, const Move *src, int t0) {
     const int i = (int)threadIdx.x - t0;
@@ -981,9 +984,11 @@
 __device__ __forceinline__ void pair_step(const Dims &d, const Consts &c, const Work &w, const SamplerCfg &s, const Chains &ch,
                                           MoveSpec se, MoveSpec next, MoveSpec se_next, int have_prev, int have_pre, int pbuf,
                                           int lidx, int dbg, int nband, int nroles, int slot, int b, int fin = 0,
-                                          unsigned sweep0 = 0u, int lprev = 0, unsigned tslot = TRACE_NOT_RECORDED) {
+                                          unsigned sweep0 = 0u, int lprev = 0, unsigned tslot = TRACE_NOT_RECORDED,
+                                          int carry = 0) {
     extern __shared__ __attribute__((aligned(16))) int dyn_i[];
     __shared__ MvShared sm_se, sm_nx;
+    __shared__ unsigned s_ctag[2];
     __shared__ Move pendA, pendB;
     __shared__ PairNote note;
     __shared__ double pre_down[2], s_down[4], s_dsum[2];
@@ -1001,7 +1006,7 @@
             pair_band_finish(d, c, w, s, ch, b, slot - nroles, nband, pair_token(sweep0, lidx), tslot, fin & 2);
             return;
         }
-        const unsigned tok = pair_token(ch.sweep[b], lidx);
+        const unsigned tok = pair_token(SOLO ? sweep0 : ch.sweep[b], lidx);
         const bool r1 = next.kind >= 0 && nroles >= 2, r2 = se_next.kind >= 0 && nroles == 3;
         if ((d.M + nband - 1) / nband > 2 * MVW)
             pair_band_block<SOLO, 4>(d, c, w, s, ch, b, slot - nroles, nband, tok, r1, r2, pbuf ^ 1, slot, lidx);
@@ -1040,7 +1045,8 @@
     int pre_se[PRE_RT], pre_nx[PRE_RT];
     mv_prefetch_rows(d, w, s, b, se, do_se && pre_ok, pre_se);
     mv_prefetch_rows(d, w, s, b, mine, (role == 2 || do_nx) && pre_ok, pre_nx);
-    const unsigned token = pair_token(ch.sweep[b], lidx);
+    const unsigned token = pair_token(SOLO ? sweep0 : ch.sweep[b], lidx);
+    const bool cdraw = SOLO && (carry & CARRY_DRAW), cuse = SOLO && (carry & CARRY_USE);
     double dth0 = 0.0, dcn0 = 0.0;
     int ld_i = 0;
     double ld_d = 0.0;
@@ -1068,7 +1074,7 @@
         if (few ? tid >= DW0 : (tid & ~(WAVE - 1)) < s.nrb_d) {
             const uint4 *src = ch.llD + (((size_t)pbuf * s.B + b) * s.nrb_d + min(i0, s.nrb_d - 1)) * 2;
             double th, cn;
-            pair_sums_wait(src, pair_token(ch.sweep[b], lprev), ch.late + ch.late_fatal + b, th, cn);
+            pair_sums_wait(src, pair_token(sweep0, lprev), ch.late + ch.late_fatal + b, th, cn);
             if (i0 < s.nrb_d) { dth0 = th; dcn0 = cn; }
 #ifdef PAIR_STAMPS
             if (tid == DW0 && b_stamp == 0 && lidx < 12) ch.leap_st[((size_t)slot * 12 + lidx) * 16 + 7] = __builtin_amdgcn_s_memrealtime();
@@ -1077,9 +1083,11 @@
     }
     const bool pre_avail = do_se && have_pre;
     if (pre_avail) {
-        if (tid >= 256 && tid < 256 + MOVE_DW) ld_i = reinterpret_cast<const int *>(ch.mvs + (size_t)pbuf * s.B + b)[tid - 256];
-        if (tid >= 320 && tid < 320 + 2 + MMAX) ld_i = reinterpret_cast<const int *>(ch.prev + (size_t)pbuf * s.B + b)[tid - 320];
+        const int pslot = cuse ? CARRY_BUF : pbuf;
+        if (tid >= 256 && tid < 256 + MOVE_DW) ld_i = reinterpret_cast<const int *>(ch.mvs + (size_t)pslot * s.B + b)[tid - 256];
+        if (tid >= 320 && tid < 320 + 2 + MMAX) ld_i = reinterpret_cast<const int *>(ch.prev + (size_t)pslot * s.B + b)[tid - 320];
         if (tid == 328 || tid == 329) ld_d = ch.DownS[((size_t)pbuf * s.B + b) * 2 + (tid - 328)];
+        if (cuse && (tid == 330 || tid == 331)) ld_i = reinterpret_cast<const int *>(ch.prev + (size_t)CARRY_TAGS * s.B + b)[tid - 330];
     }
     static_assert(MOVE_DW <= 64 && 2 + MMAX <= 8, "the entry loads of pair_step: disjoint thread ranges");
     double hs_th = 0.0, hs_cn = 0.0, psi = 0.0;
@@ -1093,8 +1101,8 @@
     }
     psi = w.scal[(size_t)b * NSCAL + SC_PSI];
     QSTAMP(slot, lidx, 6);
-    if (do_se && !pre_avail) mv_draw(s, ch, b, se, sm_se, T);
-    if (role != 0 || do_nx) mv_draw(s, ch, b, mine, sm_nx, T);
+    if (do_se && !pre_avail) mv_draw(s, ch, b, se, sm_se, T, SOLO, sweep0);
+    if (role != 0 || do_nx) mv_draw(s, ch, b, mine, sm_nx, T, SOLO, (cdraw && role == 2) ? sweep0 + 1u : sweep0);
     QSTAMP(slot, lidx, 14);
     if (have_prev) {
         if (tid >= 64 && tid < 64 + MOVE_DW) reinterpret_cast<int *>(&pendA)[tid - 64] = ld_i;
@@ -1106,6 +1114,7 @@
         if (tid >= 256 && tid < 256 + MOVE_DW) reinterpret_cast<int *>(&sm_se.mv)[tid - 256] = ld_i;
         if (tid >= 320 && tid < 320 + 2 + MMAX) reinterpret_cast<int *>(&note)[tid - 320] = ld_i;
         if (tid == 328 || tid == 329) pre_down[tid - 328] = ld_d;
+        if (cuse && (tid == 330 || tid == 331)) s_ctag[tid - 330] = (unsigned)ld_i;
     }
     if (tid < LDSTAB_N) ltab[tid] = ld_t;
     if (have_prev && s.nrb_d <= WAVE && tid >= DW0 && tid < DW0 + WAVE) {
@@ -1155,8 +1164,12 @@
         mv_propose<NCH>(d, w, s, ch, b, mine, sm_nx, L, ltab);
         QSTAMP(slot, lidx, 2);
         RSTAMP(10);
-        Move *out = (role == 1 ? ch.mv : ch.mvs) + (size_t)(pbuf ^ 1) * s.B + b;
+        Move *out = (role == 1 ? ch.mv : ch.mvs) + (size_t)(cdraw ? CARRY_BUF : pbuf ^ 1) * s.B + b;
         move_copy(out, &sm_nx.mv, MVB - WAVE);
+        if (cdraw) {
+            if (tid == MVB - 1) reinterpret_cast<int *>(ch.prev + (size_t)CARRY_TAGS * s.B + b)[1] = (int)(sweep0 + 2u);
+            return;
+        }
         if (nband > 0 && role == 1 && tid >= MVB - WAVE)
             move_store_ll<MOVE_DW>(ch.llmv + ((size_t)(pbuf ^ 1) * s.B + b) * 32, reinterpret_cast<const int *>(&sm_nx.mv), tid - (MVB - WAVE),
                                    token);
@@ -1225,8 +1238,14 @@
     bool se_acc = false;
     if (do_se) {
         const Move *fpp = (pend_acc && pendp->any_dI) ? pendp : nullptr;
+        if (cuse) lds_barrier();
         if (tid == 0) {
             int use = pre_avail && note.ok;
+            if (cuse) {
+                const bool mine_ = s_ctag[0] == sweep0 + 1u && s_ctag[1] == sweep0 + 1u;
+                use &= mine_ ? 1 : 0;
+                s_ctag[0] = mine_ ? 1u : 0u;
+            }
             if (use) {
                 const Move &mv = sm_se.mv;
                 for (int i = 0; i < mv.n; ++i) {
@@ -1236,6 +1255,7 @@
                 }
             }
             s_use_pre = use;
+            if (cuse && s_ctag[0]) ch.late[(size_t)(use ? 2 : 3) * s.B + b] += 1u;
         }
         lds_barrier();
         const bool use_pre = s_use_pre != 0;
@@ -1243,7 +1263,7 @@
         if (!use_pre) {
             if (pre_avail) {
                 lds_barrier();
-                mv_draw(s, ch, b, se, sm_se, T);
+                mv_draw(s, ch, b, se, sm_se, T, SOLO, sweep0);
             }
             mv_rows_to_lds(d, w, s, b, se, pre_ok, pre_se, nullptr, L, rtl);
             PSTAMP(2);
@@ -1251,7 +1271,7 @@
             PSTAMP(3);
         }
         const Move &mv = sm_se.mv;
-        if (use_pre && fpp == nullptr) {
+        if (use_pre && fpp == nullptr && !cuse) {
             dth = pre_down[0]; dcn = pre_down[1];
         } else {
             if (mv.valid && mv.n > 0) own_rows_delta<MVB>(d, c, w, b, mv, psi, 0, M, ltab, dth, dcn, fpp);
@@ -1315,7 +1335,8 @@
         QSTAMP(slot, lidx, 3);
     }
     if (do_pre && tid == 0) {
-        int *nt = reinterpret_cast<int *>(ch.prev + (size_t)(pbuf ^ 1) * s.B + b);
+        int *nt = reinterpret_cast<int *>(ch.prev + (size_t)(cdraw ? CARRY_BUF : pbuf ^ 1) * s.B + b);
+        if (cdraw) reinterpret_cast<int *>(ch.prev + (size_t)CARRY_TAGS * s.B + b)[0] = (int)(sweep0 + 2u);
         const int n_pend = pend_acc ? pendp->n : 0, n_se = se_acc ? sm_se.mv.n : 0;
         const bool se_keeps = !se_acc || (((s_trans & (se_next.kind == 0 ? 1 : 2)) == 0) && n_pend + n_se <= MMAX);
         nt[0] = (se_keeps && !(waited && late2)) ? 1 : 0;
@@ -1405,14 +1426,16 @@
     for (int pair = 0; pair <= npairs; ++pair) {
         const bool closing = pair == npairs;
         const int scan = pair >> 1, half = pair & 1, nh = half ^ 1, nscan = scan + half;
-        const bool pre = pre_on && pair + 1 < npairs;
+        const bool pre = (pre_on & 1) && pair + 1 < npairs;
         const MoveSpec se = closing ? none : MoveSpec{half, 0, 2 * half, scan};
         const MoveSpec nx = closing ? MoveSpec{-2, 0, 0, 0} : MoveSpec{half, 1, 2 * half + 1, scan};
-        const MoveSpec se_next = pre ? MoveSpec{nh, 0, 2 * nh, nscan} : none;
+        const bool carry = (pre_on & 2) != 0;
+        const MoveSpec se_next = pre ? MoveSpec{nh, 0, 2 * nh, nscan} : (closing && carry) ? MoveSpec{0, 0, 0, 0} : none;
         if (dbg & PAIR_DBG_DELAYS) pair_debug_delay(dbg, slot, nroles, pair, b);
-        pair_step<NCH, true>(d, c, w, s, ch, se, nx, se_next, pair > 0 ? 1 : 0, (pair > 0 && pre_on && !closing) ? 1 : 0, pair & 1,
+        pair_step<NCH, true>(d, c, w, s, ch, se, nx, se_next, pair > 0 ? 1 : 0,
+                       ((pair > 0 && (pre_on & 1) && !closing) || (pair == 0 && carry)) ? 1 : 0, pair & 1,
                        closing ? 62 : pair, closing ? 0 : dbg, (closing && !fin) ? 0 : nband, nroles, slot, b, closing ? fin : 0, sweep0,
-                       pair - 1, tslot);
+                       pair - 1, tslot, !carry ? 0 : closing ? CARRY_DRAW : pair == 0 ? CARRY_USE : 0);
         if (closing) break;
         const int b_stamp = b - d.b0;
         (void)b_stamp;
diff --git a/covid19uk_amd/csrc/seir_hip.hip b/covid19uk_amd/csrc/seir_hip.hip
--- a/covid19uk_amd/csrc/seir_hip.hip
+++ b/covid19uk_amd/csrc/seir_hip.hip
@@ -1170,6 +1170,7 @@
     bool xcd_local = false;
     unsigned long long tail_count = 0;
     unsigned pbar_count = 0;
+    bool carry_live = false;
     int pair_debug = 0;
     int moves_mode = 0;
     int graph_skew = 0, graph_aff = 3;
@@ -1367,8 +1368,8 @@
     if (ds->num_leapfrog_steps < 1) return fail(SEIR_ERR_INVALID, "num_leapfrog_steps must be >= 1");
     if (ds->trace_capacity < 1) return fail(SEIR_ERR_INVALID, "trace_capacity must be >= 1");
     if (ds->record_events < 0 || ds->record_events > 2) return fail(SEIR_ERR_INVALID, "record_events is 0, 1 or 2");
-    if (ds->moves_mode < 0 || ds->moves_mode > 4 || ds->hmc_mode < 0 || ds->hmc_mode > 6)
-        return fail(SEIR_ERR_INVALID, "moves_mode is 0..4, hmc_mode 0..6");
+    if (ds->moves_mode < 0 || ds->moves_mode > MOVES_MODE_MAX || ds->hmc_mode < 0 || ds->hmc_mode > 6)
+        return fail(SEIR_ERR_INVALID, "moves_mode is 0..5, hmc_mode 0..6");
     if (ds->disable_mask < 0 || ds->disable_mask > 31) return fail(SEIR_ERR_INVALID, "disable_mask is a 5-bit mask");
     if (ds->leap_rows != 0 && ds->leap_rows != 24 && ds->leap_rows != 32) return fail(SEIR_ERR_INVALID, "leap_rows is 0 (auto), 24 or 32");
     if (ds->thin < 0) return fail(SEIR_ERR_INVALID, "thin must be >= 0 (0 or 1: every sweep is recorded)");
@@ -1429,7 +1430,7 @@
     S_HAND(ch.mvfix, (size_t)2 * B);
     S_HAND(ch.mvsel, (size_t)2 * B);
     S_HAND(ch.hand, (size_t)B);
-    S_HAND(ch.late, (size_t)2 * B);
+    S_HAND(ch.late, (size_t)4 * B);
     ch.late_fatal = B;
     S_HAND(ch.tail, (size_t)B * TAIL_STRIDE + (size_t)B * TAIL_FLAG_STRIDE);
     S_HAND(ch.leap, (size_t)B * LEAP_CH);
@@ -1446,9 +1447,9 @@
     S_HAND(ch.pbar, (size_t)B * PBAR_STRIDE);
     S_HAND(ch.finpart, (size_t)B * ROLE_SLOTS * 4);
     S_HAND(ch.hand2, (size_t)B);
-    S_HAND(ch.mvs, (size_t)2 * B);
+    S_HAND(ch.mvs, (size_t)3 * B);
     S_HAND(ch.DownS, (size_t)2 * B * 2);
-    S_HAND(ch.prev, (size_t)2 * B);
+    S_HAND(ch.prev, (size_t)4 * B);
     S_HAND(ch.Dpart, (size_t)B * c.nrb_d * 2);
     S_HAND(ch.llD, (size_t)2 * B * c.nrb_d * 2);
     S_HAND(ch.Down, (size_t)2 * 2 * B * 2);
@@ -1493,7 +1494,7 @@
         }
         if (e != hipSuccess) rc = fail(SEIR_ERR_DEVICE, "sampler stream setup failed: %s", hipGetErrorString(e));
     }
-    if (!rc && (HMC_FORMS[ds->hmc_mode].roles || ds->moves_mode == 0 || ds->moves_mode == 2 || ds->moves_mode == 4)) {
+    if (!rc && (HMC_FORMS[ds->hmc_mode].roles || ds->moves_mode == 0 || ds->moves_mode == 2 || ds->moves_mode == 4 || ds->moves_mode == 5)) {
         if (ctx->xcd_local < 0) ctx->xcd_local = probe_xcd_local(ctx->stream) ? 1 : 0;
         const bool ok = ctx->xcd_local == 1;
         s->xcd_local = ok;
@@ -1529,10 +1530,17 @@
     return 0;
 }
 
+static int drop_carry(seir_sampler *s) {
+    HIP_TRY(hipMemsetAsync(s->ch.prev + (size_t)CARRY_BUF * s->cfg.B, 0, sizeof(PairNote) * (size_t)2 * s->cfg.B, s->ctx->stream));
+    s->carry_live = false;
+    return 0;
+}
+
 static int reset_handoffs(seir_sampler *s) {
     hipStream_t st = s->ctx->stream;
     for (const auto &r : s->regions)
         if (r.kind == seir_sampler::R_HANDOFF) HIP_TRY(hipMemsetAsync(r.p, 0, r.bytes, st));
+    s->carry_live = false;
     s->leap_rsteps = s->leap_steps = 0;
     s->tail_count = 0;
     s->pbar_count = 0;
@@ -1543,12 +1551,13 @@
 extern "C" int seir_sampler_set_launch_form(seir_sampler *s, int32_t hmc_mode, int32_t moves_mode) {
     int rc = sampler_check(s);
     if (rc) return rc;
-    if (moves_mode < 0 || moves_mode > 4 || hmc_mode < 0 || hmc_mode > 6)
-        return fail(SEIR_ERR_INVALID, "moves_mode is 0..4, hmc_mode 0..6");
+    if (moves_mode < 0 || moves_mode > MOVES_MODE_MAX || hmc_mode < 0 || hmc_mode > 6)
+        return fail(SEIR_ERR_INVALID, "moves_mode is 0..5, hmc_mode 0..6");
     if (hmc_mode != s->hmc_mode || moves_form(moves_mode, s->cfg.n_scans) != s->moves_mode) {
         HIP_TRY(hipStreamSynchronize(s->ctx->stream));
         drop_graph(s);
         apply_launch_form(s, hmc_mode, moves_mode);
+        if ((rc = drop_carry(s))) return rc;
     }
     return 0;
 }
@@ -1630,6 +1639,7 @@
             off += (r.bytes + 255) / 256 * 256;
         }
     if ((rc = reset_handoffs(s))) return rc;
+    if ((rc = drop_carry(s))) return rc;
     if ((rc = moments_shadow(s, slot, false))) return rc;
     s->vt_dirty = true;
     HIP_TRY(hipStreamSynchronize(st));
@@ -1658,6 +1668,7 @@
         HIP_TRY(hipStreamSynchronize(s->ctx->stream));
         if ((rc = reset_handoffs(s))) return rc;
     }
+    if ((rc = drop_carry(s))) return rc;
     enqueue_refresh(s);
     HIP_TRY(hipGetLastError());
     return 0;
@@ -1680,6 +1691,7 @@
     hipLaunchKernelGGL(k_import_events, dim3(1024), dim3(256), 0, ctx->stream, d, ctx->w, s->ev_stage, B);
     s->have_state = true;
     if (s->poisoned && (rc = reset_handoffs(s))) return rc;
+    if ((rc = drop_carry(s))) return rc;
     enqueue_refresh(s);
     HIP_TRY(hipGetLastError());
     HIP_TRY(hipStreamSynchronize(ctx->stream));
@@ -2018,7 +2030,7 @@
         if (p.nband) cp.nrb_d = p.nband;
         if (p.moves == SweepPlan::PAIRS) {
             hipLaunchKernelGGL(move_pairs_fn(p.nch), dim3((3 + p.nband) * p.nbk), dim3(MVB), k_move_pairs_lds_bytes(d), st, dp, ctx->c, ctx->w, cp,
-                               s->ch, npairs, 1, p.nbk, s->pair_debug, p.nband, s->pbar_count, s->record_events ? 3 : 1);
+                               s->ch, npairs, p.carry ? 3 : 1, p.nbk, s->pair_debug, p.nband, s->pbar_count, s->record_events ? 3 : 1);
             s->pbar_count += (unsigned)(npairs * 3);
         } else {
             int have_pre = 0;
@@ -2060,6 +2072,9 @@
     if (n < 0) return fail(SEIR_ERR_INVALID, "num_sweeps must be >= 0");
     if (s->poisoned) return check_handoffs(s);
     hipStream_t main_st = s->ctx->stream;
+    const bool carry = plan_sweep(sweep_inputs(s, 0)).carry;
+    if (!carry && s->carry_live && n > 0 && (rc = drop_carry(s))) return rc;
+    if (carry && n > 0) s->carry_live = true;
     HIP_TRY(hipEventRecord(s->ev_fork, main_st));
     for (int g = 0; g < s->ngroups; ++g) {
         hipStream_t st = s->gstream[g];
@@ -3650,6 +3665,17 @@
 }
 #endif
 
+extern "C" int seir_sampler_pair_carry(seir_sampler *s, uint32_t *used, uint32_t *discarded) {
+    int rc = sampler_check(s);
+    if (rc) return rc;
+    if (!used || !discarded) return fail(SEIR_ERR_INVALID, "null pointer");
+    HIP_TRY(hipStreamSynchronize(s->ctx->stream));
+    std::vector<uint32_t> both((size_t)2 * s->cfg.B, 0u);
+    HIP_TRY(hipMemcpy(both.data(), s->ch.late + (size_t)2 * s->cfg.B, sizeof(uint32_t) * both.size(), hipMemcpyDeviceToHost));
+    for (int b = 0; b < s->cfg.B; ++b) { used[b] = both[b]; discarded[b] = both[(size_t)s->cfg.B + b]; }
+    return 0;
+}
+
 extern "C" int seir_sampler_pair_timeouts(seir_sampler *s, uint32_t *out) {
     int rc = sampler_check(s);
     if (rc) return rc;
diff --git a/covid19uk_amd/csrc/sweep_plan.h b/covid19uk_amd/csrc/sweep_plan.h
--- a/covid19uk_amd/csrc/sweep_plan.h
+++ b/covid19uk_amd/csrc/sweep_plan.h
@@ -13,6 +13,7 @@
 }
 
 inline int moves_form(int moves_mode, int n_scans) { return n_scans > 30 ? 1 : moves_mode; }
+constexpr int MOVES_MODE_MAX = 5;
 inline int chunk_ts_mode(int Mp) { return Mp <= 512 ? 1 : 2; }
 inline int move_nch(int Tp) { return Tp <= 6 * plan::WAVE ? 6 : Tp <= 12 * plan::WAVE ? 12 : 16; }
 
@@ -50,6 +51,7 @@
     int section_launches, section_evals;
     int moves, nband, nbk, pair_nlive, nch, fpend;
     bool pre, move_aff, record, advance;
+    bool carry;
 };
 
 inline SweepPlan plan_sweep(const SweepInputs &in) {
@@ -103,8 +105,9 @@
             p.nbk = p.nbv;
             p.pair_nlive = p.nlive;
         }
-        p.pre = moves == 0 || moves == 3 || moves == 4;
-        const bool pairs = p.nband > 0 && moves == 0 && in.n_scans > 0 && in.pairs_lds;
+        p.pre = moves == 0 || moves == 3 || moves == 4 || moves == 5;
+        const bool pairs = p.nband > 0 && (moves == 0 || moves == 5) && in.n_scans > 0 && in.pairs_lds;
+        p.carry = pairs && moves == 0;
         p.moves = pairs ? SweepPlan::PAIRS : SweepPlan::PAIR;
         p.fpend = pairs ? SweepPlan::F_PAIRS : in.n_scans == 0 ? SweepPlan::F_NONE
                 : in.record_events ? SweepPlan::F_RECORD : SweepPlan::F_APPLY;
diff --git a/covid19uk_amd/sampler.py b/covid19uk_amd/sampler.py
--- a/covid19uk_amd/sampler.py
+++ b/covid19uk_amd/sampler.py
@@ -11,7 +11,7 @@
 from .seir import SeirModel, _dptr
 
 MOVE_KEYS = ("move/S->E", "move/E->I", "occult/S->E", "occult/E->I")
-MOVES_MODES = {"paired": 0, "split": 1, "paired-nopre": 2, "paired-delta": 3, "paired-launch": 4}
+MOVES_MODES = {"paired": 0, "split": 1, "paired-nopre": 2, "paired-delta": 3, "paired-launch": 4, "paired-nocarry": 5}
 HMC_MODES = {"chunk": 0, "single": 1, "chunk-split": 2, "chunk-launch": 3, "chunk-leap": 4, "chunk-stage": 5,
              "chunk-launch-fold": 6}
 FALLBACK_FORMS = (("chunk-launch", "paired-launch"), ("chunk-split", "paired-delta"))
@@ -1055,6 +1055,12 @@
     def xcd_local(self) -> bool:
         return bool(self._lib.seir_sampler_xcd_local(self._s))
 
+    def pair_carry(self):
+        used, disc = np.zeros(self.B, dtype=np.uint32), np.zeros(self.B, dtype=np.uint32)
+        p32 = ctypes.POINTER(ctypes.c_uint32)
+        _lib.check(self._lib.seir_sampler_pair_carry(self._s, used.ctypes.data_as(p32), disc.ctypes.data_as(p32)))
+        return used, disc
+
     def pair_timeouts(self) -> np.ndarray:
         out = np.zeros(self.B, dtype=np.uint32)
         _lib.check(self._lib.seir_sampler_pair_timeouts(self._s, out.ctypes.data_as(ctypes.POINTER(ctypes.c_uint32))))
diff --git a/include/seir_hip.h b/include/seir_hip.h
--- a/include/seir_hip.h
+++ b/include/seir_hip.h
@@ -161,6 +161,7 @@
 int seir_sampler_xcd_local(seir_sampler *s);
 
 int seir_sampler_pair_timeouts(seir_sampler *s, uint32_t *out);
+int seir_sampler_pair_carry(seir_sampler *s, uint32_t *used, uint32_t *discarded);
 
 int seir_sampler_time_leapfrog(seir_sampler *s, int32_t sweeps, float *mean_ms, int32_t *launches, int32_t *evals);
 
```
